# LittleDang/2DLIW-SLAM

Hardware: AMD Instinct MI355X
Metric: sliding-window solves/sec (30 KF, 2k scan pts) (higher is better)
Workload: dtype f64; 1 GPU; C2 synthetic: 49152 windows/GPU x (n=30 frames, L=2000 laser_factor blocks, 29 IMU + 29 wheel, 1800 ground); step = init-topology LM solve (cap 50 iters) + marginalization per window; windows_per_gpu=49152, frames=30, laser_blocks=2000, parallelism=windows replicated over 1 GPU(s), no data-path collective, distinct_windows_per_gpu=64

## Files before the change

### 2dliw-slam_amd/__init__.py

```python
import ctypes as C
import os

import numpy as np

_HERE = os.path.dirname(os.path.abspath(__file__))
LIB_PATH = os.path.join(_HERE, "libliw_window.so")

LIW_MODE_INIT, LIW_MODE_TRACK, LIW_MODE_MARG = 0, 1, 2
LIW_ENODEV = -19
LASER_PARTIAL = 128
LASER_PARTIAL_COMPACT = 48

dp = C.POINTER(C.c_double)
ip = C.POINTER(C.c_int)
up = C.POINTER(C.c_ubyte)


class LiwError(RuntimeError):
    def __init__(self, code, msg):
        super().__init__("liw error %d: %s" % (code, msg))
        self.code = code


class ParamsC(C.Structure):
    _fields_ = [("T_imu_to_wheel", C.c_double * 16), ("T_imu_to_laser", C.c_double * 16), ("g", C.c_double),
                ("line_to_line_sigma", C.c_double), ("manifold_p_sigma", C.c_double), ("manifold_q_sigma", C.c_double),
                ("imu_noise_acc_sigma", C.c_double * 3), ("imu_bias_acc_sigma", C.c_double * 3),
                ("imu_noise_gyro_sigma", C.c_double * 3), ("imu_bias_gyro_sigma", C.c_double * 3),
                ("wheel_sigma", C.c_double * 3), ("fast_mode", C.c_int), ("normalize_extrinsics", C.c_int),
                ("device", C.c_int)]


class WindowC(C.Structure):
    _fields_ = [("n", C.c_int), ("L", C.c_int), ("states", dp), ("laser_frame", ip), ("laser_pts", dp),
                ("match_pose", dp), ("has_match", up), ("imu_X", dp), ("imu_J", dp), ("imu_sqrtP", dp), ("imu_Dt", dp),
                ("wheel_T", dp), ("wheel_sqrtP", dp), ("wheel_Dt", dp)]


class SummaryC(C.Structure):
    _fields_ = [("iterations", C.c_int), ("successful_steps", C.c_int), ("termination", C.c_int),
                ("initial_cost", C.c_double), ("final_cost", C.c_double)]


class BatchC(C.Structure):
    _fields_ = [("B", C.c_int), ("n", C.c_int), ("Ltot", C.c_int), ("x", C.c_void_p), ("laser_off", C.c_void_p),
                ("laser_frame", C.c_void_p), ("laser_pts", C.c_void_p), ("match_pose", C.c_void_p),
                ("has_match", C.c_void_p), ("imu_X", C.c_void_p), ("imu_J", C.c_void_p), ("imu_sqrtP", C.c_void_p),
                ("imu_Dt", C.c_void_p), ("wheel_T", C.c_void_p), ("wheel_sqrtP", C.c_void_p), ("prior_X", C.c_void_p),
                ("prior_J", C.c_void_p), ("prior_R", C.c_void_p), ("has_prior", C.c_void_p), ("eval_small", C.c_int),
                ("history_records", C.c_int)]


class WsLayoutC(C.Structure):
    _fields_ = [("bytes", C.c_size_t), ("laser_partial_off", C.c_size_t * 2), ("laser_partial_bytes", C.c_size_t),
                ("info_off", C.c_size_t), ("history_off", C.c_size_t), ("laser_partial_stride", C.c_int)]


EXPORTS = [
    "liw_create", "liw_destroy", "liw_last_error", "liw_get_extrinsics", "liw_set_window", "liw_clear_window", "liw_solve", "liw_get_history",
    "liw_linearize", "liw_eval_factors", "liw_marginalize", "liw_get_prior", "liw_set_prior", "liw_batch_ws_layout",
    "liw_batch_set_max_iters", "liw_batch_launch_paths", "liw_batch_packed_rows", "liw_batch_linearize", "liw_batch_time_kernels", "liw_batch_lm_begin", "liw_batch_lm_linearize", "liw_batch_laser_records", "liw_batch_lm_step",
    "liw_batch_lm_finish", "liw_batch_lm_linearize_async", "liw_batch_lm_join", "liw_batch_exchange_doubles", "liw_batch_exchange_pack",
    "liw_batch_exchange_unpack", "liw_batch_solve_sharded", "liw_batch_exchange_timing", "liw_batch_p2p_area_doubles", "liw_batch_p2p_setup", "liw_batch_p2p_status", "liw_batch_solve", "liw_batch_marg_linearize", "liw_batch_marg_schur", "liw_batch_export_dense",
    "liw_set_timing", "liw_get_timing", "liw_batch_imu_preint", "liw_batch_wheel_preint", "liw_imu_preint_create", "liw_imu_preint_destroy", "liw_imu_preint_reset",
    "liw_imu_preint_add", "liw_imu_preint_update_only_t", "liw_imu_preint_Dt", "liw_imu_preint_result",
    "liw_wheel_preint_create", "liw_wheel_preint_destroy", "liw_wheel_preint_reset", "liw_wheel_preint_add",
    "liw_wheel_preint_update_only_t", "liw_wheel_preint_result",
]

_LIB = None


def lib():
    global _LIB
    if _LIB is None:
        if not os.path.exists(LIB_PATH):
            raise LiwError(-2, "libliw_window.so is not built (run python 2dliw-slam_amd/build.py); there is no CPU fallback")
        try:
            import torch
        except ImportError:
            pass
        L = C.CDLL(LIB_PATH)
        L.liw_create.restype = C.c_void_p
        L.liw_create.argtypes = [C.POINTER(ParamsC)]
        L.liw_last_error.restype = C.c_char_p
        L.liw_last_error.argtypes = [C.c_void_p]
        L.liw_destroy.argtypes = [C.c_void_p]
        L.liw_imu_preint_create.restype = C.c_void_p
        L.liw_imu_preint_create.argtypes = [C.POINTER(ParamsC)]
        L.liw_wheel_preint_create.restype = C.c_void_p
        L.liw_wheel_preint_create.argtypes = [C.POINTER(ParamsC)]
        L.liw_imu_preint_Dt.restype = C.c_double
        for name in ("liw_imu_preint_destroy", "liw_wheel_preint_destroy"):
            getattr(L, name).argtypes = [C.c_void_p]
        _LIB = L
    return _LIB


def params_struct(prm, device=0):
    s = ParamsC()
    s.T_imu_to_wheel[:] = [float(v) for v in np.asarray(prm["T_imu_to_wheel"], dtype=np.float64).reshape(16)]
    s.T_imu_to_laser[:] = [float(v) for v in np.asarray(prm["T_imu_to_laser"], dtype=np.float64).reshape(16)]
    for k in ("g", "line_to_line_sigma", "manifold_p_sigma", "manifold_q_sigma"):
        setattr(s, k, float(prm[k]))
    for k in ("imu_noise_acc_sigma", "imu_bias_acc_sigma", "imu_noise_gyro_sigma", "imu_bias_gyro_sigma", "wheel_sigma"):
        getattr(s, k)[:] = [float(v) for v in prm[k]]
    s.fast_mode = int(bool(prm.get("fast_mode", False)))
    s.normalize_extrinsics = int(bool(prm.get("normalize_extrinsics", True)))
    s.device = int(device)
    return s


def _p(a):
    return a.ctypes.data_as(dp)


WINDOW_FIELDS = ("states", "laser_frame", "laser_pts", "match_pose", "has_match", "imu_X", "imu_J", "imu_sqrtP", "imu_Dt",
                 "wheel_T", "wheel_sqrtP", "wheel_Dt")


class Window:

    def __init__(self, d):
        self.n = int(d["n"])
        self.a = {}
        for k in WINDOW_FIELDS:
            dt = np.int32 if k == "laser_frame" else (np.uint8 if k == "has_match" else np.float64)
            arr = np.ascontiguousarray(np.array(d[k], dtype=dt, copy=True))
            if arr.size == 0:
                arr = np.zeros(12 if k == "laser_pts" else 1, dtype=dt)
            self.a[k] = arr
        self.L = int(np.asarray(d["laser_frame"]).shape[0])
        c = WindowC()
        c.n, c.L = self.n, self.L
        c.states = _p(self.a["states"]); c.laser_frame = self.a["laser_frame"].ctypes.data_as(ip)
        c.laser_pts = _p(self.a["laser_pts"]); c.match_pose = _p(self.a["match_pose"])
        c.has_match = self.a["has_match"].ctypes.data_as(up)
        for k in ("imu_X", "imu_J", "imu_sqrtP", "imu_Dt", "wheel_T", "wheel_sqrtP", "wheel_Dt"):
            setattr(c, k, _p(self.a[k]))
        self.c = c

    def __getitem__(self, k):
        return self.a[k]


class Solver:

    def __init__(self, prm, device=0):
        self.L = lib()
        self._ps = params_struct(prm, device)
        self.h = C.c_void_p(self.L.liw_create(C.byref(self._ps)))
        if not self.h:
            raise LiwError(-22, "liw_create failed")
        self.win = None

    def close(self):
        if self.h:
            self.L.liw_destroy(self.h)
            self.h = None

    def __del__(self):
        try:
            self.close()
        except Exception:
            pass

    def _chk(self, r):
        if r < 0:
            raise LiwError(r, self.L.liw_last_error(self.h).decode())
        return r

    def extrinsics(self):
        a, b = np.zeros(16), np.zeros(16)
        self._chk(self.L.liw_get_extrinsics(self.h, _p(a), _p(b)))
        return a.reshape(4, 4), b.reshape(4, 4)

    def set_window(self, win):
        self.win = win
        self._chk(self.L.liw_set_window(self.h, C.byref(win.c)))

    def _solve(self, mode, max_iters):
        s = SummaryC()
        self._chk(self.L.liw_solve(self.h, C.c_int(mode), C.c_int(max_iters), C.byref(s)))
        return dict(iterations=s.iterations, successful=s.successful_steps, termination=s.termination,
                    initial_cost=s.initial_cost, final_cost=s.final_cost)

    def init_solve(self, max_iters=0):
        return self._solve(LIW_MODE_INIT, max_iters)

    def solve(self, max_iters=0):
        return self._solve(LIW_MODE_TRACK, max_iters)

    def history(self, max_records=128):
        x = np.zeros((max_records, self.win.n, 15))
        r = self._chk(self.L.liw_get_history(self.h, _p(x), C.c_int(max_records)))
        return x[:r]

    def linearize(self, mode):
        N = 15 * self.win.n
        H, g, c = np.zeros((N, N)), np.zeros(N), C.c_double(0)
        self._chk(self.L.liw_linearize(self.h, C.c_int(mode), _p(H), _p(g), C.byref(c)))
        return H, g, c.value

    def eval_factors(self, mode):
        n, L = self.win.n, self.win.L
        out = dict(laser_res=np.zeros((max(L, 1), 2)), laser_jac=np.zeros((max(L, 1), 2, 12)), imu_res=np.zeros((max(n - 1, 1), 15)),
                   imu_jac=np.zeros((max(n - 1, 1), 15, 30)), wheel_res=np.zeros((max(n - 1, 1), 3)), wheel_jac=np.zeros((max(n - 1, 1), 3, 12)),
                   ground_res=np.zeros((n, 2)), ground_jac=np.zeros((n, 2, 6)))
        self._chk(self.L.liw_eval_factors(self.h, C.c_int(mode), *[_p(out[k]) for k in
                                          ("laser_res", "laser_jac", "imu_res", "imu_jac", "wheel_res", "wheel_jac", "ground_res", "ground_jac")]))
        out["laser_res"], out["laser_jac"] = out["laser_res"][:L], out["laser_jac"][:L]
        out["imu_res"], out["imu_jac"] = out["imu_res"][:n - 1], out["imu_jac"][:n - 1]
        out["wheel_res"], out["wheel_jac"] = out["wheel_res"][:n - 1], out["wheel_jac"][:n - 1]
        return out

    def marginalization(self):
        out = np.zeros(36 + 225 + 15)
        base = out.ctypes.data
        self._chk(self.L.liw_marginalize(self.h, C.cast(base, dp), C.cast(base + 36 * 8, dp), C.cast(base + 261 * 8, dp)))
        return dict(sqrt_H=out[:36].reshape(6, 6), Delta_H=out[36:261].reshape(15, 15), Delta_g=out[261:])

    def get_prior(self):
        X, J, R = np.zeros(15), np.zeros(225), np.zeros(15)
        has = self._chk(self.L.liw_get_prior(self.h, _p(X), _p(J), _p(R)))
        return (X, J.reshape(15, 15), R) if has else None

    def set_prior(self, prior):
        if prior is None:
            self._chk(self.L.liw_set_prior(self.h, C.c_int(0), None, None, None))
            return
        X, J, R = [np.ascontiguousarray(v, dtype=np.float64) for v in prior]
        self._chk(self.L.liw_set_prior(self.h, C.c_int(1), _p(X), _p(J.reshape(225)), _p(R)))


class ImuPreintegration:

    def __init__(self, prm):
        self.L = lib()
        self._ps = params_struct(prm)
        self.h = C.c_void_p(self.L.liw_imu_preint_create(C.byref(self._ps)))

    def __del__(self):
        try:
            self.L.liw_imu_preint_destroy(self.h)
        except Exception:
            pass

    def reset_imu_measure(self, time, acc_bias, gyr_bias):
        a, g = np.ascontiguousarray(acc_bias, dtype=np.float64), np.ascontiguousarray(gyr_bias, dtype=np.float64)
        self.L.liw_imu_preint_reset(self.h, C.c_double(time), _p(a), _p(g))

    def add_imu_measure(self, t, acc, gyro):
        a, g = np.ascontiguousarray(acc, dtype=np.float64), np.ascontiguousarray(gyro, dtype=np.float64)
        return bool(self.L.liw_imu_preint_add(self.h, C.c_double(t), _p(a), _p(g)))

    def update_only_t(self, t):
        self.L.liw_imu_preint_update_only_t(self.h, C.c_double(t))

    @property
    def Dt(self):
        return self.L.liw_imu_preint_Dt(self.h)

    def get_preintegraption_result(self):
        X, J, P, Dt = np.zeros(15), np.zeros(225), np.zeros(225), C.c_double(0)
        self.L.liw_imu_preint_result(self.h, _p(X), _p(J), _p(P), C.byref(Dt))
        return X, J.reshape(15, 15), P.reshape(15, 15), Dt.value


class WheelPreintegration:

    def __init__(self, prm):
        self.L = lib()
        self._ps = params_struct(prm)
        self.h = C.c_void_p(self.L.liw_wheel_preint_create(C.byref(self._ps)))

    def __del__(self):
        try:
            self.L.liw_wheel_preint_destroy(self.h)
        except Exception:
            pass

    def reset_wheel_odom_measure(self, time):
        self.L.liw_wheel_preint_reset(self.h, C.c_double(time))

    def add_wheel_odom_measure(self, t, R9, t3):
        r, tt = np.ascontiguousarray(R9, dtype=np.float64).reshape(9), np.ascontiguousarray(t3, dtype=np.float64)
        return bool(self.L.liw_wheel_preint_add(self.h, C.c_double(t), _p(r), _p(tt)))

    def update_only_t(self, t):
        self.L.liw_wheel_preint_update_only_t(self.h, C.c_double(t))

    def get_preintegraption_result(self):
        T, P, Dt = np.zeros(12), np.zeros(9), C.c_double(0)
        self.L.liw_wheel_preint_result(self.h, _p(T), _p(P), C.byref(Dt))
        return T, P.reshape(3, 3), Dt.value


class HostPreint:

    def __init__(self, prm):
        self.prm = prm

    def imu_preint(self, samples, t_start, t_end, bias6):
        p = ImuPreintegration(self.prm)
        for i, s in enumerate(np.asarray(samples)):
            p.add_imu_measure(s[0], s[1:4], s[4:7])
            if i == 0:
                p.reset_imu_measure(t_start, bias6[0:3], bias6[3:6])
        p.update_only_t(t_end)
        return p.get_preintegraption_result()

    def wheel_preint(self, samples, t_start, t_end):
        p = WheelPreintegration(self.prm)
        did = False
        for s in np.asarray(samples):
            if not did and s[0] > t_start:
                p.update_only_t(t_start)
                p.reset_wheel_odom_measure(t_start)
                did = True
            p.add_wheel_odom_measure(s[0], s[1:10], s[10:13])
        if not did:
            p.update_only_t(t_start)
            p.reset_wheel_odom_measure(t_start)
        p.update_only_t(t_end)
        return p.get_preintegraption_result()


from .batch import BatchPreint, BatchSolver, shard_laser
from . import fleet, gridmap, laser, laser_batch, loop, loop_batch, outputs, posegraph, posegraph_batch
from .fleet import FleetTracker, FleetTrajectory
from .loop_batch import FleetLoopDetector
from .posegraph_batch import FleetBackEnd
```

### 2dliw-slam_amd/batch.py

```python
import ctypes as C

import numpy as np


XFN = C.CFUNCTYPE(C.c_int, C.c_void_p, C.c_void_p, C.c_void_p, C.c_size_t, C.c_void_p)


def shard_laser(win, rank, world):
    L = int(np.asarray(win["laser_frame"]).shape[0])
    lo, hi = (L * rank) // world, (L * (rank + 1)) // world
    out = dict(win)
    out["laser_frame"] = np.asarray(win["laser_frame"])[lo:hi].copy()
    out["laser_pts"] = np.asarray(win["laser_pts"])[lo:hi].copy()
    return out


def allreduce_sum_(t, group=None):
    import torch.distributed as dist
    if dist.is_available() and dist.is_initialized() and dist.get_world_size(group) > 1:
        dist.all_reduce(t, op=dist.ReduceOp.SUM, group=group)
    return t


def allgather_(out, t, group=None):
    import torch.distributed as dist
    if dist.is_available() and dist.is_initialized() and dist.get_world_size(group) > 1:
        if t.is_cuda and dist.get_backend(group) == "gloo":
            import torch
            host = torch.empty(out.shape, dtype=out.dtype)
            dist.all_gather_into_tensor(host.view(-1), t.cpu(), group=group)
            out.copy_(host)
        else:
            dist.all_gather_into_tensor(out.view(-1), t, group=group)
    else:
        out.view(-1)[:t.numel()].copy_(t)
    return out


EXCHANGES = ("allreduce", "oneshot", "auto", "p2p")


class TorchComm:

    def __init__(self, group=None):
        self.group = group

    def all_reduce_sum_(self, t):
        return allreduce_sum_(t, self.group)

    def all_gather_(self, out, t):
        return allgather_(out, t, self.group)

    def all_reduce_max_(self, t):
        import torch.distributed as dist
        if dist.is_available() and dist.is_initialized() and dist.get_world_size(self.group) > 1:
            if t.is_cuda and dist.get_backend(self.group) == "gloo":
                h = t.cpu()
                dist.all_reduce(h, op=dist.ReduceOp.MAX, group=self.group)
                t.copy_(h)
            else:
                dist.all_reduce(t, op=dist.ReduceOp.MAX, group=self.group)
        return t


class LockstepComm:

    def __init__(self, shared, rank):
        self.sh, self.rank = shared, rank

    @staticmethod
    def make(world):
        import threading
        shared = {"slots": [None] * world, "bar": threading.Barrier(world), "world": world}
        return [LockstepComm(shared, r) for r in range(world)]

    def _deposit(self, t):
        self.sh["slots"][self.rank] = t
        self.sh["bar"].wait()

    def all_reduce_sum_(self, t):
        self._deposit(t)
        tot = self.sh["slots"][0].clone()
        for r in range(1, self.sh["world"]):
            tot += self.sh["slots"][r]
        self.sh["bar"].wait()
        t.copy_(tot)
        self.sh["bar"].wait()
        return t

    def all_gather_(self, out, t):
        self._deposit(t)
        for r in range(self.sh["world"]):
            out[r].copy_(self.sh["slots"][r])
        self.sh["bar"].wait()
        return out

    def all_reduce_max_(self, t):
        self._deposit(t)
        tot = self.sh["slots"][0].clone()
        for r in range(1, self.sh["world"]):
            tot = self.torch_max(tot, self.sh["slots"][r])
        self.sh["bar"].wait()
        t.copy_(tot)
        self.sh["bar"].wait()
        return t

    @staticmethod
    def torch_max(a, b):
        import torch
        return torch.maximum(a, b)


def host_arrays(windows):
    B = len(windows)
    Ls = [int(np.asarray(w["laser_frame"]).shape[0]) for w in windows]
    Ltot = int(sum(Ls))
    off = np.zeros(B + 1, dtype=np.int32)
    off[1:] = np.cumsum(Ls)
    cat = lambda k, dt: np.ascontiguousarray(np.concatenate([np.asarray(w[k], dtype=dt).reshape(-1) for w in windows]))
    pts = np.concatenate([np.asarray(w["laser_pts"], dtype=np.float64).reshape(-1, 12) for w in windows], axis=0) if Ltot else np.zeros((1, 12))
    return dict(
        x=cat("states", np.float64), laser_off=off, laser_frame=cat("laser_frame", np.int32) if Ltot else np.zeros(1, np.int32),
        laser_pts=np.ascontiguousarray(pts.T).reshape(-1),
        match_pose=cat("match_pose", np.float64), has_match=cat("has_match", np.uint8),
        imu_X=cat("imu_X", np.float64), imu_J=cat("imu_J", np.float64), imu_sqrtP=cat("imu_sqrtP", np.float64), imu_Dt=cat("imu_Dt", np.float64),
        wheel_T=cat("wheel_T", np.float64), wheel_sqrtP=cat("wheel_sqrtP", np.float64),
        prior_X=np.zeros(B * 15), prior_J=np.zeros(B * 225), prior_R=np.zeros(B * 15), has_prior=np.zeros(B, dtype=np.int32), _Ltot=Ltot)


def tiled_tensors(base, tile, device):
    import torch
    B, nb, n = int(tile["B"]), len(base), int(base[0]["n"])
    dev = torch.device(device)
    assert B >= 1 and nb >= 1
    reps, rem = divmod(B, nb)
    host = host_arrays(base)
    Lb = int(host.pop("_Ltot"))
    Lrem = int(host["laser_off"][rem])
    Ltot = reps * Lb + Lrem
    assert Ltot < 2 ** 31, "laser_off is int32"
    d = {k: torch.from_numpy(a if a.size else np.zeros(1, dtype=a.dtype)).to(dev) for k, a in host.items()}

    t_ = {}

    def cyc(t, per):
        if per == 0 or t.numel() < nb * per:
            return t.clone()
        return torch.cat([t.repeat(reps), t[:rem * per]]) if rem else t.repeat(reps)
    for k, per in (("has_match", n), ("imu_X", (n - 1) * 15), ("imu_J", (n - 1) * 225), ("imu_sqrtP", (n - 1) * 225), ("imu_Dt", n - 1),
                   ("wheel_T", (n - 1) * 12), ("wheel_sqrtP", (n - 1) * 9)):
        t_[k] = cyc(d[k], per)
    if Lb:
        pb = d["laser_pts"].view(12, Lb)
        t_["laser_pts"] = (torch.cat([pb.repeat(1, reps), pb[:, :Lrem]], dim=1) if Lrem else pb.repeat(1, reps)).contiguous().view(-1)
        fb = d["laser_frame"]
        t_["laser_frame"] = torch.cat([fb.repeat(reps), fb[:Lrem]]) if Lrem else fb.repeat(reps)
    else:
        t_["laser_pts"], t_["laser_frame"] = d["laser_pts"], d["laser_frame"]
    ob = d["laser_off"][:nb].to(torch.int64)
    off = (torch.arange(reps, device=dev, dtype=torch.int64)[:, None] * Lb + ob[None, :]).reshape(-1)
    tail = reps * Lb + d["laser_off"][:rem + 1].to(torch.int64)
    t_["laser_off"] = torch.cat([off, tail]).to(torch.int32)
    assert t_["laser_off"].numel() == B + 1
    st = np.ascontiguousarray(np.asarray(tile["states"], dtype=np.float64).reshape(-1))
    mp = np.ascontiguousarray(np.asarray(tile["match_pose"], dtype=np.float64).reshape(-1))
    assert st.size == B * n * 15 and mp.size == B * n * 12
    t_["x"] = torch.from_numpy(st).to(dev)
    t_["match_pose"] = torch.from_numpy(mp).to(dev)
    z = lambda m, dt=torch.float64: torch.zeros(m, dtype=dt, device=dev)
    t_.update(prior_X=z(B * 15), prior_J=z(B * 225), prior_R=z(B * 15), has_prior=z(B, torch.int32))
    return t_, B, Ltot


class BatchSolver:

    def __init__(self, prm, windows, device="cuda:0", history_records=0, rank=0, world=1, group=None, exchange="allreduce", force_exchange=False, comm=None, tile=None):
        import torch
        from . import BatchC, WsLayoutC, lib, params_struct, LiwError
        self.torch = torch
        self.LiwError = LiwError
        self.L = lib()
        self.dev = torch.device(device)
        dev_index = self.dev.index if self.dev.index is not None else 0
        self._ps = params_struct(prm, dev_index)
        self.h = C.c_void_p(self.L.liw_create(C.byref(self._ps)))
        self.rank, self.world, self.group = rank, world, group
        assert exchange in EXCHANGES, exchange
        self.exchange, self.sharded = exchange, (world > 1 or force_exchange)
        self.comm = comm if comm is not None else TorchComm(group)
        self.exchange_ms, self.exchange_calls, self._xev, self._xbuf = 0.0, 0, [], {}
        self.time_exchange = False
        if world > 1:
            windows = [shard_laser(w, rank, world) for w in windows]
        self.n = int(windows[0]["n"])
        n = self.n
        for w in windows:
            assert int(w["n"]) == n, "uniform n per batch"
        if tile is None:
            self.B = len(windows)
            host = host_arrays(windows)
            self.Ltot = int(host.pop("_Ltot"))
            self.t = {}
            for k, a in host.items():
                if a.size == 0:
                    a = np.zeros(1, dtype=a.dtype)
                self.t[k] = torch.from_numpy(a).to(self.dev)
        else:
            self.t, self.B, self.Ltot = tiled_tensors(windows, tile, self.dev)
        B = self.B
        self.history_records = int(history_records)
        lay = WsLayoutC()
        r = self.L.liw_batch_ws_layout(C.c_int(B), C.c_int(n), C.c_int(self.history_records), C.byref(lay))
        if r < 0:
            raise LiwError(r, "liw_batch_ws_layout")
        self.lay = lay
        self.ws = torch.zeros(int(lay.bytes), dtype=torch.uint8, device=self.dev)
        b = BatchC()
        b.B, b.n, b.Ltot = B, n, self.Ltot
        for k in ("x", "laser_off", "laser_frame", "laser_pts", "match_pose", "has_match", "imu_X", "imu_J", "imu_sqrtP", "imu_Dt",
                  "wheel_T", "wheel_sqrtP", "prior_X", "prior_J", "prior_R", "has_prior"):
            setattr(b, k, self.t[k].data_ptr())
        b.eval_small = 1
        b.history_records = self.history_records
        self.b = b
        nd = int(lay.laser_partial_bytes) // 8
        self.PL_raw = [self.ws[int(lay.laser_partial_off[k]):int(lay.laser_partial_off[k]) + nd * 8].view(torch.float64) for k in range(2)]
        self._pl_mode = 0

    @property
    def PL(self):
        from . import LASER_PARTIAL
        if int(self.lay.laser_partial_stride) == LASER_PARTIAL:
            return self.PL_raw
        out = []
        for k in range(2):
            o = self.torch.empty(self.B * self.n * LASER_PARTIAL, dtype=self.torch.float64, device=self.dev)
            self._chk(self.L.liw_batch_laser_records(self.h, C.byref(self.b), C.c_int(self._pl_mode), C.c_int(k), self._wsp(),
                                                     C.c_void_p(o.data_ptr()), self._stream()))
            out.append(o)
        return out

    INPUT_KEYS = ("x", "laser_off", "laser_frame", "laser_pts", "match_pose", "has_match", "imu_X", "imu_J", "imu_sqrtP", "imu_Dt", "wheel_T", "wheel_sqrtP")

    def rebind(self, t, Ltot):
        for k in self.INPUT_KEYS:
            self.t[k] = t[k]
            setattr(self.b, k, t[k].data_ptr())
        self.Ltot = int(Ltot)
        self.b.Ltot = int(Ltot)

    def close(self):
        if self.h:
            self.L.liw_destroy(self.h)
            self.h = None

    def __del__(self):
        try:
            self.close()
        except Exception:
            pass

    def _chk(self, r):
        if r < 0:
            raise self.LiwError(r, self.L.liw_last_error(self.h).decode())
        return r

    def _stream(self):
        return C.c_void_p(self.torch.cuda.current_stream(self.dev).cuda_stream)

    def _wsp(self):
        return C.c_void_p(self.ws.data_ptr())

    def launch_paths(self):
        flags, rows, blocks = C.c_int(0), C.c_longlong(0), C.c_longlong(0)
        self._chk(self.L.liw_batch_launch_paths(self.h, C.byref(self.b), self._wsp(), C.byref(flags)))
        self._chk(self.L.liw_batch_packed_rows(self.h, C.byref(self.b), self._wsp(), C.byref(rows), C.byref(blocks)))
        return dict(flags=flags.value, large_batch_format=bool(flags.value & 1), lane_per_group_laser=bool(flags.value & 2), packed_rows=rows.value,
                    blocks=blocks.value, padding_ratio=(64.0 * rows.value / blocks.value) if (rows.value and blocks.value) else None)

    def solve(self, mode, max_iters=0, use_graph=False):
        self._pl_mode = int(mode)
        if not self.sharded:
            if use_graph:
                torch = self.torch
                if getattr(self, "_side", None) is None:
                    self._side = torch.cuda.Stream(device=self.dev)
                cur = torch.cuda.current_stream(self.dev)
                self._side.wait_stream(cur)
                with torch.cuda.stream(self._side):
                    self._chk(self.L.liw_batch_solve(self.h, C.byref(self.b), C.c_int(mode), C.c_int(max_iters), self._wsp(), self._stream(), C.c_int(1)))
                cur.wait_stream(self._side)
                return
            self._chk(self.L.liw_batch_solve(self.h, C.byref(self.b), C.c_int(mode), C.c_int(max_iters), self._wsp(), self._stream(), C.c_int(0)))
            return
        buf, allb, nd = self._xbuffers(mode)
        if self.exchange == "p2p":
            assert getattr(self, "_p2p", None) is not None and self._p2p["mode"] == mode, "attach the receive areas first (p2p_attach_local / p2p_attach_ipc)"
            self._chk(self.L.liw_batch_exchange_timing(self.h, C.c_int(1 if self.time_exchange else 0), None, None))
            self._chk(self.L.liw_batch_solve_sharded(self.h, C.byref(self.b), C.c_int(mode), C.c_int(max_iters), self._wsp(), self._stream(),
                                                     C.c_void_p(buf.data_ptr()), None, C.c_int(max(self.world, 1)), XFN(0), None))
            self._last_x = buf
            return
        oneshot = self.exchange == "oneshot"
        err = []

        def _cb(user, pbuf, pall, doubles, stream):
            try:
                if oneshot:
                    self.comm.all_gather_(allb, buf)
                    return max(self.world, 1)
                self.comm.all_reduce_sum_(buf)
                return 1
            except BaseException as e:
                err.append(e)
                return -1
        cb = XFN(_cb)
        self._chk(self.L.liw_batch_exchange_timing(self.h, C.c_int(1 if self.time_exchange else 0), None, None))
        r = self.L.liw_batch_solve_sharded(self.h, C.byref(self.b), C.c_int(mode), C.c_int(max_iters), self._wsp(), self._stream(),
                                           C.c_void_p(buf.data_ptr()), C.c_void_p(allb.data_ptr()) if allb is not None else None,
                                           C.c_int(max(self.world, 1)), cb, None)
        if err:
            raise err[0]
        self._chk(r)
        self._last_x = allb[0] if oneshot else buf

    def pick_exchange(self, mode, reps=3):
        t = self.torch
        reps = max(1, int(reps))
        nd = int(self.L.liw_batch_exchange_doubles(C.c_int(self.B), C.c_int(self.n), C.c_int(mode)))
        buf = t.zeros(nd, dtype=t.float64, device=self.dev)
        allb = t.zeros((max(self.world, 1), nd), dtype=t.float64, device=self.dev)
        ms = {}
        for name in ("allreduce", "oneshot"):
            for rep in range(reps + 1):
                if rep == 1:
                    e0, e1 = t.cuda.Event(enable_timing=True), t.cuda.Event(enable_timing=True)
                    e0.record()
                if name == "allreduce":
                    self.comm.all_reduce_sum_(buf)
                else:
                    self.comm.all_gather_(allb, buf)
                    buf.copy_(allb.sum(dim=0))
            e1.record()
            t.cuda.synchronize(self.dev)
            ms[name] = e0.elapsed_time(e1) / reps
            buf.zero_()
        both = t.tensor([ms["allreduce"], ms["oneshot"]], dtype=t.float64, device=self.dev)
        self.comm.all_reduce_max_(both)
        ms = {"allreduce": float(both[0].item()), "oneshot": float(both[1].item())}
        ms["picked"] = "oneshot" if ms["oneshot"] < ms["allreduce"] else "allreduce"
        self.exchange = ms["picked"]
        self._xbuf = {}
        self.exchange_pick = ms
        return ms

    def _xbuffers(self, mode):
        if self.exchange == "auto":
            self.pick_exchange(mode)
        nd = int(self.L.liw_batch_exchange_doubles(C.c_int(self.B), C.c_int(self.n), C.c_int(mode)))
        if (mode, "buf") not in self._xbuf:
            t = self.torch
            self._xbuf[(mode, "buf")] = t.zeros(nd, dtype=t.float64, device=self.dev)
            self._xbuf[(mode, "all")] = t.zeros((max(self.world, 1), nd), dtype=t.float64, device=self.dev) if self.exchange == "oneshot" else None
        return self._xbuf[(mode, "buf")], self._xbuf[(mode, "all")], nd

    def exchange_bytes(self, mode):
        return 8 * int(self.L.liw_batch_exchange_doubles(C.c_int(self.B), C.c_int(self.n), C.c_int(mode)))

    def _exchange(self, mode, candidate):
        buf, allb, nd = self._xbuffers(mode)
        s = self._stream()
        ev = None
        if self.time_exchange:
            ev = (self.torch.cuda.Event(enable_timing=True), self.torch.cuda.Event(enable_timing=True))
            ev[0].record()
        self._chk(self.L.liw_batch_exchange_pack(self.h, C.byref(self.b), C.c_int(mode), C.c_int(candidate), self._wsp(), C.c_void_p(buf.data_ptr()), s))
        if self.exchange == "oneshot":
            self.comm.all_gather_(allb, buf)
            self._chk(self.L.liw_batch_exchange_unpack(self.h, C.byref(self.b), C.c_int(mode), C.c_int(candidate), self._wsp(),
                                                       C.c_void_p(allb.data_ptr()), C.c_int(max(self.world, 1)), s))
            self._last_x = allb[0]
        else:
            self.comm.all_reduce_sum_(buf)
            self._chk(self.L.liw_batch_exchange_unpack(self.h, C.byref(self.b), C.c_int(mode), C.c_int(candidate), self._wsp(),
                                                       C.c_void_p(buf.data_ptr()), C.c_int(1), s))
            self._last_x = buf
        if ev:
            ev[1].record()
            self._xev.append(ev)

    def _lin_exchange(self, mode, candidate):
        self._chk(self.L.liw_batch_lm_linearize_async(self.h, C.byref(self.b), C.c_int(mode), C.c_int(candidate), self._wsp(), self._stream()))
        self._exchange(mode, candidate)
        self._chk(self.L.liw_batch_lm_join(self.h, self._stream()))

    def active_windows(self, mode):
        buf, allb, nd = self._xbuffers(mode)
        if self.exchange == "oneshot":
            return int(round(float(allb[:, nd - 1].sum().item()))) // max(self.world, 1)
        return int(round(float(buf[nd - 1].item()))) // max(self.world, 1)

    def _p2p_alloc(self, mode):
        t = self.torch
        L = self.L
        L.liw_batch_p2p_area_doubles.restype = C.c_size_t
        nd = int(L.liw_batch_p2p_area_doubles(C.c_int(self.B), C.c_int(self.n), C.c_int(mode), C.c_int(max(self.world, 1))))
        area = t.zeros(nd, dtype=t.float64, device=self.dev)
        flags = t.zeros(max(self.world, 1), dtype=t.int64, device=self.dev)
        return area, flags

    def _p2p_set(self, mode, area_ptrs, flag_ptrs, keep):
        w = max(self.world, 1)
        A = (C.c_void_p * w)(*area_ptrs)
        F = (C.c_void_p * w)(*flag_ptrs)
        self._chk(self.L.liw_batch_p2p_setup(self.h, C.c_int(self.rank), C.c_int(w), A, F))
        self._p2p = {"mode": mode, "keep": keep}

    @staticmethod
    def p2p_attach_local(ranks, mode):
        bufs = [rk._p2p_alloc(mode) for rk in ranks]
        for rk in ranks:
            rk.torch.cuda.synchronize(rk.dev)
            rk._p2p_set(mode, [a.data_ptr() for a, _ in bufs], [f.data_ptr() for _, f in bufs], bufs)

    def p2p_attach_ipc(self, mode):
        import torch.distributed as dist
        hip = C.CDLL("libamdhip64.so")

        class Handle(C.Structure):
            _fields_ = [("reserved", C.c_byte * 64)]
        L = self.L
        L.liw_batch_p2p_area_doubles.restype = C.c_size_t
        w = max(self.world, 1)
        nd = int(L.liw_batch_p2p_area_doubles(C.c_int(self.B), C.c_int(self.n), C.c_int(mode), C.c_int(w)))
        own = []
        for nbytes in (8 * nd, 8 * w):
            p = C.c_void_p()
            assert hip.hipMalloc(C.byref(p), C.c_size_t(nbytes)) == 0
            assert hip.hipMemset(p, 0, C.c_size_t(nbytes)) == 0
            own.append(p)
        hs = []
        for p in own:
            h = Handle()
            assert hip.hipIpcGetMemHandle(C.byref(h), p) == 0
            hs.append(bytes(h.reserved))
        allh = [None] * w
        dist.all_gather_object(allh, hs, group=self.group)
        areas, flags = [], []
        for r in range(w):
            if r == self.rank:
                areas.append(own[0].value); flags.append(own[1].value)
                continue
            ptrs = []
            for raw in allh[r]:
                h = Handle()
                C.memmove(h.reserved, raw, 64)
                q = C.c_void_p()
                assert hip.hipIpcOpenMemHandle(C.byref(q), h, C.c_uint(1)) == 0
                ptrs.append(q.value)
            areas.append(ptrs[0]); flags.append(ptrs[1])
        dist.barrier(group=self.group)
        self._p2p_ptrs = (areas, flags)
        self._p2p_set(mode, areas, flags, own)

    def exchange_timing(self):
        self.torch.cuda.synchronize(self.dev)
        ms = [a.elapsed_time(b) for a, b in self._xev]
        self._xev = []
        avg, cnt = C.c_double(0.0), C.c_int(0)
        self._chk(self.L.liw_batch_exchange_timing(self.h, C.c_int(1 if self.time_exchange else 0), C.byref(avg), C.byref(cnt)))
        tot, num = sum(ms) + avg.value * cnt.value, len(ms) + cnt.value
        return (tot / num if num else 0.0), num

    def lm_begin(self, mode, max_iters=0):
        K = self._chk(self.L.liw_batch_set_max_iters(self.h, C.c_int(mode), C.c_int(max_iters)))
        self._chk(self.L.liw_batch_lm_begin(self.h, C.byref(self.b), C.c_int(mode), C.c_int(K), self._wsp(), self._stream()))
        return K

    def lm_linearize(self, mode, candidate):
        self._pl_mode = int(mode)
        self._chk(self.L.liw_batch_lm_linearize(self.h, C.byref(self.b), C.c_int(mode), C.c_int(candidate), self._wsp(), self._stream()))

    def lm_step(self, mode):
        self._chk(self.L.liw_batch_lm_step(self.h, C.byref(self.b), C.c_int(mode), self._wsp(), self._stream()))

    def lm_finish(self, mode):
        self._chk(self.L.liw_batch_lm_finish(self.h, C.byref(self.b), C.c_int(mode), self._wsp(), self._stream()))

    def time_kernels(self, mode, reps=3):
        out = (C.c_double * 6)()
        self._chk(self.L.liw_batch_time_kernels(self.h, C.byref(self.b), C.c_int(mode), self._wsp(), self._stream(), C.c_int(reps), out))
        self.torch.cuda.synchronize(self.dev)
        return dict(zip(("k_lin_laser", "k_lin_imu", "k_lin_small", "k_lm_step", "k_marg_schur", "k_lin_laser_marg"), [float(v) for v in out]))

    def linearize(self, mode):
        self._pl_mode = int(mode)
        self._chk(self.L.liw_batch_linearize(self.h, C.byref(self.b), C.c_int(mode), self._wsp(), self._stream()))
        if self.sharded:
            self._exchange_plain(mode)

    def _exchange_plain(self, mode):
        self.comm.all_reduce_sum_(self.PL_raw[0])

    def export_dense(self, mode):
        N = 15 * self.n
        torch = self.torch
        H = torch.zeros((self.B, N, N), dtype=torch.float64, device=self.dev)
        g = torch.zeros((self.B, N), dtype=torch.float64, device=self.dev)
        c = torch.zeros(self.B, dtype=torch.float64, device=self.dev)
        self._chk(self.L.liw_batch_export_dense(self.h, C.byref(self.b), C.c_int(mode), C.c_int(0), self._wsp(), C.c_void_p(H.data_ptr()),
                                                C.c_void_p(g.data_ptr()), C.c_void_p(c.data_ptr()), self._stream()))
        return H, g, c

    def marginalize(self):
        torch = self.torch
        sH = torch.zeros((self.B, 36), dtype=torch.float64, device=self.dev)
        dH = torch.zeros((self.B, 225), dtype=torch.float64, device=self.dev)
        dg = torch.zeros((self.B, 15), dtype=torch.float64, device=self.dev)
        s = self._stream()
        from . import LIW_MODE_MARG as _MARG
        self._pl_mode = _MARG
        self._chk(self.L.liw_batch_marg_linearize(self.h, C.byref(self.b), self._wsp(), s))
        if self.sharded:
            from . import LIW_MODE_MARG
            self._exchange(LIW_MODE_MARG, 0)
        self._chk(self.L.liw_batch_marg_schur(self.h, C.byref(self.b), self._wsp(), C.c_void_p(sH.data_ptr()), C.c_void_p(dH.data_ptr()),
                                              C.c_void_p(dg.data_ptr()), s))
        return sH, dH, dg

    def states(self):
        return self.t["x"].cpu().numpy().reshape(self.B, self.n, 15)

    def set_states(self, x):
        self.t["x"].copy_(self.torch.from_numpy(np.ascontiguousarray(x, dtype=np.float64).reshape(-1)).to(self.dev))

    def summaries(self):
        from . import SummaryC
        raw = self.ws[int(self.lay.info_off):int(self.lay.info_off) + C.sizeof(SummaryC) * self.B].cpu().numpy().tobytes()
        arr = (SummaryC * self.B).from_buffer_copy(raw)
        return [dict(iterations=a.iterations, successful=a.successful_steps, termination=a.termination,
                     initial_cost=a.initial_cost, final_cost=a.final_cost) for a in arr]

    def history(self):
        if not self.history_records:
            return None
        nd = self.history_records * self.B * self.n * 15
        o = int(self.lay.history_off)
        return self.ws[o:o + nd * 8].view(self.torch.float64).cpu().numpy().reshape(self.history_records, self.B, self.n, 15)

    def set_timing(self, on):
        self._chk(self.L.liw_set_timing(self.h, C.c_int(int(on))))

    def get_timing(self):
        a, b, c, d = C.c_double(0), C.c_int(0), C.c_double(0), C.c_int(0)
        self._chk(self.L.liw_get_timing(self.h, C.byref(a), C.byref(b), C.byref(c), C.byref(d)))
        return dict(linearize_ms=a.value, linearize_launches=b.value, step_ms=c.value, step_launches=d.value)


class BatchPreint:

    def __init__(self, prm, device="cuda:0"):
        import torch
        from . import lib, params_struct, LiwError
        self.torch, self.LiwError, self.L = torch, LiwError, lib()
        self.dev = torch.device(device)
        self._ps = params_struct(prm, self.dev.index if self.dev.index is not None else 0)
        self.h = C.c_void_p(self.L.liw_create(C.byref(self._ps)))

    def close(self):
        if self.h:
            self.L.liw_destroy(self.h)
            self.h = None

    def __del__(self):
        try:
            self.close()
        except Exception:
            pass

    def _chk(self, r):
        if r < 0:
            raise self.LiwError(r, self.L.liw_last_error(self.h).decode())

    def _pack(self, intervals, width):
        torch = self.torch
        M = len(intervals)
        cnt = [int(np.asarray(iv[0]).shape[0]) for iv in intervals]
        off = np.zeros(M + 1, dtype=np.int32)
        off[1:] = np.cumsum(cnt)
        smp = np.concatenate([np.asarray(iv[0], dtype=np.float64).reshape(-1, width) for iv in intervals], axis=0) if M else np.zeros((1, width))
        ts = np.array([iv[1] for iv in intervals], dtype=np.float64)
        te = np.array([iv[2] for iv in intervals], dtype=np.float64)
        d = lambda a: torch.from_numpy(np.ascontiguousarray(a)).to(self.dev)
        return M, d(off), d(smp.reshape(-1)), d(ts), d(te)

    def imu(self, intervals):
        torch = self.torch
        M, off, smp, ts, te = self._pack(intervals, 7)
        bias = torch.from_numpy(np.ascontiguousarray(np.array([iv[3] for iv in intervals], dtype=np.float64).reshape(-1))).to(self.dev)
        z = lambda *sh: torch.zeros(sh, dtype=torch.float64, device=self.dev)
        X, J, P, S, Dt = z(M, 15), z(M, 15, 15), z(M, 15, 15), z(M, 15, 15), z(M)
        p = lambda t: C.c_void_p(t.data_ptr())
        self._chk(self.L.liw_batch_imu_preint(self.h, C.c_int(M), p(off), p(smp), p(ts), p(te), p(bias), p(X), p(J), p(P), p(S), p(Dt),
                                              C.c_void_p(torch.cuda.current_stream(self.dev).cuda_stream)))
        self.last_P = P
        return X, J, S, Dt

    def wheel(self, intervals):
        torch = self.torch
        M, off, smp, ts, te = self._pack(intervals, 13)
        z = lambda *sh: torch.zeros(sh, dtype=torch.float64, device=self.dev)
        T, S, Dt = z(M, 12), z(M, 3, 3), z(M)
        p = lambda t: C.c_void_p(t.data_ptr())
        self._chk(self.L.liw_batch_wheel_preint(self.h, C.c_int(M), p(off), p(smp), p(ts), p(te), p(T), p(S), p(Dt),
                                                C.c_void_p(torch.cuda.current_stream(self.dev).cuda_stream)))
        return T, S, Dt
```

### 2dliw-slam_amd/csrc/k_laser_slab.hip

```cpp
#include "liw_kernels.hpp"
#include <algorithm>
#include <cstdlib>

namespace liw {

#ifdef LIW_CLK
__device__ long long g_clk_slab[16];
#define SSTAMP(id) do { asm volatile("s_waitcnt vmcnt(0) lgkmcnt(0)" ::: "memory"); if (item == slab_items_probe && (threadIdx.x & 63) == 0) g_clk_slab[(id)] = clock64(); } while (0)
__device__ int slab_items_probe = 11000;
#else
#define SSTAMP(id) do { } while (0)
#endif

namespace {

constexpr int TF2 = 24;
__device__ __forceinline__ void frame_tf2(const DevParams& P, const double* pose6, double* o) {
    typedef LJN<3> J3;
    const V3<J3> p = cast_v3<J3>(pose6);
    const V3<J3> th(seed<3>(pose6[3], 0, true), seed<3>(pose6[4], 1, true), seed<3>(pose6[5], 2, true));
    const Iso<J3> Twl = mul(make_tf(p, th), cast_iso<J3>(P.Ril, P.til));
    const J3 tt[2] = {Twl.t.x, Twl.t.y};
#pragma unroll
    for (int r = 0; r < 2; ++r) {
#pragma unroll
        for (int c = 0; c < 2; ++c) {
            o[r * 2 + c] = Twl.R(r, c).v;
#pragma unroll
            for (int k = 0; k < 3; ++k) o[6 + 4 * k + 2 * r + c] = Twl.R(r, c).d[k];
        }
        o[4 + r] = tt[r].v;
#pragma unroll
        for (int k = 0; k < 3; ++k) o[18 + 2 * k + r] = tt[r].d[k];
    }
}

constexpr int slab_pairidx(int c1, int c2) { return laser_pairidx<true>(c1, c2); }
constexpr int slab_pairidx1(int c1, int c2) { return laser_pairidx<false>(c1, c2); }
constexpr int slab_slot_code(int s) { return laser_slot_code<true>(s); }
constexpr int slab_slot_code1(int s) { return laser_slot_code<false>(s); }
template <bool BOTH, int S_> __device__ __forceinline__ double slab_slot(const double* acc) {
    constexpr int code = BOTH ? slab_slot_code(S_) : slab_slot_code1(S_);
    if constexpr (code < 0) return 0.0;
    else if constexpr ((code & 64) != 0) return -acc[code & 63];
    else return acc[code & 63];
}

constexpr int STG = 34;
template <bool BOTH, int C_, int I_ = 0> __device__ __forceinline__ void slab_stage(double* st, const double* acc) {
    if constexpr (I_ < 16) {
        typedef double __attribute__((ext_vector_type(2))) dbl2;
        dbl2 v;
        v.x = slab_slot<BOTH, 32 * C_ + 2 * I_>(acc); v.y = slab_slot<BOTH, 32 * C_ + 2 * I_ + 1>(acc);
        *reinterpret_cast<dbl2*>(st + 2 * I_) = v;
        slab_stage<BOTH, C_, I_ + 1>(st, acc);
    }
}
template <bool BOTH, int C_> __device__ __forceinline__ void slab_flush(double* lds, const unsigned long long* pw, const double* acc, int lane) {
    if constexpr (C_ < 4) {
        typedef double __attribute__((ext_vector_type(2))) dbl2;
        lds_sync();
        slab_stage<BOTH, C_>(lds + lane * STG, acc);
        lds_sync();
        const int wq = lane >> 4, pc = lane & 15;
#pragma unroll
        for (int t = 0; t < 16; ++t) {
            const int w = 4 * t + wq;
            const unsigned long long p = pw[w];
            const dbl2 v = *reinterpret_cast<const dbl2*>(lds + w * STG + 2 * pc);
            if (p) __builtin_nontemporal_store(v, reinterpret_cast<dbl2*>(reinterpret_cast<double*>(p) + 32 * C_ + 2 * pc));
        }
        slab_flush<BOTH, C_ + 1>(lds, pw, acc, lane);
    }
}

template <int N_, int S_> __device__ __forceinline__ double slab_total(const double* acc) {
    if constexpr (S_ < N_) return acc[S_]; else return 0.0;
}
template <int N_, int S0_, int CNT_, int I_ = 0> __device__ __forceinline__ void slab_stage_totals(double* st, const double* acc) {
    if constexpr (I_ < CNT_) {
        typedef double __attribute__((ext_vector_type(2))) dbl2;
        dbl2 v;
        v.x = slab_total<N_, S0_ + 2 * I_>(acc); v.y = slab_total<N_, S0_ + 2 * I_ + 1>(acc);
        *reinterpret_cast<dbl2*>(st + 2 * I_) = v;
        slab_stage_totals<N_, S0_, CNT_, I_ + 1>(st, acc);
    }
}
template <int N_> __device__ __forceinline__ void slab_flush_compact(double* lds, const unsigned long long* pw, const double* acc, int lane) {
    typedef double __attribute__((ext_vector_type(2))) dbl2;
    static_assert(LPC == 48 && N_ <= LPC, "one and a half chunks");
    lds_sync();
    slab_stage_totals<N_, 0, 16>(lds + lane * STG, acc);
    lds_sync();
    {
        const int wq = lane >> 4, pc = lane & 15;
#pragma unroll
        for (int t = 0; t < 16; ++t) {
            const int w = 4 * t + wq;
            const unsigned long long p = pw[w];
            const dbl2 v = *reinterpret_cast<const dbl2*>(lds + w * STG + 2 * pc);
            if (p) __builtin_nontemporal_store(v, reinterpret_cast<dbl2*>(reinterpret_cast<double*>(p) + 2 * pc));
        }
    }
    lds_sync();
    slab_stage_totals<N_, 32, 8>(lds + lane * STG, acc);
    lds_sync();
    {
        const int wq = lane >> 3, pc = lane & 7;
#pragma unroll
        for (int t = 0; t < 8; ++t) {
            const int w = 8 * t + wq;
            const unsigned long long p = pw[w];
            const dbl2 v = *reinterpret_cast<const dbl2*>(lds + w * STG + 2 * pc);
            if (p) __builtin_nontemporal_store(v, reinterpret_cast<dbl2*>(reinterpret_cast<double*>(p) + 32 + 2 * pc));
        }
    }
}

__device__ __forceinline__ double slab_weight(double d1x, double d1y, double d2x, double d2y) {
    const double l2 = fmin(d1x * d1x + d1y * d1y, d2x * d2x + d2y * d2y);
    const double lmin25 = l2 > 0.0 ? 25.0 * (l2 * fast_rsqrt(l2)) : 0.0;
    return lmin25 > 0.0 ? lmin25 * fast_rsqrt(lmin25) : 0.0;
}

constexpr int SLAB = 64;
constexpr int ROWD = LASER_SLAB_ROWD;
constexpr int NPL = ROWD / SLAB;

}

template <bool BOTH>
__device__ __forceinline__ void slab_item(const LinArgs& A, const DevParams& P, const int item) {
    const int lane = threadIdx.x & 63, n = A.n;
    const int s = item / n, f = item % n;
    SSTAMP(0);
    const int b = A.laser_perm[(size_t)f * ((size_t)laser_slab_count(A.B) * SLAB) + (size_t)s * SLAB + lane];
    bool in = b >= 0;
    const int bb = in ? b : 0;
    const int g0 = A.group_off[bb * (n + 1) + f], g1 = A.group_off[bb * (n + 1) + f + 1];
    const int hm = A.has_match[bb * n + f];
    const int curv = A.lm ? A.lm[bb].cur : 0;
    double pa6[6], pb6[6];
#pragma unroll
    for (int k = 0; k < 6; ++k) {
        pa6[k] = BOTH ? A.x[(size_t)bb * n * 15 + k] : A.match_pose[((size_t)bb * n + f) * 12 + k];
        pb6[k] = A.x[((size_t)bb * n + f) * 15 + k];
    }
    if (in) in = window_live(A, bb);
    if (!__any(in)) return;
    const bool fon = in && hm != 0 && (BOTH || A.mode != LIW_MODE_TRACK || f == n - 1 || A.marg_older);
    const int cnt = fon ? g1 - g0 : 0;
    int maxc = cnt;
#pragma unroll
    for (int o = 32; o > 0; o >>= 1) maxc = max(maxc, __shfl_xor(maxc, o, 64));
    maxc = __builtin_amdgcn_readfirstlane(maxc);
    const int psel = (in && A.lm) ? (A.candidate ? 1 - curv : curv) : 0;
    constexpr int TFR = 4;
    __shared__ double lds[2 * (TF2 - TFR) * SLAB];
    double* const lta = lds;
    double* const ltb = lds + (TF2 - TFR) * SLAB;
    double ra[TFR], rb[TFR];
    SSTAMP(1);
    {
        double ta2[TF2], tb2[TF2];
        if (in && maxc > 0) { frame_tf2(P, pa6, ta2); frame_tf2(P, pb6, tb2); }
        else {
#pragma unroll
            for (int k = 0; k < TF2; ++k) { ta2[k] = 0.0; tb2[k] = 0.0; }
        }
#pragma unroll
        for (int k = 0; k < TF2; ++k) {
            if (k < TFR) { ra[k] = ta2[k]; rb[k] = tb2[k]; }
            else { lta[(k - TFR) * SLAB + lane] = ta2[k]; ltb[(k - TFR) * SLAB + lane] = tb2[k]; }
        }
    }
    lds_sync();
    SSTAMP(2);
    constexpr int NACC = BOTH ? 45 : 21;
    double acc[NACC];
#pragma unroll
    for (int e = 0; e < NACC; ++e) acc[e] = 0.0;
    const double* row0 = A.laser_pk + (size_t)A.laser_slab_off[(size_t)s * n + f] * ROWD + lane;
    auto load_row = [&](double* q, int j) {
        const double* r = row0 + (size_t)j * ROWD;
#pragma unroll
        for (int c = 0; c < NPL; ++c) q[c] = __builtin_nontemporal_load(r + c * SLAB);
    };
    const double w0 = P.laser_sqrt_info;
#define TA(k) ((k) < TFR ? ra[(k) < TFR ? (k) : 0] : lta[((k) < TFR ? 0 : (k) - TFR) * SLAB + lane])
#define TB(k) ((k) < TFR ? rb[(k) < TFR ? (k) : 0] : ltb[((k) < TFR ? 0 : (k) - TFR) * SLAB + lane])
    auto block = [&](const double* p) {
        const double d1x = p[0] - p[2], d1y = p[1] - p[3];
        const double d2x = p[4] - p[6], d2y = p[5] - p[7];
        const double l2 = fmin(d1x * d1x + d1y * d1y, d2x * d2x + d2y * d2y);
        const double lmin25 = l2 > 0.0 ? 25.0 * (l2 * fast_rsqrt(l2)) : 0.0;
        const double sum = lmin25 > 0.0 ? lmin25 * fast_rsqrt(lmin25) : 0.0;
        double Ap[2], Bp[2], C[2][2];
#pragma unroll
        for (int r = 0; r < 2; ++r) {
            Ap[r] = TA(4 + r) + TA(r * 2) * p[0] + TA(r * 2 + 1) * p[1];
            Bp[r] = TA(4 + r) + TA(r * 2) * p[2] + TA(r * 2 + 1) * p[3];
            C[0][r] = TB(4 + r) + TB(r * 2) * p[4] + TB(r * 2 + 1) * p[5];
            C[1][r] = TB(4 + r) + TB(r * 2) * p[6] + TB(r * 2 + 1) * p[7];
        }
        __builtin_amdgcn_sched_barrier(0);
        const double ux = Bp[0] - Ap[0], uy = Bp[1] - Ap[1];
        const double zz = ux * ux + uy * uy;
        const bool regular = zz > 0.0;
        const double rlen = regular ? fast_rsqrt(zz) : 1.0;
        const double lx = ux * rlen, ly = uy * rlen;
        double dBx[3], dBy[3], dlx[3], dly[3];
#pragma unroll
        for (int k = 0; k < 3; ++k) {
            const double m0 = TA(6 + 4 * k), m1 = TA(6 + 4 * k + 1), m3 = TA(6 + 4 * k + 2), m4 = TA(6 + 4 * k + 3);
            const double t0 = TA(18 + 2 * k), t1 = TA(18 + 2 * k + 1);
            const double dAx = t0 + m0 * p[0] + m1 * p[1];
            const double dAy = t1 + m3 * p[0] + m4 * p[1];
            dBx[k] = t0 + m0 * p[2] + m1 * p[3];
            dBy[k] = t1 + m3 * p[2] + m4 * p[3];
            const double dux = dBx[k] - dAx, duy = dBy[k] - dAy;
            const double pr = lx * dux + ly * duy;
            dlx[k] = (dux - lx * pr) * rlen;
            dly[k] = (duy - ly * pr) * rlen;
        }
        const double w = sum * w0;
        __builtin_amdgcn_sched_barrier(0);
#pragma unroll
        for (int k = 0; k < 2; ++k) {
            __builtin_amdgcn_sched_barrier(0);
            const double pt0 = p[4 + 2 * k], pt1 = p[5 + 2 * k];
            const double ex = C[k][0] - Bp[0], ey = C[k][1] - Bp[1];
            double dCx[3], dCy[3];
#pragma unroll
            for (int m = 0; m < 3; ++m) {
                dCx[m] = TB(18 + 2 * m) + TB(6 + 4 * m) * pt0 + TB(6 + 4 * m + 1) * pt1;
                dCy[m] = TB(18 + 2 * m + 1) + TB(6 + 4 * m + 2) * pt0 + TB(6 + 4 * m + 3) * pt1;
            }
            double dist, jc[8], ws = w;
            if (regular) {
                const double sg = lx * ey - ly * ex;
                ws = sg < 0.0 ? -w : w;
                dist = fabs(sg);
                {
                    const double prj = lx * ex + ly * ey;
                    const double vx = ex - prj * lx, vy = ey - prj * ly;
                    if (vx * vx + vy * vy == 0.0) ws = __builtin_nan("");
                }
                jc[0] = ly; jc[1] = -lx;
#pragma unroll
                for (int m = 0; m < 3; ++m) {
                    jc[2 + m] = dlx[m] * ey - dly[m] * ex - lx * dBy[m] + ly * dBx[m];
                    jc[5 + m] = lx * dCy[m] - ly * dCx[m];
                }
            } else {
                dist = sqrt(ex * ex + ey * ey);
                const double nx = ex / dist, ny = ey / dist;
                jc[0] = -nx; jc[1] = -ny;
#pragma unroll
                for (int m = 0; m < 3; ++m) {
                    jc[2 + m] = -(nx * dBx[m] + ny * dBy[m]);
                    jc[5 + m] = nx * dCx[m] + ny * dCy[m];
                }
            }
            __builtin_amdgcn_sched_barrier(0);
            double rw[9];
#pragma unroll
            for (int c = 0; c < 8; ++c) rw[c] = ws * jc[c];
            rw[8] = sum * (w0 * dist);
            if constexpr (BOTH) {
#pragma unroll
                for (int c1 = 0; c1 < 9; ++c1)
#pragma unroll
                    for (int c2 = c1; c2 < 9; ++c2) acc[c1 * 9 - c1 * (c1 - 1) / 2 + (c2 - c1)] += rw[c1] * rw[c2];
            } else {
                const double r1[6] = {-rw[0], -rw[1], rw[5], rw[6], rw[7], rw[8]};
#pragma unroll
                for (int c1 = 0; c1 < 6; ++c1)
#pragma unroll
                    for (int c2 = c1; c2 < 6; ++c2) acc[c1 * 6 - c1 * (c1 - 1) / 2 + (c2 - c1)] += r1[c1] * r1[c2];
            }
        }
    };
    bool irregular = false;
    auto block_fast = [&](const double* p) {
        const double d1x = p[0] - p[2], d1y = p[1] - p[3];
        const double d2x = p[4] - p[6], d2y = p[5] - p[7];
        const double w = slab_weight(d1x, d1y, d2x, d2y) * w0;
        const double ux = -(ra[0] * d1x + ra[1] * d1y), uy = -(ra[2] * d1x + ra[3] * d1y);
        const double zz = ux * ux + uy * uy;
        if (__builtin_expect(!(zz > 0.0), 0)) { irregular = true; return; }
        const double Bx = TA(4) + ra[0] * p[2] + ra[1] * p[3], By = TA(5) + ra[2] * p[2] + ra[3] * p[3];
        const double tbx = TB(4), tby = TB(5);
        double ex[2], ey[2];
#pragma unroll
        for (int k = 0; k < 2; ++k) {
            ex[k] = (tbx + rb[0] * p[4 + 2 * k] + rb[1] * p[5 + 2 * k]) - Bx;
            ey[k] = (tby + rb[2] * p[4 + 2 * k] + rb[3] * p[5 + 2 * k]) - By;
        }
        __builtin_amdgcn_sched_barrier(0);
        const double rlen = fast_rsqrt(zz);
        const double lx = ux * rlen, ly = uy * rlen;
        const double rlw = rlen * w;
        const double lxw = ux * rlw, lyw = uy * rlw;
        double dlxw[3], dlyw[3], kap[3];
        if constexpr (BOTH) {
#pragma unroll
            for (int k = 0; k < 3; ++k) {
                const double m0 = TA(6 + 4 * k), m1 = TA(6 + 4 * k + 1), m3 = TA(6 + 4 * k + 2), m4 = TA(6 + 4 * k + 3);
                const double dux = -(m0 * d1x + m1 * d1y), duy = -(m3 * d1x + m4 * d1y);
                const double pr = lx * dux + ly * duy;
                dlxw[k] = (dux - lx * pr) * rlw;
                dlyw[k] = (duy - ly * pr) * rlw;
                const double dBx = TA(18 + 2 * k) + m0 * p[2] + m1 * p[3];
                const double dBy = TA(18 + 2 * k + 1) + m3 * p[2] + m4 * p[3];
                kap[k] = lyw * dBx - lxw * dBy;
            }
        }
        __builtin_amdgcn_sched_barrier(0);
        double al[3], be[3], ga[3];
#pragma unroll
        for (int m = 0; m < 3; ++m) {
            al[m] = lxw * TB(18 + 2 * m + 1) - lyw * TB(18 + 2 * m);
            be[m] = lxw * TB(6 + 4 * m + 2) - lyw * TB(6 + 4 * m);
            ga[m] = lxw * TB(6 + 4 * m + 3) - lyw * TB(6 + 4 * m + 1);
        }
        const double tiny = 1e-13 * w;
#pragma unroll
        for (int k = 0; k < 2; ++k) {
            __builtin_amdgcn_sched_barrier(0);
            const double pt0 = p[4 + 2 * k], pt1 = p[5 + 2 * k];
            if constexpr (BOTH) {
                double rw[9];
                rw[0] = lyw; rw[1] = -lxw;
                rw[8] = lxw * ey[k] - lyw * ex[k];
#pragma unroll
                for (int m = 0; m < 3; ++m) {
                    rw[2 + m] = dlxw[m] * ey[k] - dlyw[m] * ex[k] + kap[m];
                    rw[5 + m] = al[m] + be[m] * pt0 + ga[m] * pt1;
                }
                if (__builtin_expect(fabs(rw[8]) <= tiny * (fabs(ex[k]) + fabs(ey[k])), 0)) {
                    const double prj = lx * ex[k] + ly * ey[k];
                    const double vx = ex[k] - prj * lx, vy = ey[k] - prj * ly;
                    if (vx * vx + vy * vy == 0.0) {
#pragma unroll
                        for (int c = 0; c < 8; ++c) rw[c] = __builtin_nan("");
                    }
                }
                __builtin_amdgcn_sched_barrier(0);
#pragma unroll
                for (int c1 = 0; c1 < 9; ++c1)
#pragma unroll
                    for (int c2 = c1; c2 < 9; ++c2) acc[c1 * 9 - c1 * (c1 - 1) / 2 + (c2 - c1)] += rw[c1] * rw[c2];
            } else {
                double rw[6];
                rw[0] = -lyw; rw[1] = lxw;
                rw[5] = lxw * ey[k] - lyw * ex[k];
#pragma unroll
                for (int m = 0; m < 3; ++m) rw[2 + m] = al[m] + be[m] * pt0 + ga[m] * pt1;
                if (__builtin_expect(fabs(rw[5]) <= tiny * (fabs(ex[k]) + fabs(ey[k])), 0)) {
                    const double prj = lx * ex[k] + ly * ey[k];
                    const double vx = ex[k] - prj * lx, vy = ey[k] - prj * ly;
                    if (vx * vx + vy * vy == 0.0) {
#pragma unroll
                        for (int c = 0; c < 5; ++c) rw[c] = __builtin_nan("");
                    }
                }
                __builtin_amdgcn_sched_barrier(0);
#pragma unroll
                for (int c1 = 0; c1 < 6; ++c1)
#pragma unroll
                    for (int c2 = c1; c2 < 6; ++c2) acc[c1 * 6 - c1 * (c1 - 1) / 2 + (c2 - c1)] += rw[c1] * rw[c2];
            }
        }
    };
    const int last = maxc - 1;
    double q0[NPL], q1[NPL];
    if (maxc > 0) {
        load_row(q0, 0);
        for (int j = 0; j < maxc; j += 2) {
            asm volatile("" ::: "memory");
            load_row(q1, min(j + 1, last));
            if (j < cnt) block_fast(q0);
            __builtin_amdgcn_sched_barrier(0);
            load_row(q0, min(j + 2, last));
            if (j + 1 < cnt) block_fast(q1);
            __builtin_amdgcn_sched_barrier(0);
        }
    }
    if (__builtin_expect(__any(irregular), 0)) {
        for (int j = 0; j < maxc; ++j) {
            double q[NPL];
            load_row(q, j);
            const double d1x = q[0] - q[2], d1y = q[1] - q[3];
            const double ux = -(ra[0] * d1x + ra[1] * d1y), uy = -(ra[2] * d1x + ra[3] * d1y);
            if (irregular && j < cnt && !(ux * ux + uy * uy > 0.0)) block(q);
        }
    }
    SSTAMP(3);
#undef TA
#undef TB
    {
        static_assert(SLAB * STG + SLAB <= 2 * (TF2 - TFR) * SLAB && LP == 128, "staging area of the record epilogue");
        unsigned long long* pw = reinterpret_cast<unsigned long long*>(lds + SLAB * STG);
        lds_sync();
        pw[lane] = in ? (unsigned long long)((psel ? A.PL[1] : A.PL[0]) + ((size_t)bb * n + f) * laser_stride(A.pl_compact)) : 0ull;
        if (A.pl_compact) slab_flush_compact<NACC>(lds, pw, acc, lane);
        else slab_flush<BOTH, 0>(lds, pw, acc, lane);
    }
    if (in && A.CS[0]) (psel ? A.CS[1] : A.CS[0])[cs_index(n, bb, CS_LASER, f)] = acc[BOTH ? slab_pairidx(8, 8) : slab_pairidx1(5, 5)];
    SSTAMP(4);
}
__global__ __launch_bounds__(64, 2) void k_lin_laser_slab(LinArgs A, DevParams P) { slab_item<true>(A, P, (int)blockIdx.x); }
__global__ __launch_bounds__(64, 2) void k_lin_laser_slab1(LinArgs A, DevParams P) { slab_item<false>(A, P, (int)blockIdx.x); }

constexpr int SORT_BINS = 4096;
__global__ __launch_bounds__(1024) void k_laser_slab_order(int B, int n, const int* group_off, int* perm) {
    __shared__ int bin[SORT_BINS];
    __shared__ int part[1024];
    const int f = (int)blockIdx.x, t = (int)threadIdx.x;
    const size_t Bp = (size_t)((B + SLAB - 1) / SLAB) * SLAB;
    for (int e = t; e < SORT_BINS; e += 1024) bin[e] = 0;
    __syncthreads();
    auto key = [&](int b) { return SORT_BINS - 1 - min(group_off[b * (n + 1) + f + 1] - group_off[b * (n + 1) + f], SORT_BINS - 1); };
    for (int b = t; b < B; b += 1024) atomicAdd(&bin[key(b)], 1);
    __syncthreads();
    int sum = 0;
#pragma unroll
    for (int k = 0; k < SORT_BINS / 1024; ++k) sum += bin[t * (SORT_BINS / 1024) + k];
    part[t] = sum;
    __syncthreads();
    for (int d = 1; d < 1024; d <<= 1) {
        const int v = t >= d ? part[t - d] : 0;
        __syncthreads();
        part[t] += v;
        __syncthreads();
    }
    int base = part[t] - sum;
#pragma unroll
    for (int k = 0; k < SORT_BINS / 1024; ++k) { const int h = bin[t * (SORT_BINS / 1024) + k]; bin[t * (SORT_BINS / 1024) + k] = base; base += h; }
    __syncthreads();
    for (int b = t; b < B; b += 1024) perm[(size_t)f * Bp + atomicAdd(&bin[key(b)], 1)] = b;
    for (size_t e = (size_t)B + t; e < Bp; e += 1024) perm[(size_t)f * Bp + e] = -1;
}
__global__ void k_laser_slab_max(int B, int n, const int* group_off, const int* perm, int* mx) {
    const int t = blockIdx.x * blockDim.x + threadIdx.x;
    const int S = (B + SLAB - 1) / SLAB;
    if (t >= S * n) return;
    const int s = t / n, f = t % n;
    int m = 0;
    for (int l = 0; l < SLAB; ++l) {
        const int b = perm[(size_t)f * ((size_t)S * SLAB) + (size_t)s * SLAB + l];
        if (b >= 0) m = max(m, group_off[b * (n + 1) + f + 1] - group_off[b * (n + 1) + f]);
    }
    mx[t] = m;
}
__global__ __launch_bounds__(1024) void k_laser_slab_scan(int N, const int* mx, long long* off, const int* hz) {
    __shared__ long long part[1024];
    const int t = threadIdx.x, per = (N + 1023) / 1024;
    long long sum = 0;
    for (int k = 0; k < per; ++k) { const int e = t * per + k; if (e < N) sum += mx[e]; }
    part[t] = sum;
    __syncthreads();
    for (int d = 1; d < 1024; d <<= 1) {
        const long long v = t >= d ? part[t - d] : 0;
        __syncthreads();
        part[t] += v;
        __syncthreads();
    }
    long long base = part[t] - sum;
    for (int k = 0; k < per; ++k) { const int e = t * per + k; if (e < N) { off[e] = base; base += mx[e]; } }
    if (t == 1023) { off[N] = part[1023]; off[N + 1] = hz ? (long long)*hz : 0; }
}
__global__ __launch_bounds__(256) void k_laser_slab_pack(int B, int n, long Ltot, const int* group_off, const int* perm, const double* pts, const long long* off, const int* mx, double* pk) {
    __shared__ double tile[64 * 65];
    __shared__ int g0s[SLAB], cnts[SLAB];
    const int s = (int)blockIdx.x / n, f = (int)blockIdx.x % n, t = threadIdx.x;
    if (t < SLAB) {
        const int b = perm[(size_t)f * ((size_t)((B + SLAB - 1) / SLAB) * SLAB) + (size_t)s * SLAB + t];
        g0s[t] = b >= 0 ? group_off[b * (n + 1) + f] : 0;
        cnts[t] = b >= 0 ? group_off[b * (n + 1) + f + 1] - g0s[t] : 0;
    }
    __syncthreads();
    const int maxc = mx[(size_t)s * n + f];
    double* base = pk + (size_t)off[(size_t)s * n + f] * ROWD;
    for (int jb = 0; jb < maxc; jb += 64) {
        for (int c = 0; c < 8; ++c) {
            const double* plane = pts + (size_t)(c + c / 2) * (size_t)Ltot;
            for (int pass = 0; pass < 4; ++pass) {
                const int l = pass * 16 + (t >> 4), jj = t & 15;
#pragma unroll
                for (int i = 0; i < 4; ++i) {
                    const int j = jb + jj + 16 * i;
                    tile[(jj + 16 * i) * 65 + l] = j < cnts[l] ? plane[(size_t)g0s[l] + j] : 0.0;
                }
            }
            __syncthreads();
            const int rows = min(64, maxc - jb);
            for (int r = t >> 6; r < rows; r += 4) base[(size_t)(jb + r) * ROWD + c * SLAB + (t & 63)] = tile[r * 65 + (t & 63)];
            __syncthreads();
        }
    }
}

#ifdef LIW_CLK
extern "C" void liw_debug_clk_slab(long long* out, int nn) { hipMemcpyFromSymbol(out, HIP_SYMBOL(g_clk_slab), sizeof(long long) * nn); }
#endif
__global__ void k_laser_slab_identity(int B, int n, int* perm) {
    const size_t Bp = (size_t)((B + SLAB - 1) / SLAB) * SLAB;
    const size_t t = (size_t)blockIdx.x * blockDim.x + threadIdx.x;
    if (t < Bp * n) perm[t] = (int)(t % Bp) < B ? (int)(t % Bp) : -1;
}
void launch_laser_slab_prepare(int B, int n, const int* group_off, int* perm, int* mx, long long* off, const int* hz, hipStream_t s) {
    const int N = laser_slab_count(B) * n;
    if (std::getenv("LIW_SLAB_BATCH_ORDER")) hipLaunchKernelGGL(k_laser_slab_identity, dim3((unsigned)(((size_t)N * SLAB + 255) / 256)), dim3(256), 0, s, B, n, perm);
    else hipLaunchKernelGGL(k_laser_slab_order, dim3((unsigned)n), dim3(1024), 0, s, B, n, group_off, perm);
    hipLaunchKernelGGL(k_laser_slab_max, dim3((N + 255) / 256), dim3(256), 0, s, B, n, group_off, (const int*)perm, mx);
    hipLaunchKernelGGL(k_laser_slab_scan, dim3(1), dim3(1024), 0, s, N, (const int*)mx, off, hz);
}
void launch_laser_slab_pack(int B, int n, long Ltot, const int* group_off, const int* perm, const double* pts, const long long* off, const int* mx, double* pk, hipStream_t s) {
    hipLaunchKernelGGL(k_laser_slab_pack, dim3((unsigned)(laser_slab_count(B) * n)), dim3(256), 0, s, B, n, Ltot, group_off, perm, pts, off, mx, pk);
}
void launch_lin_laser_slab(const LinArgs& A, const DevParams& P, hipStream_t s) {
    if (A.mode == LIW_MODE_INIT) hipLaunchKernelGGL(k_lin_laser_slab, dim3((unsigned)(laser_slab_count(A.B) * A.n)), dim3(64), 0, s, A, P);
    else hipLaunchKernelGGL(k_lin_laser_slab1, dim3((unsigned)(laser_slab_count(A.B) * A.n)), dim3(64), 0, s, A, P);
}

}
```

### 2dliw-slam_amd/csrc/liw_capi.hip

```cpp
#include <hip/hip_runtime.h>

#include <algorithm>
#include <cmath>
#include <cstdio>
#include <cstdlib>
#include <atomic>
#include <chrono>
#include <cstring>
#include <string>
#include <vector>

#include "liw_kernels.hpp"

using namespace liw;

struct DevBuf {
    void* p = nullptr;
    size_t cap = 0;
    int ensure(size_t bytes) {
        if (bytes <= cap && p) return 0;
        if (p) (void)hipFree(p);
        p = nullptr; cap = 0;
        if (hipMalloc(&p, bytes ? bytes : 8) != hipSuccess) return -1;
        cap = bytes ? bytes : 8;
        return 0;
    }
    void release() { if (p) (void)hipFree(p); p = nullptr; cap = 0; }
    template <class T> T* as() const { return (T*)p; }
};

struct liw_ctx {
    liw_params prm;
    DevParams dp;
    std::string err;
    bool have_device = false;
    hipStream_t stream = nullptr;
    liw_window hw{};
    bool have_window = false;
    int n = 0, L = 0;
    DevBuf arena;
    void* pinned = nullptr;
    size_t pinned_cap = 0, img_cap = 0, readback_cap = 0;
    int img_cur = 0;
    bool img_valid = false;
    size_t part_off[13] = {0}, part_bytes[13] = {0};
    hipEvent_t ev_upload = nullptr;
    DevBuf prior_X, prior_J, prior_R, has_prior, ws, scratch;
    DevBuf priorn_X, priorn_J, priorn_R, has_priorn, result, marg_status;
    bool spec_marg = true, spec_valid = false;
    bool reattach = true;
    double spec_out[36 + 225 + 15];
    liw_batch sb{};
    liw_ws_layout lay{};
    int hist_records = 0;
    int last_iters = 0;
    int solved_records = 0;
    bool timing = false;
    std::vector<hipEvent_t> ev_lin, ev_step, ev_x;
    size_t ev_lin_used = 0, ev_step_used = 0, xev_used = 0;
    bool time_exchange = false;
    int pack_seq = 0;
    const double* last_x = nullptr;
    int last_x_copies = 1;
    P2pPeers p2p{};
    int p2p_rank = 0, p2p_world = 0;
    unsigned long long p2p_epoch = 0;
    DevBuf p2p_err;
    LinFork fork{};
    bool have_fork = false;
    DevBuf lpk, lpk_off, lpk_mx, lpk_perm;
    struct { const void* ws; const void* pts; const void* frame; int B, n; long Ltot; } lpk_key{};
    bool lpk_on = false;
    long long lpk_rows = 0;
    int* rb_pin = nullptr;
    hipGraphExec_t gexec = nullptr;
    std::vector<unsigned char> gkey;
};

static int fail(liw_ctx* c, int code, const char* what, hipError_t e = hipSuccess) {
    if (c) {
        char buf[256];
        if (e != hipSuccess) snprintf(buf, sizeof buf, "%s: %s", what, hipGetErrorString(e));
        else snprintf(buf, sizeof buf, "%s", what);
        c->err = buf;
    }
    return code;
}
#define HIPCHK(c, call)                                                   \
    do {                                                                  \
        hipError_t e_ = (call);                                           \
        if (e_ != hipSuccess) return fail((c), LIW_EHIP, #call, e_);      \
    } while (0)
#define NEEDDEV(c)                                                                                         \
    do {                                                                                                   \
        if (!(c)) return LIW_EINVAL;                                                                       \
        if (!(c)->have_device) return fail((c), LIW_ENODEV, "no usable gfx950 device (no CPU fallback)"); \
    } while (0)

static void normalize_tf_host(double* R) {
    double c[4];
    double t = R[0] + R[4] + R[8];
    auto M = [&](int r, int cc) { return R[r * 3 + cc]; };
    if (t > 0.0) {
        t = std::sqrt(t + 1.0);
        c[3] = 0.5 * t; t = 0.5 / t;
        c[0] = (M(2, 1) - M(1, 2)) * t; c[1] = (M(0, 2) - M(2, 0)) * t; c[2] = (M(1, 0) - M(0, 1)) * t;
    } else {
        int i = 0;
        if (M(1, 1) > M(0, 0)) i = 1;
        if (M(2, 2) > M(i, i)) i = 2;
        int j = (i + 1) % 3, k = (j + 1) % 3;
        t = std::sqrt(M(i, i) - M(j, j) - M(k, k) + 1.0);
        c[i] = 0.5 * t; t = 0.5 / t;
        c[3] = (M(k, j) - M(j, k)) * t; c[j] = (M(j, i) + M(i, j)) * t; c[k] = (M(k, i) + M(i, k)) * t;
    }
    const double qw = c[3], qx = c[0], qy = c[1], qz = c[2];
    const double tx = 2 * qx, ty = 2 * qy, tz = 2 * qz;
    const double twx = tx * qw, twy = ty * qw, twz = tz * qw, txx = tx * qx, txy = ty * qx, txz = tz * qx, tyy = ty * qy, tyz = tz * qy, tzz = tz * qz;
    R[0] = 1 - (tyy + tzz); R[1] = txy - twz;       R[2] = txz + twy;
    R[3] = txy + twz;       R[4] = 1 - (txx + tzz); R[5] = tyz - twx;
    R[6] = txz - twy;       R[7] = tyz + twx;       R[8] = 1 - (txx + tyy);
}
void liw_normalize_rotation_host(double* R9) { normalize_tf_host(R9); }
hipStream_t liw_ctx_stream(liw_ctx* c) { return c->stream; }
const DevParams* liw_ctx_devparams(liw_ctx* c) { return &c->dp; }
int liw_ctx_device(liw_ctx* c) { return c->prm.device; }
bool liw_ctx_has_device(liw_ctx* c) { return c && c->have_device; }
int liw_ctx_fail(liw_ctx* c, int code, const char* what) { return fail(c, code, what); }

void liw_fill_devparams(const liw_params* prm, DevParams* dp) {
    for (int i = 0; i < 3; ++i) {
        for (int j = 0; j < 3; ++j) { dp->Riw[i * 3 + j] = prm->T_imu_to_wheel[i * 4 + j]; dp->Ril[i * 3 + j] = prm->T_imu_to_laser[i * 4 + j]; }
        dp->tiw[i] = prm->T_imu_to_wheel[i * 4 + 3];
        dp->til[i] = prm->T_imu_to_laser[i * 4 + 3];
    }
    if (prm->normalize_extrinsics) { normalize_tf_host(dp->Riw); normalize_tf_host(dp->Ril); }
    dp->g = prm->g;
    dp->laser_sqrt_info = 1.0 / prm->line_to_line_sigma;
    dp->ground_p_info = 1.0 / prm->manifold_p_sigma;
    dp->ground_q_info = 1.0 / prm->manifold_q_sigma;
    dp->fast_mode = prm->fast_mode;
}

extern "C" {

liw_ctx* liw_create(const liw_params* prm) {
    if (!prm) return nullptr;
    liw_ctx* c = new liw_ctx();
    c->prm = *prm;
    liw_fill_devparams(prm, &c->dp);
    int ndev = 0;
    if (hipGetDeviceCount(&ndev) == hipSuccess && ndev > prm->device && prm->device >= 0) {
        hipDeviceProp_t props;
        if (hipSetDevice(prm->device) == hipSuccess && hipGetDeviceProperties(&props, prm->device) == hipSuccess) {
            if (std::strstr(props.gcnArchName, "gfx950") != nullptr) {
                if (hipStreamCreate(&c->stream) == hipSuccess) c->have_device = true;
                if (c->have_device && hipStreamCreateWithFlags(&c->fork.side[0], hipStreamNonBlocking) == hipSuccess &&
                    hipStreamCreateWithFlags(&c->fork.side[1], hipStreamNonBlocking) == hipSuccess &&
                    hipEventCreateWithFlags(&c->fork.ev_fork, hipEventDisableTiming) == hipSuccess &&
                    hipEventCreateWithFlags(&c->fork.ev_join[0], hipEventDisableTiming) == hipSuccess &&
                    hipEventCreateWithFlags(&c->fork.ev_join[1], hipEventDisableTiming) == hipSuccess &&
                    hipEventCreateWithFlags(&c->fork.ev_compact, hipEventDisableTiming) == hipSuccess)
                    c->have_fork = true;
                if (std::getenv("LIW_SERIAL_ROLES")) c->have_fork = false;
                if (std::getenv("LIW_NO_SPEC_MARG")) c->spec_marg = false;
                if (std::getenv("LIW_NO_REATTACH")) c->reattach = false;
                (void)hipEventCreateWithFlags(&c->ev_upload, hipEventDisableTiming);
            } else {
                c->err = std::string("device is ") + props.gcnArchName + ", this library is built for gfx950 only";
            }
        }
    }
    if (!c->have_device && c->err.empty()) c->err = "no HIP device";
    return c;
}

void liw_destroy(liw_ctx* c) {
    if (!c) return;
    if (c->have_device) {
        (void)hipSetDevice(c->prm.device);
        DevBuf* bufs[] = {&c->lpk, &c->lpk_off, &c->lpk_mx, &c->lpk_perm, &c->p2p_err, &c->arena, &c->prior_X, &c->prior_J, &c->prior_R, &c->has_prior, &c->ws, &c->scratch,
                          &c->priorn_X, &c->priorn_J, &c->priorn_R, &c->has_priorn, &c->result, &c->marg_status};
        if (c->pinned) (void)hipHostFree(c->pinned);
        if (c->rb_pin) (void)hipHostFree(c->rb_pin);
        if (c->ev_upload) (void)hipEventDestroy(c->ev_upload);
        for (DevBuf* b : bufs) b->release();
        for (auto e : c->ev_lin) (void)hipEventDestroy(e);
        for (auto e : c->ev_step) (void)hipEventDestroy(e);
        for (auto e : c->ev_x) (void)hipEventDestroy(e);
        if (c->gexec) (void)hipGraphExecDestroy(c->gexec);
        if (c->have_fork) {
            (void)hipStreamDestroy(c->fork.side[0]); (void)hipStreamDestroy(c->fork.side[1]);
            (void)hipEventDestroy(c->fork.ev_fork); (void)hipEventDestroy(c->fork.ev_join[0]); (void)hipEventDestroy(c->fork.ev_join[1]); (void)hipEventDestroy(c->fork.ev_compact);
        }
        if (c->stream) (void)hipStreamDestroy(c->stream);
    }
    delete c;
}

const char* liw_last_error(const liw_ctx* c) { return c ? c->err.c_str() : "null ctx"; }

int liw_get_extrinsics(const liw_ctx* c, double* A, double* Bm) {
    if (!c) return LIW_EINVAL;
    auto put = [](const double* R, const double* t, double* m) {
        for (int i = 0; i < 3; ++i) { for (int j = 0; j < 3; ++j) m[i * 4 + j] = R[i * 3 + j]; m[i * 4 + 3] = t[i]; }
        m[12] = m[13] = m[14] = 0.0; m[15] = 1.0;
    };
    if (A) put(c->dp.Riw, c->dp.tiw, A);
    if (Bm) put(c->dp.Ril, c->dp.til, Bm);
    return LIW_OK;
}

static size_t al256(size_t v) { return (v + 255) & ~(size_t)255; }
struct FullLayout {
    size_t PL[2], PI[2], PW[2], PG[2], CS[2], x_cand, group_off, lm, solve_ws, info, history, active, imu_pk, imu_pk_bad, bytes;
};
static FullLayout full_layout(int B, int n, int hist) {
    FullLayout f{};
    size_t o = 0;
    const int nm = n > 1 ? n - 1 : 1;
    const int lps = laser_stride(pi_frame_format(B) ? 1 : 0);
    for (int k = 0; k < 2; ++k) { f.PI[k] = o; o = al256(o + sizeof(double) * (size_t)B * pi_doubles_per_window(n)); }
    for (int k = 0; k < 2; ++k) { f.PW[k] = o; o = al256(o + sizeof(double) * (size_t)B * nm * PWS); }
    for (int k = 0; k < 2; ++k) { f.PL[k] = o; o = al256(o + sizeof(double) * (size_t)B * n * lps); }
    for (int k = 0; k < 2; ++k) { f.PG[k] = o; o = al256(o + sizeof(double) * (size_t)B * n * PGS); }
    f.x_cand = o; o = al256(o + sizeof(double) * (size_t)B * n * 15);
    f.group_off = o; o = al256(o + sizeof(int) * (size_t)B * (n + 1));
    f.active = o; o = al256(o + compact_list_bytes_host(B));
    f.lm = o; o = al256(o + sizeof(LmState) * (size_t)B);
    f.solve_ws = o; o = al256(o + sizeof(double) * (size_t)B * n * SOLVE_WS);
    f.info = o; o = al256(o + sizeof(liw_summary) * (size_t)B);
    f.history = hist > 0 ? o : 0;
    if (hist > 0) o = al256(o + sizeof(double) * (size_t)hist * B * n * 15);
    f.imu_pk_bad = o; o = al256(o + 2 * sizeof(int));
    f.imu_pk = o; o = al256(o + sizeof(double) * (size_t)B * nm * IMU_PK);
    for (int k = 0; k < 2; ++k) { f.CS[k] = o; o = al256(o + sizeof(double) * (size_t)B * 4 * n); }
    f.bytes = o;
    return f;
}
static WsView make_view(void* ws, int B, int n, int hist) {
    FullLayout f = full_layout(B, n, hist);
    char* base = (char*)ws;
    WsView v{};
    for (int k = 0; k < 2; ++k) {
        v.PL[k] = (double*)(base + f.PL[k]); v.PI[k] = (double*)(base + f.PI[k]);
        v.PW[k] = (double*)(base + f.PW[k]); v.PG[k] = (double*)(base + f.PG[k]);
    }
    v.x_cand = (double*)(base + f.x_cand);
    v.group_off = (int*)(base + f.group_off);
    v.lm = (LmState*)(base + f.lm);
    v.solve_ws = (double*)(base + f.solve_ws);
    v.info = (liw_summary*)(base + f.info);
    v.history = hist > 0 ? (double*)(base + f.history) : nullptr;
    v.history_records = hist;
    v.active = (int*)(base + f.active);
    v.pi_frame = pi_frame_format(B) ? 1 : 0;
    v.pl_compact = v.pi_frame;
    for (int k = 0; k < 2; ++k) v.CS[k] = (double*)(base + f.CS[k]);
    v.imu_pk = (double*)(base + f.imu_pk);
    v.imu_pk_bad = (int*)(base + f.imu_pk_bad);
    return v;
}

int liw_batch_ws_layout(int B, int n, int history_records, liw_ws_layout* out) {
    if (!out || B <= 0 || n <= 0 || n > 64) return LIW_EINVAL;
    FullLayout f = full_layout(B, n, history_records);
    out->bytes = f.bytes;
    out->laser_partial_off[0] = f.PL[0];
    out->laser_partial_off[1] = f.PL[1];
    out->laser_partial_stride = laser_stride(pi_frame_format(B) ? 1 : 0);
    out->laser_partial_bytes = sizeof(double) * (size_t)B * n * out->laser_partial_stride;
    out->info_off = f.info;
    out->history_off = f.history;
    return LIW_OK;
}

static int check_batch(liw_ctx* c, const liw_batch* b, int min_n = 1) {
    if (!b || b->B <= 0 || b->n <= 0 || b->n > 64) return fail(c, LIW_EINVAL, "bad batch (need 1 <= n <= 64, B >= 1)");
    if (b->n < min_n) return fail(c, LIW_EINVAL, "TRACK / MARG topology needs n >= 2 (the prior block is tied to frame n-2)");
    return LIW_OK;
}
static int min_frames(int mode) { return mode == LIW_MODE_INIT ? 1 : 2; }
static bool lpk_matches(const liw_ctx* c, const liw_batch* b, const void* ws) {
    return c && c->lpk_on && c->lpk_key.ws == ws && c->lpk_key.pts == b->laser_pts && c->lpk_key.frame == b->laser_frame && c->lpk_key.B == b->B &&
           c->lpk_key.n == b->n && c->lpk_key.Ltot == (long)b->Ltot;
}
static int laser_slab_begin(liw_ctx* c, const liw_batch* b, int mode, const WsView& v, void* ws, hipStream_t s, bool may_sync) {
    c->lpk_on = false;
    if (!may_sync || std::getenv("LIW_NO_LASER_SLAB")) return LIW_OK;
    const int S = laser_slab_count(b->B), N = S * b->n;
    if ((mode == LIW_MODE_INIT ? N < 2048 : S < 256) || b->Ltot <= 0) return LIW_OK;
    if (c->lpk_mx.ensure(sizeof(int) * (size_t)N) || c->lpk_off.ensure(sizeof(long long) * ((size_t)N + 2)) || c->lpk_perm.ensure(sizeof(int) * (size_t)N * 64))
        return fail(c, LIW_ENOMEM, "hipMalloc");
    launch_laser_slab_prepare(b->B, b->n, v.group_off, c->lpk_perm.as<int>(), c->lpk_mx.as<int>(), c->lpk_off.as<long long>(), v.imu_pk_bad + 1, s);
    if (!c->rb_pin) HIPCHK(c, hipHostMalloc((void**)&c->rb_pin, 64, hipHostMallocDefault));
    long long* const tail = reinterpret_cast<long long*>(c->rb_pin) + 2;
    tail[0] = 0; tail[1] = 1;
    HIPCHK(c, hipMemcpyAsync(tail, c->lpk_off.as<long long>() + N, 2 * sizeof(long long), hipMemcpyDeviceToHost, s));
    HIPCHK(c, hipStreamSynchronize(s));
    const long long rows = tail[0];
    if (tail[1] != 0 || rows <= 0) return LIW_OK;
    if (rows * 64 > 4 * (long long)b->Ltot + 64ll * N) return LIW_OK;
    if (c->lpk.ensure(sizeof(double) * LASER_SLAB_ROWD * (size_t)rows)) { c->lpk.release(); return LIW_OK; }
    launch_laser_slab_pack(b->B, b->n, (long)b->Ltot, v.group_off, c->lpk_perm.as<int>(), b->laser_pts, c->lpk_off.as<long long>(), c->lpk_mx.as<int>(), c->lpk.as<double>(), s);
    c->lpk_key = {ws, b->laser_pts, b->laser_frame, b->B, b->n, (long)b->Ltot};
    c->lpk_on = true;
    c->lpk_rows = rows;
    return LIW_OK;
}
static LinArgs lin_args(const liw_batch* b, int mode, const double* x, const WsView& v, int candidate, bool use_lm, bool packed = false, const liw_ctx* c = nullptr, const void* ws = nullptr) {
    LinArgs A{};
    A.B = b->B; A.n = b->n; A.mode = mode; A.eval_small = b->eval_small;
    A.x = x; A.group_off = v.group_off; A.laser_off = b->laser_off; A.laser_pts = b->laser_pts; A.Ltot = b->Ltot;
    A.match_pose = b->match_pose; A.has_match = b->has_match;
    A.imu_X = b->imu_X; A.imu_J = b->imu_J; A.imu_sqrtP = b->imu_sqrtP; A.imu_Dt = b->imu_Dt;
    A.wheel_T = b->wheel_T; A.wheel_sqrtP = b->wheel_sqrtP;
    for (int k = 0; k < 2; ++k) { A.PL[k] = v.PL[k]; A.PI[k] = v.PI[k]; A.PW[k] = v.PW[k]; A.PG[k] = v.PG[k]; }
    A.lm = use_lm ? v.lm : nullptr;
    A.active = use_lm ? v.active : nullptr;
    A.candidate = candidate;
    A.pi_frame = v.pi_frame;
    A.pl_compact = v.pl_compact;
    for (int k = 0; k < 2; ++k) A.CS[k] = v.pi_frame ? v.CS[k] : nullptr;
    if (packed && b->n > 1 && b->eval_small) { A.imu_pk = v.imu_pk; A.imu_pk_bad = v.imu_pk_bad; }
    if (packed) A.laser_hz = v.imu_pk_bad + 1;
    if (packed && lpk_matches(c, b, ws)) { A.laser_pk = c->lpk.as<double>(); A.laser_slab_off = c->lpk_off.as<long long>(); A.laser_perm = c->lpk_perm.as<int>(); }
    return A;
}
static StepArgs step_args(liw_ctx* c, const liw_batch* b, int mode, int max_iters, const WsView& v) {
    StepArgs a{};
    a.B = b->B; a.n = b->n; a.mode = mode; a.max_iters = max_iters; a.fast_mode = c->prm.fast_mode;
    a.x = b->x; a.match_pose = b->match_pose; a.has_match = b->has_match;
    a.prior_X = b->prior_X; a.prior_J = b->prior_J; a.has_prior = b->has_prior;
    a.w = v;
    a.use_active = lin_builds_active_list(b->B, b->eval_small) ? 1 : 0;
    return a;
}
static int resolve_iters(liw_ctx* c, int mode, int max_iters) {
    if (max_iters > 0) return max_iters;
    return (mode == LIW_MODE_TRACK && c->prm.fast_mode) ? 10 : 50;
}


int liw_batch_lm_begin(liw_ctx* c, const liw_batch* b, int mode, int max_iters, void* ws, void* stream) {
    NEEDDEV(c);
    if (int r = check_batch(c, b, min_frames(mode))) return r;
    c->last_iters = resolve_iters(c, mode, max_iters);
    WsView v = make_view(ws, b->B, b->n, b->history_records);
    hipStream_t s = (hipStream_t)stream;
    launch_group_offsets(b->B, b->n, b->laser_off, b->laser_frame, v.group_off, s);
    launch_lm_begin(b->B, b->n, v.lm, c->last_iters, s);
    (void)hipMemsetAsync(v.active + b->B + 1, 0, compact_list_bytes_host(b->B) - sizeof(int) * ((size_t)b->B + 1), s);
    if (b->n > 1 && b->eval_small) {
        if ((long)b->B * (b->n - 1) >= 4096 && !std::getenv("LIW_NO_IMU_PACK"))
            launch_imu_pack(b->B, b->n, b->imu_X, b->imu_J, b->imu_sqrtP, b->imu_Dt, v.imu_pk, v.imu_pk_bad, s);
        else (void)hipMemsetAsync(v.imu_pk_bad, 0xff, sizeof(int), s);
    }
    if ((long)b->B * (b->n - 1) >= 4096) {
        launch_laser_z_scan(b->Ltot, b->laser_pts, v.imu_pk_bad + 1, s);
        hipStreamCaptureStatus cap = hipStreamCaptureStatusNone;
        (void)hipStreamIsCapturing(s, &cap);
        if (int r = laser_slab_begin(c, b, mode, v, ws, s, cap == hipStreamCaptureStatusNone)) return r;
    } else {
        (void)hipMemsetAsync(v.imu_pk_bad + 1, 0xff, sizeof(int), s);
        c->lpk_on = false;
    }
    HIPCHK(c, hipGetLastError());
    return LIW_OK;
}
int liw_batch_launch_paths(liw_ctx* c, const liw_batch* b, const void* ws, int* flags) {
    if (!c) return LIW_EINVAL;
    if (int r = check_batch(c, b)) return r;
    if (!flags) return fail(c, LIW_EINVAL, "liw_batch_launch_paths: null flags");
    *flags = (pi_frame_format(b->B) ? 1 : 0) | (lpk_matches(c, b, ws) ? 2 : 0);
    return LIW_OK;
}
int liw_batch_packed_rows(liw_ctx* c, const liw_batch* b, const void* ws, long long* rows, long long* blocks) {
    if (!c) return LIW_EINVAL;
    if (int r = check_batch(c, b)) return r;
    if (rows) *rows = lpk_matches(c, b, ws) ? c->lpk_rows : 0;
    if (blocks) *blocks = (long long)b->Ltot;
    return LIW_OK;
}
int liw_batch_lm_linearize(liw_ctx* c, const liw_batch* b, int mode, int candidate, void* ws, void* stream) {
    NEEDDEV(c);
    if (int r = check_batch(c, b, min_frames(mode))) return r;
    WsView v = make_view(ws, b->B, b->n, b->history_records);
    LinArgs A = lin_args(b, mode, candidate ? v.x_cand : b->x, v, candidate != 0, true, true, c, ws);
    launch_linearize(A, c->dp, (hipStream_t)stream, c->have_fork ? &c->fork : nullptr);
    HIPCHK(c, hipGetLastError());
    return LIW_OK;
}
int liw_batch_lm_linearize_async(liw_ctx* c, const liw_batch* b, int mode, int candidate, void* ws, void* stream) {
    NEEDDEV(c);
    if (int r = check_batch(c, b, min_frames(mode))) return r;
    WsView v = make_view(ws, b->B, b->n, b->history_records);
    LinArgs A = lin_args(b, mode, candidate ? v.x_cand : b->x, v, candidate != 0, true, true, c, ws);
    launch_linearize(A, c->dp, (hipStream_t)stream, c->have_fork ? &c->fork : nullptr, true);
    HIPCHK(c, hipGetLastError());
    return LIW_OK;
}
int liw_batch_lm_join(liw_ctx* c, void* stream) {
    NEEDDEV(c);
    launch_linearize_join((hipStream_t)stream, c->have_fork ? &c->fork : nullptr);
    HIPCHK(c, hipGetLastError());
    return LIW_OK;
}
int liw_batch_exchange_doubles(int B, int n, int mode) {
    if (B <= 0 || n <= 0 || n > 64) return LIW_EINVAL;
    return B * n * (mode == LIW_MODE_INIT ? 45 : 21) + 1;
}
int liw_batch_exchange_pack(liw_ctx* c, const liw_batch* b, int mode, int candidate, void* ws, double* buf, void* stream) {
    NEEDDEV(c);
    if (int r = check_batch(c, b, min_frames(mode))) return r;
    if (!buf) return fail(c, LIW_EINVAL, "liw_batch_exchange_pack: null buffer");
    WsView v = make_view(ws, b->B, b->n, b->history_records);
    launch_exchange_pack(b->B, b->n, mode == LIW_MODE_INIT, v.pl_compact, v.PL[0], v.PL[1], candidate, mode == LIW_MODE_MARG ? nullptr : v.lm, buf, (hipStream_t)stream);
    HIPCHK(c, hipGetLastError());
    return LIW_OK;
}
int liw_batch_exchange_unpack(liw_ctx* c, const liw_batch* b, int mode, int candidate, void* ws, const double* buf, int copies, void* stream) {
    NEEDDEV(c);
    if (int r = check_batch(c, b, min_frames(mode))) return r;
    if (!buf || copies < 1) return fail(c, LIW_EINVAL, "liw_batch_exchange_unpack: null buffer / copies < 1");
    WsView v = make_view(ws, b->B, b->n, b->history_records);
    const size_t stride = (size_t)liw_batch_exchange_doubles(b->B, b->n, mode);
    launch_exchange_unpack(b->B, b->n, mode == LIW_MODE_INIT, v.pl_compact, copies, stride, buf, v.PL[0], v.PL[1], v.pi_frame ? v.CS[0] : nullptr, v.pi_frame ? v.CS[1] : nullptr, candidate, mode == LIW_MODE_MARG ? nullptr : v.lm, (hipStream_t)stream);
    HIPCHK(c, hipGetLastError());
    return LIW_OK;
}
int liw_batch_laser_records(liw_ctx* c, const liw_batch* b, int mode, int buffer, void* ws, double* out, void* stream) {
    NEEDDEV(c);
    if (int r = check_batch(c, b, min_frames(mode))) return r;
    if (!out || buffer < 0 || buffer > 1) return fail(c, LIW_EINVAL, "liw_batch_laser_records: null output / buffer not 0 or 1");
    WsView v = make_view(ws, b->B, b->n, b->history_records);
    launch_laser_expand(b->B, b->n, mode == LIW_MODE_INIT, v.pl_compact, v.PL[buffer], out, (hipStream_t)stream);
    HIPCHK(c, hipGetLastError());
    return LIW_OK;
}
static hipEvent_t next_event(std::vector<hipEvent_t>& pool, size_t& used);
int liw_batch_solve_sharded(liw_ctx* c, const liw_batch* b, int mode, int max_iters, void* ws, void* stream,
                            double* xbuf, double* xall, int world, liw_exchange_fn exchange, void* user) {
    NEEDDEV(c);
    if (int r = check_batch(c, b, min_frames(mode))) return r;
    if (mode != LIW_MODE_INIT && mode != LIW_MODE_TRACK) return fail(c, LIW_EINVAL, "liw_batch_solve_sharded: mode must be INIT or TRACK");
    const bool p2p = exchange == nullptr && c->p2p_world > 0;
    if (!xbuf || (!exchange && !p2p) || world < 1) return fail(c, LIW_EINVAL, "liw_batch_solve_sharded: exchange buffer / callback (or liw_batch_p2p_setup) / world");
    if (p2p && world != c->p2p_world) return fail(c, LIW_EINVAL, "liw_batch_solve_sharded: world differs from liw_batch_p2p_setup");
    const int K = resolve_iters(c, mode, max_iters);
    const size_t nd = (size_t)liw_batch_exchange_doubles(b->B, b->n, mode);
    hipStream_t s = (hipStream_t)stream;
    c->xev_used = 0;
    auto lin_exchange = [&](int cand) -> int {
        if (int r = liw_batch_lm_linearize_async(c, b, mode, cand, ws, stream)) return r;
        if (c->time_exchange) (void)hipEventRecord(next_event(c->ev_x, c->xev_used), s);
        if (int r = liw_batch_exchange_pack(c, b, mode, cand, ws, xbuf, stream)) return r;
        if (p2p) {
            const unsigned long long e = ++c->p2p_epoch;
            launch_p2p_exchange(nd, xbuf, c->p2p, c->p2p_rank, world, e, c->p2p_err.as<int>(), s);
            c->last_x = c->p2p.area[c->p2p_rank] + (size_t)(e & 1ull) * world * nd;
            c->last_x_copies = world;
            WsView v = make_view(ws, b->B, b->n, b->history_records);
            launch_exchange_unpack(b->B, b->n, mode == LIW_MODE_INIT, v.pl_compact, world, nd, c->last_x, v.PL[0], v.PL[1], v.pi_frame ? v.CS[0] : nullptr, v.pi_frame ? v.CS[1] : nullptr, cand, v.lm, s, true);
            HIPCHK(c, hipGetLastError());
            if (c->time_exchange) (void)hipEventRecord(next_event(c->ev_x, c->xev_used), s);
            return liw_batch_lm_join(c, stream);
        }
        const int copies = exchange(user, xbuf, xall, nd, stream);
        if (copies != 1 && !(copies == world && xall)) return fail(c, LIW_EINVAL, "liw_batch_solve_sharded: the exchange callback must return 1 (sum in buf) or world (images in all)");
        c->last_x = copies == 1 ? xbuf : xall;
        c->last_x_copies = copies;
        if (int r = liw_batch_exchange_unpack(c, b, mode, cand, ws, c->last_x, copies, stream)) return r;
        if (c->time_exchange) (void)hipEventRecord(next_event(c->ev_x, c->xev_used), s);
        return liw_batch_lm_join(c, stream);
    };
    auto p2p_failed = [&]() -> int {
        int e = 0;
        HIPCHK(c, hipMemcpyAsync(&e, c->p2p_err.p, sizeof(int), hipMemcpyDeviceToHost, s));
        HIPCHK(c, hipStreamSynchronize(s));
        if (e) return fail(c, LIW_EHIP, "peer-write exchange: a peer's flag never arrived (rank in p2p status)");
        return LIW_OK;
    };
    auto active = [&](long* out) -> int {
        double tot = 0.0;
        for (int k = 0; k < c->last_x_copies; ++k) {
            double v = 0.0;
            HIPCHK(c, hipMemcpyAsync(&v, c->last_x + (size_t)k * nd + (nd - 1), sizeof(double), hipMemcpyDeviceToHost, s));
            HIPCHK(c, hipStreamSynchronize(s));
            tot += v;
        }
        *out = (long)(tot + 0.5) / world;
        if (p2p) return p2p_failed();
        return LIW_OK;
    };
    if (int r = liw_batch_lm_begin(c, b, mode, K, ws, stream)) return r;
    if (int r = lin_exchange(0)) return r;
    int k = 0, chunk = 4;
    while (k < K) {
        const int m = std::min(chunk, K - k);
        for (int i = 0; i < m; ++i) {
            if (int r = liw_batch_lm_step(c, b, mode, ws, stream)) return r;
            if (int r = lin_exchange(1)) return r;
        }
        k += m;
        if (k < K) {
            long act = 0;
            if (int r = active(&act)) return r;
            if (act == 0) break;
        }
        chunk *= 2;
    }
    if (int r = liw_batch_lm_step(c, b, mode, ws, stream)) return r;
    if (int r = liw_batch_lm_finish(c, b, mode, ws, stream)) return r;
    if (p2p) return p2p_failed();
    return LIW_OK;
}
size_t liw_batch_p2p_area_doubles(int B, int n, int mode, int world) {
    if (world < 1 || world > P2P_MAX) return 0;
    const int nd = liw_batch_exchange_doubles(B, n, mode);
    return nd > 0 ? (size_t)2 * world * nd : 0;
}
int liw_batch_p2p_setup(liw_ctx* c, int rank, int world, double* const* areas, unsigned long long* const* flags) {
    NEEDDEV(c);
    if (world == 0) { c->p2p_world = 0; return LIW_OK; }
    if (world < 1 || world > P2P_MAX || rank < 0 || rank >= world || !areas || !flags) return fail(c, LIW_EINVAL, "liw_batch_p2p_setup: rank / world / pointers");
    for (int r = 0; r < world; ++r) {
        if (!areas[r] || !flags[r]) return fail(c, LIW_EINVAL, "liw_batch_p2p_setup: null peer pointer");
        c->p2p.area[r] = areas[r]; c->p2p.flags[r] = flags[r];
    }
    if (c->p2p_err.ensure(sizeof(int))) return fail(c, LIW_ENOMEM, "hipMalloc");
    HIPCHK(c, hipMemset(c->p2p_err.p, 0, sizeof(int)));
    unsigned long long seen[P2P_MAX] = {0}, e0 = 0;
    HIPCHK(c, hipMemcpy(seen, flags[rank], sizeof(unsigned long long) * (size_t)world, hipMemcpyDeviceToHost));
    for (int r = 0; r < world; ++r) e0 = std::max(e0, seen[r]);
    c->p2p_rank = rank; c->p2p_world = world; c->p2p_epoch = e0;
    return LIW_OK;
}
int liw_batch_p2p_status(liw_ctx* c, int* timed_out_rank_plus_1) {
    NEEDDEV(c);
    int e = 0;
    if (c->p2p_err.p) HIPCHK(c, hipMemcpy(&e, c->p2p_err.p, sizeof(int), hipMemcpyDeviceToHost));
    if (timed_out_rank_plus_1) *timed_out_rank_plus_1 = e;
    return LIW_OK;
}
int liw_batch_exchange_timing(liw_ctx* c, int enable, double* avg_ms, int* count) {
    NEEDDEV(c);
    if (avg_ms || count) {
        double tot = 0.0;
        int cnt = 0;
        for (size_t i = 0; i + 1 < c->xev_used; i += 2) {
            float ms = 0.f;
            (void)hipEventSynchronize(c->ev_x[i + 1]);
            if (hipEventElapsedTime(&ms, c->ev_x[i], c->ev_x[i + 1]) == hipSuccess) { tot += ms; ++cnt; }
        }
        if (avg_ms) *avg_ms = cnt ? tot / cnt : 0.0;
        if (count) *count = cnt;
        c->xev_used = 0;
    }
    c->time_exchange = enable != 0;
    return LIW_OK;
}
int liw_batch_lm_step(liw_ctx* c, const liw_batch* b, int mode, void* ws, void* stream) {
    NEEDDEV(c);
    if (int r = check_batch(c, b, min_frames(mode))) return r;
    WsView v = make_view(ws, b->B, b->n, b->history_records);
    StepArgs a = step_args(c, b, mode, c->last_iters, v);
    launch_lm_step(a, (hipStream_t)stream);
    HIPCHK(c, hipGetLastError());
    return LIW_OK;
}
int liw_batch_lm_finish(liw_ctx* c, const liw_batch* b, int mode, void* ws, void* stream) {
    NEEDDEV(c);
    if (int r = check_batch(c, b, min_frames(mode))) return r;
    WsView v = make_view(ws, b->B, b->n, b->history_records);
    StepArgs a = step_args(c, b, mode, c->last_iters, v);
    launch_lm_finish(a, (hipStream_t)stream);
    HIPCHK(c, hipGetLastError());
    return LIW_OK;
}
int liw_batch_set_max_iters(liw_ctx* c, int mode, int max_iters) {
    if (!c) return LIW_EINVAL;
    c->last_iters = resolve_iters(c, mode, max_iters);
    return c->last_iters;
}

static hipEvent_t next_event(std::vector<hipEvent_t>& pool, size_t& used) {
    if (used == pool.size()) { hipEvent_t e; (void)hipEventCreate(&e); pool.push_back(e); }
    return pool[used++];
}

static int enqueue_solve(liw_ctx* c, const liw_batch* b, int mode, int K, void* ws, hipStream_t s, bool timed) {
    WsView v = make_view(ws, b->B, b->n, b->history_records);
    launch_group_offsets(b->B, b->n, b->laser_off, b->laser_frame, v.group_off, s);
    launch_lm_begin(b->B, b->n, v.lm, K, s);
    (void)hipMemsetAsync(v.active + b->B + 1, 0, compact_list_bytes_host(b->B) - sizeof(int) * ((size_t)b->B + 1), s);
    const bool pack = b->n > 1 && b->eval_small && !std::getenv("LIW_NO_IMU_PACK") && (long)b->B * (b->n - 1) >= 4096;
    if (pack) launch_imu_pack(b->B, b->n, b->imu_X, b->imu_J, b->imu_sqrtP, b->imu_Dt, v.imu_pk, v.imu_pk_bad, s);
    if (pack) launch_laser_z_scan(b->Ltot, b->laser_pts, v.imu_pk_bad + 1, s);
    c->lpk_on = false;
    if (pack) {
        hipStreamCaptureStatus cap = hipStreamCaptureStatusNone;
        (void)hipStreamIsCapturing(s, &cap);
        if (int r = laser_slab_begin(c, b, mode, v, ws, s, cap == hipStreamCaptureStatusNone)) return r;
    }
    StepArgs st = step_args(c, b, mode, K, v);
    auto lin = [&](int cand) {
        LinArgs A = lin_args(b, mode, cand ? v.x_cand : b->x, v, cand, true, pack, c, ws);
        if (timed) (void)hipEventRecord(next_event(c->ev_lin, c->ev_lin_used), s);
        launch_linearize(A, c->dp, s, c->have_fork ? &c->fork : nullptr);
        if (timed) (void)hipEventRecord(next_event(c->ev_lin, c->ev_lin_used), s);
    };
    auto step = [&]() {
        if (timed) (void)hipEventRecord(next_event(c->ev_step, c->ev_step_used), s);
        launch_lm_step(st, s);
        if (timed) (void)hipEventRecord(next_event(c->ev_step, c->ev_step_used), s);
    };
    lin(0);
    hipStreamCaptureStatus capst = hipStreamCaptureStatusNone;
    (void)hipStreamIsCapturing(s, &capst);
    const bool no_exit = std::getenv("LIW_NO_EARLY_EXIT") != nullptr;
    const bool can_exit = capst == hipStreamCaptureStatusNone && !no_exit && lin_builds_active_list(b->B, b->eval_small);
    int next_check = can_exit ? 3 : K + 1;
    for (int k = 0; k < K; ++k) {
        step();
        lin(1);
        if (k + 1 == next_check && k + 1 < K) {
            if (!c->rb_pin) HIPCHK(c, hipHostMalloc((void**)&c->rb_pin, 64, hipHostMallocDefault));
            int* const act = c->rb_pin;
            act[0] = -1; act[1] = 0;
            HIPCHK(c, hipMemcpyAsync(act, v.active, sizeof(int), hipMemcpyDeviceToHost, s));
            HIPCHK(c, hipMemcpyAsync(act + 1, v.active + b->B + 2, sizeof(int), hipMemcpyDeviceToHost, s));
            HIPCHK(c, hipStreamSynchronize(s));
            if (act[1] != 1 || act[0] < 0 || act[0] > b->B) { next_check = K + 1; continue; }
            if (act[0] == 0) break;
            next_check += act[0] > b->B / 4 ? (mode == LIW_MODE_TRACK ? 3 : 8) : (act[0] > b->B / 64 ? 3 : 2);
        }
    }
    step();
    launch_lm_finish(st, s);
    return LIW_OK;
}

int liw_batch_solve(liw_ctx* c, const liw_batch* b, int mode, int max_iters, void* ws, void* stream, int use_graph) {
    NEEDDEV(c);
    if (int r = check_batch(c, b, min_frames(mode))) return r;
    if (mode != LIW_MODE_INIT && mode != LIW_MODE_TRACK) return fail(c, LIW_EINVAL, "liw_batch_solve: mode must be INIT or TRACK");
    const int K = resolve_iters(c, mode, max_iters);
    c->last_iters = K;
    hipStream_t s = (hipStream_t)stream;
    if (use_graph && !c->timing) {
        std::vector<unsigned char> key(sizeof(liw_batch) + sizeof(int) * 2 + sizeof(void*));
        std::memcpy(key.data(), b, sizeof(liw_batch));
        std::memcpy(key.data() + sizeof(liw_batch), &mode, sizeof(int));
        std::memcpy(key.data() + sizeof(liw_batch) + sizeof(int), &K, sizeof(int));
        std::memcpy(key.data() + sizeof(liw_batch) + 2 * sizeof(int), &ws, sizeof(void*));
        if (!c->gexec || key != c->gkey) {
            if (c->gexec) { (void)hipGraphExecDestroy(c->gexec); c->gexec = nullptr; }
            hipGraph_t g = nullptr;
            HIPCHK(c, hipStreamBeginCapture(s, hipStreamCaptureModeThreadLocal));
            enqueue_solve(c, b, mode, K, ws, s, false);
            HIPCHK(c, hipStreamEndCapture(s, &g));
            HIPCHK(c, hipGraphInstantiate(&c->gexec, g, nullptr, nullptr, 0));
            (void)hipGraphDestroy(g);
            c->gkey = key;
        }
        c->lpk_on = false;
        HIPCHK(c, hipGraphLaunch(c->gexec, s));
        return LIW_OK;
    }
    if (int r = enqueue_solve(c, b, mode, K, ws, s, c->timing)) return r;
    HIPCHK(c, hipGetLastError());
    return LIW_OK;
}

int liw_batch_marg_linearize(liw_ctx* c, const liw_batch* b, void* ws, void* stream) {
    NEEDDEV(c);
    if (int r = check_batch(c, b, 2)) return r;
    WsView v = make_view(ws, b->B, b->n, b->history_records);
    hipStream_t s = (hipStream_t)stream;
    launch_group_offsets(b->B, b->n, b->laser_off, b->laser_frame, v.group_off, s);
    LinArgs A = lin_args(b, LIW_MODE_MARG, b->x, v, 0, false);
    if (lpk_matches(c, b, ws)) { A.laser_pk = c->lpk.as<double>(); A.laser_slab_off = c->lpk_off.as<long long>(); A.laser_perm = c->lpk_perm.as<int>(); }
    if (c->timing) (void)hipEventRecord(next_event(c->ev_lin, c->ev_lin_used), s);
    launch_linearize(A, c->dp, s, c->have_fork ? &c->fork : nullptr);
    if (c->timing) (void)hipEventRecord(next_event(c->ev_lin, c->ev_lin_used), s);
    HIPCHK(c, hipGetLastError());
    return LIW_OK;
}
int liw_batch_marg_schur(liw_ctx* c, const liw_batch* b, void* ws, double* sqrt_H, double* Delta_H, double* Delta_g, void* stream) {
    NEEDDEV(c);
    if (int r = check_batch(c, b, 2)) return r;
    if (c->prm.fast_mode) return LIW_OK;
    WsView v = make_view(ws, b->B, b->n, b->history_records);
    MargArgs a{};
    a.B = b->B; a.n = b->n; a.x = b->x;
    a.prior_X = b->prior_X; a.prior_J = b->prior_J; a.prior_R = b->prior_R; a.has_prior = b->has_prior;
    a.w = v; a.sqrt_H = sqrt_H; a.Delta_H = Delta_H; a.Delta_g = Delta_g; a.status = nullptr;
    launch_marg_schur(a, (hipStream_t)stream);
    HIPCHK(c, hipGetLastError());
    return LIW_OK;
}
int liw_batch_export_dense(liw_ctx* c, const liw_batch* b, int mode, int buf, void* ws, double* H, double* g, double* cost, void* stream) {
    NEEDDEV(c);
    if (int r = check_batch(c, b, min_frames(mode))) return r;
    WsView v = make_view(ws, b->B, b->n, b->history_records);
    ExportArgs a{};
    a.B = b->B; a.n = b->n; a.mode = mode; a.fast_mode = c->prm.fast_mode; a.buf = buf;
    a.x = b->x; a.prior_X = b->prior_X; a.prior_J = b->prior_J; a.has_prior = b->has_prior;
    a.w = v; a.H = H; a.g = g; a.cost = cost;
    launch_export_dense(a, (hipStream_t)stream);
    HIPCHK(c, hipGetLastError());
    return LIW_OK;
}
int liw_batch_linearize(liw_ctx* c, const liw_batch* b, int mode, void* ws, void* stream) {
    NEEDDEV(c);
    if (int r = check_batch(c, b, min_frames(mode))) return r;
    WsView v = make_view(ws, b->B, b->n, b->history_records);
    hipStream_t s = (hipStream_t)stream;
    launch_group_offsets(b->B, b->n, b->laser_off, b->laser_frame, v.group_off, s);
    LinArgs A = lin_args(b, mode, b->x, v, 0, false);
    if (c->timing) (void)hipEventRecord(next_event(c->ev_lin, c->ev_lin_used), s);
    launch_linearize(A, c->dp, s, c->have_fork ? &c->fork : nullptr);
    if (c->timing) (void)hipEventRecord(next_event(c->ev_lin, c->ev_lin_used), s);
    HIPCHK(c, hipGetLastError());
    return LIW_OK;
}

int liw_batch_time_kernels(liw_ctx* c, const liw_batch* b, int mode, void* ws, void* stream, int reps, double* out_ms) {
    NEEDDEV(c);
    if (int r = check_batch(c, b, 2)) return r;
    if (mode != LIW_MODE_INIT && mode != LIW_MODE_TRACK) return fail(c, LIW_EINVAL, "liw_batch_time_kernels: mode must be INIT or TRACK");
    if (!out_ms || reps < 1) return fail(c, LIW_EINVAL, "liw_batch_time_kernels: out / reps");
    hipStream_t s = (hipStream_t)stream;
    WsView v = make_view(ws, b->B, b->n, b->history_records);
    const int K = resolve_iters(c, mode, 0);
    if (int r = liw_batch_lm_begin(c, b, mode, K, ws, stream)) return r;
    const bool packed = true;
    auto lin = [&](int cand, int mask) {
        LinArgs A = lin_args(b, mode, cand ? v.x_cand : b->x, v, cand, true, packed, c, ws);
        A.role_mask = mask;
        launch_linearize(A, c->dp, s, nullptr);
    };
    StepArgs st = step_args(c, b, mode, K, v);
    lin(0, 0);
    launch_lm_step(st, s);
    lin(1, 0);
    struct EventPool {
        std::vector<hipEvent_t> v;
        ~EventPool() { for (auto e : v) if (e) (void)hipEventDestroy(e); }
        hipEvent_t& operator[](size_t i) { return v[i]; }
    } ev;
    ev.v.assign((size_t)reps * 5 + 4, nullptr);
    for (auto& e : ev.v) HIPCHK(c, hipEventCreate(&e));
    for (int r = 0; r < reps; ++r) {
        hipEvent_t* e = &ev[(size_t)r * 5];
        lin(1, 8);
        (void)hipEventRecord(e[0], s); lin(1, 1);
        if (getenv("LIW_KT_IMU_TWICE")) lin(1, 2);
        (void)hipEventRecord(e[1], s); lin(1, 2);
        (void)hipEventRecord(e[2], s); lin(1, 4);
        (void)hipEventRecord(e[3], s); launch_lm_step(st, s);
        (void)hipEventRecord(e[4], s);
    }
    hipEvent_t* m = &ev[(size_t)reps * 5];
    {
        launch_group_offsets(b->B, b->n, b->laser_off, b->laser_frame, v.group_off, s);
        LinArgs A = lin_args(b, LIW_MODE_MARG, b->x, v, 0, false);
        if (lpk_matches(c, b, ws)) { A.laser_pk = c->lpk.as<double>(); A.laser_slab_off = c->lpk_off.as<long long>(); A.laser_perm = c->lpk_perm.as<int>(); }
        A.role_mask = 6;
        launch_linearize(A, c->dp, s, nullptr);
        (void)hipEventRecord(m[0], s);
        A.role_mask = 1;
        launch_linearize(A, c->dp, s, nullptr);
        (void)hipEventRecord(m[1], s);
    }
    if (!c->prm.fast_mode) {
        DevBuf tmp;
        if (tmp.ensure(sizeof(double) * (size_t)b->B * (36 + 225 + 15))) return fail(c, LIW_ENOMEM, "hipMalloc");
        DevBuf pX, pJ, pR, pH;
        if (pX.ensure(sizeof(double) * 15 * b->B) || pJ.ensure(sizeof(double) * 225 * b->B) || pR.ensure(sizeof(double) * 15 * b->B) || pH.ensure(sizeof(int) * b->B))
            return fail(c, LIW_ENOMEM, "hipMalloc");
        MargArgs a{};
        a.B = b->B; a.n = b->n; a.x = b->x;
        a.prior_X = b->prior_X; a.prior_J = b->prior_J; a.prior_R = b->prior_R; a.has_prior = b->has_prior;
        a.out_X = pX.as<double>(); a.out_J = pJ.as<double>(); a.out_R = pR.as<double>(); a.out_has = pH.as<int>();
        a.w = v; a.sqrt_H = tmp.as<double>(); a.Delta_H = a.sqrt_H + (size_t)36 * b->B; a.Delta_g = a.Delta_H + (size_t)225 * b->B; a.status = nullptr;
        (void)hipEventRecord(m[2], s);
        launch_marg_schur(a, s);
        (void)hipEventRecord(m[3], s);
        HIPCHK(c, hipStreamSynchronize(s));
        tmp.release(); pX.release(); pJ.release(); pR.release(); pH.release();
    } else {
        (void)hipEventRecord(m[2], s); (void)hipEventRecord(m[3], s);
    }
    HIPCHK(c, hipStreamSynchronize(s));
    for (int k = 0; k < 6; ++k) out_ms[k] = 0.0;
    for (int r = 0; r < reps; ++r)
        for (int k = 0; k < 4; ++k) {
            float f = 0.f;
            (void)hipEventElapsedTime(&f, ev[(size_t)r * 5 + k], ev[(size_t)r * 5 + k + 1]);
            out_ms[k] += f / reps;
        }
    float f = 0.f;
    (void)hipEventElapsedTime(&f, m[2], m[3]); out_ms[4] = f;
    (void)hipEventElapsedTime(&f, m[0], m[1]); out_ms[5] = f;
    HIPCHK(c, hipGetLastError());
    return LIW_OK;
}

static PreintNoise preint_noise(const liw_params& prm) {
    PreintNoise N{};
    for (int k = 0; k < 3; ++k) {
        N.q_na[k] = prm.imu_noise_acc_sigma[k] * prm.imu_noise_acc_sigma[k];
        N.q_nw[k] = prm.imu_noise_gyro_sigma[k] * prm.imu_noise_gyro_sigma[k];
        N.q_nba[k] = prm.imu_bias_acc_sigma[k] * prm.imu_bias_acc_sigma[k];
        N.q_nbw[k] = prm.imu_bias_gyro_sigma[k] * prm.imu_bias_gyro_sigma[k];
        N.wheel_cov[k] = prm.wheel_sigma[k] * prm.wheel_sigma[k];
    }
    return N;
}
int liw_batch_imu_preint(liw_ctx* c, int M, const int* sample_off, const double* samples, const double* t_start, const double* t_end,
                         const double* bias6, double* X, double* J, double* P_scratch, double* sqrt_inverse_P, double* Dt, void* stream) {
    NEEDDEV(c);
    if (M < 0 || (M > 0 && (!sample_off || !samples || !t_start || !t_end || !bias6 || !X || !J || !P_scratch || !sqrt_inverse_P || !Dt)))
        return fail(c, LIW_EINVAL, "liw_batch_imu_preint: null argument");
    if (M == 0) return LIW_OK;
    launch_preint_imu(M, sample_off, samples, t_start, t_end, bias6, preint_noise(c->prm), X, J, P_scratch, sqrt_inverse_P, Dt, (hipStream_t)stream);
    HIPCHK(c, hipGetLastError());
    return LIW_OK;
}
int liw_batch_wheel_preint(liw_ctx* c, int M, const int* sample_off, const double* samples, const double* t_start, const double* t_end,
                           double* delta_Tij, double* sqrt_inverse_P, double* Dt, void* stream) {
    NEEDDEV(c);
    if (M < 0 || (M > 0 && (!sample_off || !samples || !t_start || !t_end || !delta_Tij || !sqrt_inverse_P || !Dt)))
        return fail(c, LIW_EINVAL, "liw_batch_wheel_preint: null argument");
    if (M == 0) return LIW_OK;
    launch_preint_wheel(M, sample_off, samples, t_start, t_end, preint_noise(c->prm), delta_Tij, sqrt_inverse_P, Dt, (hipStream_t)stream);
    HIPCHK(c, hipGetLastError());
    return LIW_OK;
}

int liw_set_timing(liw_ctx* c, int enable) {
    if (!c) return LIW_EINVAL;
    c->timing = enable != 0;
    c->ev_lin_used = c->ev_step_used = 0;
    return LIW_OK;
}
int liw_get_timing(liw_ctx* c, double* lin_ms, int* lin_n, double* step_ms, int* step_n) {
    NEEDDEV(c);
    auto total = [&](std::vector<hipEvent_t>& pool, size_t used, double* ms, int* cnt) {
        double t = 0.0; int k = 0;
        for (size_t i = 0; i + 1 < used; i += 2) {
            float f = 0.f;
            if (hipEventSynchronize(pool[i + 1]) != hipSuccess) continue;
            if (hipEventElapsedTime(&f, pool[i], pool[i + 1]) == hipSuccess) { t += f; ++k; }
        }
        if (ms) *ms = k ? t / k : 0.0;
        if (cnt) *cnt = k;
    };
    total(c->ev_lin, c->ev_lin_used, lin_ms, lin_n);
    total(c->ev_step, c->ev_step_used, step_ms, step_n);
    c->ev_lin_used = c->ev_step_used = 0;
    return LIW_OK;
}

int liw_set_window(liw_ctx* c, const liw_window* w) {
    NEEDDEV(c);
    if (!w || w->n < 1 || w->n > 64 || w->L < 0) return fail(c, LIW_EINVAL, "liw_set_window: need 1 <= n <= 64, L >= 0");
    if (!w->states || !w->match_pose || !w->has_match) return fail(c, LIW_EINVAL, "liw_set_window: states / match_pose / has_match are NULL");
    if (w->L > 0 && (!w->laser_frame || !w->laser_pts)) return fail(c, LIW_EINVAL, "liw_set_window: L > 0 but laser_frame / laser_pts are NULL");
    if (w->n > 1 && (!w->imu_X || !w->imu_J || !w->imu_sqrtP || !w->imu_Dt || !w->wheel_T || !w->wheel_sqrtP))
        return fail(c, LIW_EINVAL, "liw_set_window: n > 1 but an IMU / wheel array is NULL");
    HIPCHK(c, hipSetDevice(c->prm.device));
    const int n = w->n, L = w->L;
    for (int j = 1; j < L; ++j) if (w->laser_frame[j] < w->laser_frame[j - 1]) return fail(c, LIW_EINVAL, "laser_frame must be ascending");
    for (int j = 0; j < L; ++j) if (w->laser_frame[j] < 0 || w->laser_frame[j] >= n) return fail(c, LIW_EINVAL, "laser_frame out of range");
    struct Part { const void* src; size_t bytes; };
    int off2[2] = {0, L};
    int goff[65];
    for (int i = 0, j = 0; i <= n; ++i) { while (j < L && w->laser_frame[j] < i) ++j; goff[i] = j; }
    const Part parts[13] = {
        {w->states, sizeof(double) * n * 15}, {off2, sizeof(off2)}, {w->laser_frame, sizeof(int) * (size_t)L},
        {nullptr, sizeof(double) * 12 * (size_t)L},
        {w->match_pose, sizeof(double) * n * 12}, {w->has_match, (size_t)n},
        {w->imu_X, sizeof(double) * (n - 1) * 15}, {w->imu_J, sizeof(double) * (n - 1) * 225},
        {w->imu_sqrtP, sizeof(double) * (n - 1) * 225}, {w->imu_Dt, sizeof(double) * (n - 1)},
        {w->wheel_T, sizeof(double) * (n - 1) * 12}, {w->wheel_sqrtP, sizeof(double) * (n - 1) * 9},
        {goff, sizeof(int) * (size_t)(n + 1)},
    };
    size_t off[13], tot = 0;
    for (int k = 0; k < 13; ++k) { off[k] = tot; tot = al256(tot + (parts[k].bytes ? parts[k].bytes : 8)); }
    const size_t readback = al256(sizeof(double) * (LIW_RESULT_HDR + (size_t)n * 27 + 276));
    if (c->img_cap < tot || c->readback_cap < readback) {
        (void)hipStreamSynchronize(c->stream);
        if (c->pinned) (void)hipHostFree(c->pinned);
        c->pinned = nullptr; c->img_cap = c->readback_cap = c->pinned_cap = 0; c->img_valid = false;
        const size_t ic = std::max(tot * 2, (size_t)65536), rc = std::max(readback * 2, (size_t)8192);
        if (hipHostMalloc(&c->pinned, 2 * ic + rc, hipHostMallocDefault) != hipSuccess) return fail(c, LIW_ENOMEM, "hipHostMalloc");
        c->img_cap = ic; c->readback_cap = rc; c->pinned_cap = 2 * ic + rc;
        std::memset((char*)c->pinned + 2 * ic, 0, rc);
    }
    const int stage_id = c->img_valid ? 1 - c->img_cur : 0;
    char* stage = (char*)c->pinned + (size_t)stage_id * c->img_cap;
    if (c->ev_upload) (void)hipEventSynchronize(c->ev_upload);
    for (int k = 0; k < 13; ++k) {
        if (k == 3) {
            double* soa = (double*)(stage + off[k]);
            for (int j = 0; j < L; ++j) for (int q = 0; q < 12; ++q) soa[(size_t)q * L + j] = w->laser_pts[(size_t)j * 12 + q];
        } else if (parts[k].bytes) {
            std::memcpy(stage + off[k], parts[k].src, parts[k].bytes);
        }
    }
    bool same = c->reattach && c->img_valid && c->n == n && c->L == L;
    if (same) {
        const char* cur = (const char*)c->pinned + (size_t)c->img_cur * c->img_cap;
        for (int k = 0; k < 13 && same; ++k)
            if (parts[k].bytes && std::memcmp(stage + off[k], cur + off[k], parts[k].bytes) != 0) same = false;
    }
    if (same) { c->hw = *w; c->have_window = true; return LIW_OK; }
    c->solved_records = 0;
    c->spec_valid = false;
    c->have_window = false;
    if (c->arena.ensure(tot)) return fail(c, LIW_ENOMEM, "hipMalloc");
    HIPCHK(c, hipMemcpyAsync(c->arena.p, stage, tot, hipMemcpyHostToDevice, c->stream));
    if (c->ev_upload) HIPCHK(c, hipEventRecord(c->ev_upload, c->stream));
    c->img_valid = false;
    for (int k = 0; k < 13; ++k) { c->part_off[k] = off[k]; c->part_bytes[k] = parts[k].bytes; }
    char* dev = (char*)c->arena.p;
    bool fresh_prior = c->prior_X.p == nullptr;
    if (c->prior_X.ensure(sizeof(double) * 15) || c->prior_J.ensure(sizeof(double) * 225) || c->prior_R.ensure(sizeof(double) * 15) ||
        c->has_prior.ensure(sizeof(int)) || c->priorn_X.ensure(sizeof(double) * 15) || c->priorn_J.ensure(sizeof(double) * 225) ||
        c->priorn_R.ensure(sizeof(double) * 15) || c->has_priorn.ensure(sizeof(int)) || c->marg_status.ensure(sizeof(int)) ||
        c->result.ensure(sizeof(double) * (LIW_RESULT_HDR + (size_t)n * 27 + 276)))
        return fail(c, LIW_ENOMEM, "hipMalloc");
    if (fresh_prior) {
        HIPCHK(c, hipMemsetAsync(c->prior_X.p, 0, sizeof(double) * 15, c->stream));
        HIPCHK(c, hipMemsetAsync(c->prior_J.p, 0, sizeof(double) * 225, c->stream));
        HIPCHK(c, hipMemsetAsync(c->prior_R.p, 0, sizeof(double) * 15, c->stream));
        HIPCHK(c, hipMemsetAsync(c->has_prior.p, 0, sizeof(int), c->stream));
    }
    c->hist_records = 64;
    FullLayout f = full_layout(1, n, c->hist_records);
    if (c->ws.ensure(f.bytes)) return fail(c, LIW_ENOMEM, "hipMalloc workspace");
    c->hw = *w; c->have_window = true; c->n = n; c->L = L;
    c->img_cur = stage_id; c->img_valid = true;
    liw_batch& b = c->sb;
    b.B = 1; b.n = n; b.Ltot = L;
    b.x = (double*)(dev + off[0]); b.laser_off = (int*)(dev + off[1]); b.laser_frame = (int*)(dev + off[2]);
    b.laser_pts = (double*)(dev + off[3]); b.match_pose = (double*)(dev + off[4]); b.has_match = (unsigned char*)(dev + off[5]);
    b.imu_X = (double*)(dev + off[6]); b.imu_J = (double*)(dev + off[7]); b.imu_sqrtP = (double*)(dev + off[8]);
    b.imu_Dt = (double*)(dev + off[9]); b.wheel_T = (double*)(dev + off[10]); b.wheel_sqrtP = (double*)(dev + off[11]);
    b.prior_X = c->prior_X.as<double>(); b.prior_J = c->prior_J.as<double>(); b.prior_R = c->prior_R.as<double>(); b.has_prior = c->has_prior.as<int>();
    b.eval_small = 1; b.history_records = c->hist_records;
    return LIW_OK;
}
int liw_clear_window(liw_ctx* c) {
    if (!c) return LIW_EINVAL;
    c->have_window = false;
    c->hw = liw_window{};
    c->solved_records = 0;
    return LIW_OK;
}
#define NEEDWIN(c)                                                                          \
    do {                                                                                    \
        NEEDDEV(c);                                                                         \
        if (!(c)->have_window) return fail((c), LIW_ESTATE, "liw_set_window was not called"); \
        HIPCHK(c, hipSetDevice((c)->prm.device));                                           \
    } while (0)

int liw_solve(liw_ctx* c, int mode, int max_iters, liw_summary* summary) {
    NEEDWIN(c);
    if (mode != LIW_MODE_INIT && mode != LIW_MODE_TRACK) return fail(c, LIW_EINVAL, "liw_solve: mode must be LIW_MODE_INIT or LIW_MODE_TRACK");
    if (c->n < min_frames(mode)) return fail(c, LIW_EINVAL, "liw_solve: TRACK topology needs n >= 2");
    if (mode == LIW_MODE_INIT && c->L > 0 && c->hw.laser_frame[0] == 0 && c->hw.has_match[0])
        return fail(c, LIW_EINVAL, "init topology: frame 0 must not own laser blocks (duplicate parameter blocks)");
    int K = resolve_iters(c, mode, max_iters);
    c->solved_records = 0;
    c->spec_valid = false;
    if (K + 1 > c->hist_records) {
        c->hist_records = K + 1;
        c->sb.history_records = c->hist_records;
        FullLayout f = full_layout(1, c->n, c->hist_records);
        if (c->ws.ensure(f.bytes)) return fail(c, LIW_ENOMEM, "hipMalloc workspace");
    }
    bool spec = c->spec_marg && mode == LIW_MODE_TRACK && !c->prm.fast_mode && c->n >= 2;
    if (spec && c->L > 0) {
        const int* lf = c->hw.laser_frame;
        const long older = std::lower_bound(lf, lf + c->L, c->n - 1) - lf, newest = (long)c->L - older;
        static const char* lim_env = std::getenv("LIW_SPEC_OLDER_MAX");
        const long lim = lim_env ? std::atol(lim_env) : 256;
        if (older > std::max(lim, 4 * newest)) spec = false;
    }
    const size_t rdoubles = LIW_RESULT_HDR + (size_t)c->n * 27 + 276;
    char* rb = (char*)c->pinned + 2 * c->img_cap;
    {
        c->last_iters = K;
        const liw_batch* b = &c->sb;
        hipStream_t s = c->stream;
        WsView v = make_view(c->ws.p, 1, c->n, b->history_records);
        v.group_off = (int*)((char*)c->arena.p + c->part_off[12]);
        StepArgs st = step_args(c, b, mode, K, v);
        bool first = true;
        auto lin = [&](int cand) {
            LinArgs A = lin_args(b, mode, cand ? v.x_cand : b->x, v, cand, !first);
            if (first) { A.reset_lm = v.lm; A.reset_iters = K; first = false; }
            A.active = nullptr;
            A.marg_older = spec ? 1 : 0;
            launch_linearize(A, c->dp, s, c->have_fork ? &c->fork : nullptr);
        };
        static const bool zero_copy = std::getenv("LIW_NO_ZEROCOPY") == nullptr;
        double* res = zero_copy ? (double*)rb : c->result.as<double>();
        double* marg_out = res + LIW_RESULT_HDR + (size_t)c->n * 27;
        PackArgs pk{};
        pk.n = c->n; pk.mode = mode; pk.lm = v.lm; pk.info = v.info; pk.x = b->x; pk.match_pose = b->match_pose; pk.has_match = b->has_match;
        pk.marg = nullptr; pk.marg_status = spec ? c->marg_status.as<int>() : nullptr; pk.out = res;
        MargArgs ma{};
        if (spec) {
            ma.B = 1; ma.n = c->n; ma.x = b->x;
            ma.prior_X = b->prior_X; ma.prior_J = b->prior_J; ma.prior_R = b->prior_R; ma.has_prior = b->has_prior;
            ma.out_X = c->priorn_X.as<double>(); ma.out_J = c->priorn_J.as<double>(); ma.out_R = c->priorn_R.as<double>(); ma.out_has = c->has_priorn.as<int>();
            ma.w = v; ma.sqrt_H = marg_out; ma.Delta_H = marg_out + 36; ma.Delta_g = marg_out + 36 + 225; ma.status = c->marg_status.as<int>();
            ma.gate = v.lm; ma.use_cur = 1;
        }
        int k = 0, chunk = 4;
        bool done = false;
        while (!done) {
            const int m = std::min(chunk, K + 1 - k);
            for (int i = 0; i < m; ++i) { lin(k + i > 0 ? 1 : 0); launch_lm_step(st, s); }
            k += m;
            if (spec) launch_marg_schur(ma, s);
            pk.seq = ++c->pack_seq;
            launch_pack_result(pk, s);
            HIPCHK(c, hipGetLastError());
            if (!zero_copy) HIPCHK(c, hipMemcpyAsync(rb, res, sizeof(double) * rdoubles, hipMemcpyDeviceToHost, s));
            static const bool poll = zero_copy && std::getenv("LIW_NO_POLL") == nullptr;
            bool seen = false;
            if (poll) {
                const volatile int* h = (const volatile int*)rb;
                const auto t0 = std::chrono::steady_clock::now();
                for (int spin = 0; !seen; ++spin) {
                    if (h[3] == pk.seq) { seen = true; break; }
                    if ((spin & 255) == 255 && std::chrono::steady_clock::now() - t0 > std::chrono::microseconds(2000)) break;
                }
                std::atomic_thread_fence(std::memory_order_acquire);
            }
            if (!seen) HIPCHK(c, hipStreamSynchronize(s));
            done = ((const int*)rb)[0] != 0;
            if (!done && k >= K + 1) return fail(c, LIW_EHIP, "liw_solve: the window did not terminate within its iteration cap");
            chunk *= 2;
        }
    }
    const int* hdr = (const int*)rb;
    const liw_summary* sp = (const liw_summary*)(rb + 16);
    const double* xs = (const double*)rb + LIW_RESULT_HDR;
    const double* mp = xs + (size_t)c->n * 15;
    std::memcpy(c->hw.states, xs, sizeof(double) * c->n * 15);
    std::memcpy(c->hw.match_pose, mp, sizeof(double) * c->n * 12);
    {
        char* img = (char*)c->pinned + (size_t)c->img_cur * c->img_cap;
        std::memcpy(img + c->part_off[0], xs, sizeof(double) * c->n * 15);
        std::memcpy(img + c->part_off[4], mp, sizeof(double) * c->n * 12);
    }
    if (spec && hdr[1] == 0) {
        std::memcpy(c->spec_out, mp + (size_t)c->n * 12, sizeof(c->spec_out));
        c->spec_valid = true;
    }
    if (summary) *summary = *sp;
    c->solved_records = std::max(0, std::min(sp->iterations + 1, c->hist_records));
    return LIW_OK;
}
int liw_get_history(liw_ctx* c, double* x, int max_records) {
    NEEDWIN(c);
    if (c->solved_records <= 0) return fail(c, LIW_ESTATE, "liw_get_history: no completed liw_solve on the current window");
    if (!x || max_records <= 0) return fail(c, LIW_EINVAL, "liw_get_history: null buffer");
    FullLayout f = full_layout(1, c->n, c->hist_records);
    int rec = c->solved_records;
    if (rec > max_records) rec = max_records;
    HIPCHK(c, hipMemcpy(x, (char*)c->ws.p + f.history, sizeof(double) * (size_t)rec * c->n * 15, hipMemcpyDeviceToHost));
    return rec;
}
int liw_linearize(liw_ctx* c, int mode, double* H, double* g, double* cost) {
    NEEDWIN(c);
    const size_t N = (size_t)15 * c->n;
    if (c->scratch.ensure(sizeof(double) * (N * N + N + 1))) return fail(c, LIW_ENOMEM, "hipMalloc");
    double* dH = c->scratch.as<double>();
    double* dg = dH + N * N;
    double* dc = dg + N;
    if (int r = liw_batch_linearize(c, &c->sb, mode, c->ws.p, c->stream)) return r;
    if (int r = liw_batch_export_dense(c, &c->sb, mode, 0, c->ws.p, dH, dg, dc, c->stream)) return r;
    if (H) HIPCHK(c, hipMemcpyAsync(H, dH, sizeof(double) * N * N, hipMemcpyDeviceToHost, c->stream));
    if (g) HIPCHK(c, hipMemcpyAsync(g, dg, sizeof(double) * N, hipMemcpyDeviceToHost, c->stream));
    if (cost) HIPCHK(c, hipMemcpyAsync(cost, dc, sizeof(double), hipMemcpyDeviceToHost, c->stream));
    HIPCHK(c, hipStreamSynchronize(c->stream));
    return LIW_OK;
}
int liw_eval_factors(liw_ctx* c, int mode, double* laser_res, double* laser_jac, double* imu_res, double* imu_jac, double* wheel_res,
                     double* wheel_jac, double* ground_res, double* ground_jac) {
    NEEDWIN(c);
    const size_t n = c->n, L = c->L, nm = n - 1;
    const size_t sz[8] = {L * 2, L * 24, nm * 15, nm * 450, nm * 3, nm * 36, n * 2, n * 12};
    size_t tot = 0;
    for (size_t v : sz) tot += v;
    if (c->scratch.ensure(sizeof(double) * (tot + 8))) return fail(c, LIW_ENOMEM, "hipMalloc");
    HIPCHK(c, hipMemsetAsync(c->scratch.p, 0, sizeof(double) * (tot + 8), c->stream));
    double* base = c->scratch.as<double>();
    double* dptr[8];
    size_t o = 0;
    for (int k = 0; k < 8; ++k) { dptr[k] = base + o; o += sz[k]; }
    WsView v = make_view(c->ws.p, 1, c->n, c->sb.history_records);
    launch_group_offsets(1, c->n, c->sb.laser_off, c->sb.laser_frame, v.group_off, c->stream);
    LinArgs A = lin_args(&c->sb, mode, c->sb.x, v, 0, false);
    A.dbg_laser_res = dptr[0]; A.dbg_laser_jac = dptr[1]; A.dbg_imu_res = dptr[2]; A.dbg_imu_jac = dptr[3];
    A.dbg_wheel_res = dptr[4]; A.dbg_wheel_jac = dptr[5]; A.dbg_ground_res = dptr[6]; A.dbg_ground_jac = dptr[7];
    launch_linearize(A, c->dp, c->stream, c->have_fork ? &c->fork : nullptr);
    HIPCHK(c, hipGetLastError());
    double* hptr[8] = {laser_res, laser_jac, imu_res, imu_jac, wheel_res, wheel_jac, ground_res, ground_jac};
    for (int k = 0; k < 8; ++k)
        if (hptr[k] && sz[k]) HIPCHK(c, hipMemcpyAsync(hptr[k], dptr[k], sizeof(double) * sz[k], hipMemcpyDeviceToHost, c->stream));
    HIPCHK(c, hipStreamSynchronize(c->stream));
    return LIW_OK;
}
int liw_marginalize(liw_ctx* c, double* sqrt_H36, double* Delta_H225, double* Delta_g15) {
    NEEDWIN(c);
    if (c->prm.fast_mode) return LIW_OK;
    if (c->n < 2) return fail(c, LIW_EINVAL, "liw_marginalize: needs n >= 2");
    if (c->spec_valid) {
        c->spec_valid = false;
        if (sqrt_H36) std::memcpy(sqrt_H36, c->spec_out, sizeof(double) * 36);
        if (Delta_H225) std::memcpy(Delta_H225, c->spec_out + 36, sizeof(double) * 225);
        if (Delta_g15) std::memcpy(Delta_g15, c->spec_out + 36 + 225, sizeof(double) * 15);
        std::swap(c->prior_X, c->priorn_X); std::swap(c->prior_J, c->priorn_J); std::swap(c->prior_R, c->priorn_R); std::swap(c->has_prior, c->has_priorn);
        c->sb.prior_X = c->prior_X.as<double>(); c->sb.prior_J = c->prior_J.as<double>();
        c->sb.prior_R = c->prior_R.as<double>(); c->sb.has_prior = c->has_prior.as<int>();
        return LIW_OK;
    }
    if (c->scratch.ensure(sizeof(double) * (36 + 225 + 15))) return fail(c, LIW_ENOMEM, "hipMalloc");
    double* d = c->scratch.as<double>();
    if (int r = liw_batch_marg_linearize(c, &c->sb, c->ws.p, c->stream)) return r;
    if (int r = liw_batch_marg_schur(c, &c->sb, c->ws.p, d, d + 36, d + 36 + 225, c->stream)) return r;
    double h[36 + 225 + 15];
    HIPCHK(c, hipMemcpyAsync(h, d, sizeof(h), hipMemcpyDeviceToHost, c->stream));
    HIPCHK(c, hipStreamSynchronize(c->stream));
    if (sqrt_H36) std::memcpy(sqrt_H36, h, sizeof(double) * 36);
    if (Delta_H225) std::memcpy(Delta_H225, h + 36, sizeof(double) * 225);
    if (Delta_g15) std::memcpy(Delta_g15, h + 36 + 225, sizeof(double) * 15);
    return LIW_OK;
}
int liw_get_prior(liw_ctx* c, double* X15, double* J225, double* R15) {
    NEEDDEV(c);
    if (!c->prior_X.p) return 0;
    int has = 0;
    HIPCHK(c, hipMemcpy(&has, c->has_prior.p, sizeof(int), hipMemcpyDeviceToHost));
    if (!has) return 0;
    if (X15) HIPCHK(c, hipMemcpy(X15, c->prior_X.p, sizeof(double) * 15, hipMemcpyDeviceToHost));
    if (J225) HIPCHK(c, hipMemcpy(J225, c->prior_J.p, sizeof(double) * 225, hipMemcpyDeviceToHost));
    if (R15) HIPCHK(c, hipMemcpy(R15, c->prior_R.p, sizeof(double) * 15, hipMemcpyDeviceToHost));
    return 1;
}
int liw_set_prior(liw_ctx* c, int has_prior, const double* X15, const double* J225, const double* R15) {
    if (c) c->spec_valid = false;
    NEEDDEV(c);
    HIPCHK(c, hipSetDevice(c->prm.device));
    if (c->prior_X.ensure(sizeof(double) * 15) || c->prior_J.ensure(sizeof(double) * 225) || c->prior_R.ensure(sizeof(double) * 15) ||
        c->has_prior.ensure(sizeof(int)))
        return fail(c, LIW_ENOMEM, "hipMalloc");
    int has = has_prior ? 1 : 0;
    HIPCHK(c, hipMemcpy(c->has_prior.p, &has, sizeof(int), hipMemcpyHostToDevice));
    if (has) {
        if (!X15 || !J225) return fail(c, LIW_EINVAL, "liw_set_prior: X and J required");
        double z[15] = {0};
        HIPCHK(c, hipMemcpy(c->prior_X.p, X15, sizeof(double) * 15, hipMemcpyHostToDevice));
        HIPCHK(c, hipMemcpy(c->prior_J.p, J225, sizeof(double) * 225, hipMemcpyHostToDevice));
        HIPCHK(c, hipMemcpy(c->prior_R.p, R15 ? R15 : z, sizeof(double) * 15, hipMemcpyHostToDevice));
    }
    if (c->have_window) {
        c->sb.prior_X = c->prior_X.as<double>(); c->sb.prior_J = c->prior_J.as<double>();
        c->sb.prior_R = c->prior_R.as<double>(); c->sb.has_prior = c->has_prior.as<int>();
    }
    return LIW_OK;
}

}
```

### 2dliw-slam_amd/csrc/liw_kernels.hpp

```cpp
#pragma once
#include <cstdlib>
#include <hip/hip_runtime.h>
#include <stdint.h>

#include "../../include/liw_window.h"
#include "liw_dual.hpp"
#include "liw_lm_rules.hpp"

namespace liw {

struct DevParams {
    double Riw[9], tiw[3];
    double Ril[9], til[3];
    double g;
    double laser_sqrt_info;
    double ground_p_info;
    double ground_q_info;
    int fast_mode;
};

constexpr int LP = LIW_LASER_PARTIAL;
constexpr int PIS = 496;
constexpr int PI_II = 0, PI_IJ = 120, PI_JJ = 345, PI_G = 465, PI_C = 495;
__host__ __device__ inline int pi_tri(int r, int c) {
    const int lo = r < c ? r : c, hi = r < c ? c : r;
    return lo * 15 - (lo * (lo - 1)) / 2 + (hi - lo);
}
constexpr int PIF_D = 0, PIF_IJ = 120, PIF_GJ = 345, PIF_GI = 360, PIF_C = 375, PIFS = 376;
constexpr int QUAD_MIN_BATCH = 1024;
enum StepVariant { STEP_AUTO = -1, STEP_LATENCY = 0, STEP_THROUGHPUT = 1, STEP_TWO_WAVE = 2, STEP_QUAD = 3, STEP_DENSE2 = 4 };
inline StepVariant forced_step_variant() {
    const char* env = getenv("LIW_STEP_VARIANT");
    if (!env) return STEP_AUTO;
    return env[0] >= '1' && env[0] <= '4' ? (StepVariant)(env[0] - '0') : STEP_LATENCY;
}
inline bool step_variant_is(StepVariant forced, StepVariant v, bool by_size) { return forced == STEP_AUTO ? by_size : forced == v; }
inline bool pi_frame_format(int B, StepVariant forced = forced_step_variant()) { return step_variant_is(forced, STEP_QUAD, B >= QUAD_MIN_BATCH); }
__host__ __device__ inline size_t pi_doubles_per_window(int n) {
    const size_t a = (size_t)(n > 1 ? n - 1 : 1) * PIS, b = (size_t)n * PIFS;
    return a > b ? a : b;
}
template <int N> __host__ __device__ constexpr int tri_sym(int r, int c) {
    return r <= c ? r * N - (r * (r - 1)) / 2 + (c - r) : c * N - (c * (c - 1)) / 2 + (r - c);
}
constexpr int CS_LASER = 0, CS_GROUND = 1, CS_IMU = 2, CS_WHEEL = 3;
__host__ __device__ inline size_t cs_index(int n, int b, int role, int rec) { return ((size_t)b * 4 + role) * n + rec; }
constexpr int PWS = 92;
__host__ __device__ constexpr int PW_II(int r, int c) { return tri_sym<6>(r, c); }
__host__ __device__ constexpr int PW_IJ(int r, int c) { return 21 + r * 6 + c; }
__host__ __device__ constexpr int PW_JJ(int r, int c) { return 57 + tri_sym<6>(r, c); }
__host__ __device__ constexpr int PW_G(int e) { return 78 + e; }
constexpr int PW_C = 90;
constexpr int PGS = 28;
__host__ __device__ constexpr int PG_H(int r, int c) { return tri_sym<7>(r, c); }
__host__ __device__ constexpr int PG_G(int r) { return tri_sym<7>(r, 6); }
constexpr int PG_C = 27;
constexpr int FTF = 32;

struct LmState {
    double radius, decrease_factor, x_cost, x_norm, minimum_cost;
    double cand_step_norm, model_cost_change;
    int reuse_diagonal, iteration, done, termination, successful, cur, invalid_steps, have_candidate;
    int max_iters, pad_;
    double initial_cost;
    double scale[15 * 64];
    double diagonal[15 * 64];
    double x0[15 * 64];
};

__device__ __forceinline__ void lm_reset(LmState& s, int max_iters) {
    s.radius = kInitRadius; s.decrease_factor = 2.0; s.x_cost = 0.0; s.x_norm = 0.0; s.minimum_cost = 0.0;
    s.cand_step_norm = 0.0; s.model_cost_change = 0.0; s.reuse_diagonal = 0; s.iteration = 0; s.done = 0; s.termination = 0;
    s.successful = 0; s.cur = 0; s.invalid_steps = 0; s.have_candidate = 0; s.initial_cost = 0.0; s.max_iters = max_iters; s.pad_ = 0;
}

struct WsView {
    double* PL[2]; double* PI[2]; double* PW[2]; double* PG[2];
    double* x_cand;
    int* group_off;
    LmState* lm;
    double* solve_ws;
    liw_summary* info;
    double* history;
    int history_records;
    int* active;
    int pi_frame;
    int pl_compact;
    double* CS[2];
    double* imu_pk;
    int* imu_pk_bad;
};
constexpr int IMU_PK = 192, IPK_DT = 15, IPK_J = 16, IPK_S = 70;
constexpr int REC_LD = 22;
constexpr int REC_GS = 15 * REC_LD;
constexpr int SOLVE_WS = REC_GS + 16;

struct LinArgs {
    int B, n, mode, eval_small;
    const double* x;
    const int* group_off;
    const int* laser_off;
    const double* laser_pts; int Ltot;
    const double* match_pose;
    const unsigned char* has_match;
    const double* imu_X; const double* imu_J; const double* imu_sqrtP; const double* imu_Dt;
    const double* wheel_T; const double* wheel_sqrtP;
    double* PL[2]; double* PI[2]; double* PW[2]; double* PG[2];
    const LmState* lm;
    const LmState* gate;
    LmState* reset_lm;
    int reset_iters;
    int marg_older;
    int candidate;
    int small_per_wave;
    int imu_per_wave;
    int small_nd;
    int* active;
    int pi_frame;
    int pl_compact;
    double* CS[2];
    const double* imu_pk;
    const int* imu_pk_bad;
    const int* laser_hz;
    const double* laser_pk;
    const long long* laser_slab_off;
    const int* laser_perm;
    int role_mask;
    double* dbg_laser_res; double* dbg_laser_jac; double* dbg_imu_res; double* dbg_imu_jac;
    double* dbg_wheel_res; double* dbg_wheel_jac; double* dbg_ground_res; double* dbg_ground_jac;
};

template <bool BOTH> constexpr int laser_pairidx(int c1, int c2) {
    constexpr int NC = BOTH ? 9 : 6;
    return c1 > c2 ? laser_pairidx<BOTH>(c2, c1) : c1 * NC - c1 * (c1 - 1) / 2 + (c2 - c1);
}
constexpr int laser_col_a(int idx) { return idx < 2 ? idx : (idx == 2 ? -1 : idx - 1); }
template <bool BOTH> constexpr int laser_col_b(int idx) { return BOTH ? (idx < 2 ? idx : (idx == 2 ? -1 : idx + 2)) : (idx == 2 ? -1 : (idx < 2 ? idx : idx - 1)); }
template <bool BOTH> constexpr bool laser_neg_b(int idx) { return BOTH && idx < 2; }
template <bool BOTH>
__host__ __device__ constexpr int laser_slot_code(int s) {
    constexpr int RC = (BOTH ? 9 : 6) - 1;
    int src = -1;
    bool neg = false;
    if (s < 0) {
    } else if (s < 36) {
        const int ca = laser_col_a(s / 6), cb = laser_col_a(s % 6);
        if (BOTH && ca >= 0 && cb >= 0) src = laser_pairidx<BOTH>(ca, cb);
    } else if (s < 72) {
        const int ia = (s - 36) / 6, ib = (s - 36) % 6, ca = laser_col_b<BOTH>(ia), cb = laser_col_b<BOTH>(ib);
        if (ca >= 0 && cb >= 0) { src = laser_pairidx<BOTH>(ca, cb); neg = laser_neg_b<BOTH>(ia) != laser_neg_b<BOTH>(ib); }
    } else if (s < 108) {
        const int ia = (s - 72) / 6, ib = (s - 72) % 6, ca = laser_col_a(ia), cb = laser_col_b<BOTH>(ib);
        if (BOTH && ca >= 0 && cb >= 0) { src = laser_pairidx<BOTH>(ca, cb); neg = laser_neg_b<BOTH>(ib); }
    } else if (s < 114) {
        const int ca = laser_col_a(s - 108);
        if (BOTH && ca >= 0) src = laser_pairidx<BOTH>(ca, RC);
    } else if (s < 120) {
        const int cb = laser_col_b<BOTH>(s - 114);
        if (cb >= 0) { src = laser_pairidx<BOTH>(cb, RC); neg = laser_neg_b<BOTH>(s - 114); }
    } else if (s == 120) {
        src = laser_pairidx<BOTH>(RC, RC);
    }
    return src < 0 ? -1 : (src | (neg ? 64 : 0));
}
template <bool BOTH> __host__ __device__ constexpr bool laser_slot_zero(int s) { return laser_slot_code<BOTH>(s) < 0; }
constexpr int LPC = LIW_LASER_PARTIAL_COMPACT;
__host__ __device__ constexpr int laser_stride(int compact) { return compact ? LPC : LP; }
constexpr int LPC_COST_BOTH = laser_pairidx<true>(8, 8), LPC_COST_ONE = laser_pairidx<false>(5, 5);
static_assert(laser_slot_code<true>(120) == LPC_COST_BOTH && laser_slot_code<false>(120) == LPC_COST_ONE && LPC_COST_BOTH == 44 && LPC_COST_ONE == 20, "cost total");
template <bool BOTH> __host__ __device__ inline double laser_slot(const double* rec, int s, int compact) {
    if (!compact) return rec[s];
    const int code = laser_slot_code<BOTH>(s);
    if (code < 0) return 0.0;
    const double v = rec[code & 63];
    return (code & 64) ? -v : v;
}
__host__ __device__ inline double laser_slot(const double* rec, int s, int compact, bool both) {
    return both ? laser_slot<true>(rec, s, compact) : laser_slot<false>(rec, s, compact);
}
struct LaserPackTable { short slot[45]; unsigned char neg[45]; };

__device__ __forceinline__ void lds_sync() {
    __builtin_amdgcn_fence(__ATOMIC_RELEASE, "wavefront");
    __builtin_amdgcn_wave_barrier();
    __builtin_amdgcn_fence(__ATOMIC_ACQUIRE, "wavefront");
}
__device__ __forceinline__ void wave_mem_sync() {
    __builtin_amdgcn_fence(__ATOMIC_RELEASE, "workgroup");
    __builtin_amdgcn_wave_barrier();
    __builtin_amdgcn_fence(__ATOMIC_ACQUIRE, "workgroup");
}

template <typename T> __device__ __forceinline__ void nt_store(T* p, T v) { __builtin_nontemporal_store(v, p); }

__device__ __forceinline__ double fast_rsqrt(double x) {
    double y = __builtin_amdgcn_rsq(x);
    const double hx = 0.5 * x;
    y = y * __builtin_fma(-hx, y * y, 1.5);
    y = y * __builtin_fma(-hx, y * y, 1.5);
    return y;
}
__device__ __forceinline__ double fast_rcp(double x) {
    double y = __builtin_amdgcn_rcp(x);
    y = __builtin_fma(__builtin_fma(-x, y, 1.0), y, y);
    y = __builtin_fma(__builtin_fma(-x, y, 1.0), y, y);
    return y;
}

__device__ __forceinline__ const int* usable_active_list(const int* active, int B) {
    if (!active) return nullptr;
    const int st = __builtin_amdgcn_readfirstlane(active[B + 2]);
    const int cnt = __builtin_amdgcn_readfirstlane(active[0]);
    return (st == 1 && cnt >= 0 && cnt <= B) ? active : nullptr;
}
__device__ __forceinline__ double touch_lines(const void* p, size_t bytes) {
    const int lane = threadIdx.x & 63;
    const size_t a0 = (size_t)p & ~(size_t)127, last = ((size_t)p + bytes - 8) & ~(size_t)127;
    const size_t q = a0 + 128 * (size_t)lane;
    return *reinterpret_cast<const double*>(q < last ? q : last);
}

__device__ __forceinline__ bool window_live(const LinArgs& A, int b) {
    if (A.gate) return A.gate[b].done != 0;
    if (A.lm) return A.lm[b].done == 0;
    return true;
}

struct LinFork {
    hipStream_t side[2];
    hipEvent_t ev_fork, ev_join[2], ev_compact;
};


struct StepArgs {
    int B, n, mode, max_iters, fast_mode;
    double* x;
    double* match_pose;
    const unsigned char* has_match;
    const double* prior_X; const double* prior_J; const int* has_prior;
    WsView w;
    int only_slow;
    int use_active;
};
struct ExportArgs {
    int B, n, mode, fast_mode, buf;
    const double* x; const double* prior_X; const double* prior_J; const int* has_prior;
    WsView w;
    double* H; double* g; double* cost;
};
struct MargArgs {
    int B, n;
    const double* x; double* prior_X; double* prior_J; double* prior_R; int* has_prior;
    WsView w;
    double* sqrt_H; double* Delta_H; double* Delta_g; int* status;
    double* out_X; double* out_J; double* out_R; int* out_has;
    const LmState* gate;
    int use_cur;
};
constexpr int LIW_RESULT_HDR = 8;
struct PackArgs {
    int n, mode;
    const LmState* lm; liw_summary* info; const double* x; double* match_pose; const unsigned char* has_match;
    const double* marg; const int* marg_status;
    double* out;
    int seq;
};
void launch_linearize(const LinArgs& A, const DevParams& P, hipStream_t s, const LinFork* fk, bool defer_join = false);
void launch_linearize_join(hipStream_t s, const LinFork* fk);
void launch_exchange_pack(int B, int n, bool both, int compact, const double* PL0, const double* PL1, int candidate, const LmState* lm, double* buf, hipStream_t s);
void launch_exchange_unpack(int B, int n, bool both, int compact, int world, size_t stride, const double* buf, double* PL0, double* PL1, double* CS0, double* CS1, int candidate, const LmState* lm, hipStream_t s, bool sysload = false);
constexpr int P2P_MAX = 16;
struct P2pPeers { double* area[P2P_MAX]; unsigned long long* flags[P2P_MAX]; };
void launch_p2p_exchange(size_t nd, const double* buf, const P2pPeers& peers, int rank, int world, unsigned long long epoch, int* err, hipStream_t s);
void launch_group_offsets(int B, int n, const int* laser_off, const int* laser_frame, int* group_off, hipStream_t s);
void launch_laser_z_scan(long Ltot, const double* laser_pts, int* flag, hipStream_t s);
__host__ __device__ inline int laser_slab_count(int B) { return (B + 63) / 64; }
void launch_laser_slab_prepare(int B, int n, const int* group_off, int* perm, int* mx, long long* off, const int* hz, hipStream_t s);
constexpr int LASER_SLAB_ROWD = 8 * 64;
void launch_laser_slab_pack(int B, int n, long Ltot, const int* group_off, const int* perm, const double* pts, const long long* off, const int* mx, double* pk, hipStream_t s);
void launch_lin_laser_slab(const LinArgs& A, const DevParams& P, hipStream_t s);
void launch_imu_pack(int B, int n, const double* imu_X, const double* imu_J, const double* imu_sqrtP, const double* imu_Dt, double* pk, int* bad, hipStream_t s);
void launch_pack_result(const PackArgs& a, hipStream_t s);
void launch_lm_begin(int B, int n, LmState* lm, int max_iters, hipStream_t s);
void launch_lm_step(const StepArgs& a, hipStream_t s);
void launch_lm_step_quad(const StepArgs& a, hipStream_t s);
bool lm_step_quad_fits(const StepArgs& a);
size_t compact_list_bytes_host(int B);
bool lin_builds_active_list(int B, int eval_small);
void launch_lm_finish(const StepArgs& a, hipStream_t s);
void launch_export_dense(const ExportArgs& a, hipStream_t s);
void launch_laser_expand(int B, int n, bool both, int compact, const double* PL, double* out, hipStream_t s);
void launch_marg_schur(const MargArgs& a, hipStream_t s);

struct PreintNoise { double q_na[3], q_nw[3], q_nba[3], q_nbw[3], wheel_cov[3]; };
void launch_preint_imu(int M, const int* sample_off, const double* samples, const double* t_start, const double* t_end, const double* bias6,
                       const PreintNoise& N, double* X, double* J, double* Pscratch, double* sqrtP, double* Dt, hipStream_t s);
void launch_preint_wheel(int M, const int* sample_off, const double* samples, const double* t_start, const double* t_end,
                         const PreintNoise& N, double* T12, double* sq9, double* Dt, hipStream_t s);

}
```

### include/liw_window.h

```cpp
#ifndef LIW_WINDOW_H
#define LIW_WINDOW_H
#include <stddef.h>
#include <stdint.h>

#ifdef __cplusplus
extern "C" {
#endif

#define LIW_OK 0
#define LIW_EINVAL (-22)
#define LIW_ENOMEM (-12)
#define LIW_ENODEV (-19)
#define LIW_EHIP (-5)
#define LIW_ESTATE (-1)

enum { LIW_MODE_INIT = 0, LIW_MODE_TRACK = 1, LIW_MODE_MARG = 2 };

typedef struct liw_params {
    double T_imu_to_wheel[16];
    double T_imu_to_laser[16];
    double g;
    double line_to_line_sigma;
    double manifold_p_sigma, manifold_q_sigma;
    double imu_noise_acc_sigma[3], imu_bias_acc_sigma[3], imu_noise_gyro_sigma[3], imu_bias_gyro_sigma[3];
    double wheel_sigma[3];
    int fast_mode;
    int normalize_extrinsics;
    int device;
} liw_params;

typedef struct liw_window {
    int n;
    int L;
    double* states;
    const int* laser_frame;
    const double* laser_pts;
    double* match_pose;
    const unsigned char* has_match;
    const double* imu_X;
    const double* imu_J;
    const double* imu_sqrtP;
    const double* imu_Dt;
    const double* wheel_T;
    const double* wheel_sqrtP;
    const double* wheel_Dt;
} liw_window;

typedef struct liw_summary {
    int iterations;
    int successful_steps;
    int termination;
    double initial_cost, final_cost;
} liw_summary;

typedef struct liw_ctx liw_ctx;

liw_ctx* liw_create(const liw_params* prm);
void liw_destroy(liw_ctx* ctx);
const char* liw_last_error(const liw_ctx* ctx);
int liw_get_extrinsics(const liw_ctx* ctx, double* T_imu_to_wheel16, double* T_imu_to_laser16);

int liw_set_window(liw_ctx* ctx, const liw_window* w);
int liw_clear_window(liw_ctx* ctx);
int liw_solve(liw_ctx* ctx, int mode, int max_iters, liw_summary* summary);
int liw_get_history(liw_ctx* ctx, double* x, int max_records);
int liw_linearize(liw_ctx* ctx, int mode, double* H, double* g, double* cost);
int liw_eval_factors(liw_ctx* ctx, int mode, double* laser_res, double* laser_jac, double* imu_res, double* imu_jac,
                     double* wheel_res, double* wheel_jac, double* ground_res, double* ground_jac);
int liw_marginalize(liw_ctx* ctx, double* sqrt_H36, double* Delta_H225, double* Delta_g15);
int liw_get_prior(liw_ctx* ctx, double* X15, double* J225, double* R15);
int liw_set_prior(liw_ctx* ctx, int has_prior, const double* X15, const double* J225, const double* R15);

typedef struct liw_batch {
    int B;
    int n;
    int Ltot;
    double* x;
    const int* laser_off;
    const int* laser_frame;
    const double* laser_pts;
    double* match_pose;
    const unsigned char* has_match;
    const double* imu_X;
    const double* imu_J;
    const double* imu_sqrtP;
    const double* imu_Dt;
    const double* wheel_T;
    const double* wheel_sqrtP;
    double* prior_X;
    double* prior_J;
    double* prior_R;
    int* has_prior;
    int eval_small;
    int history_records;
} liw_batch;

typedef struct liw_ws_layout {
    size_t bytes;
    size_t laser_partial_off[2];
    size_t laser_partial_bytes;
    size_t info_off;
    size_t history_off;
    int laser_partial_stride;
} liw_ws_layout;
#define LIW_LASER_PARTIAL 128
#define LIW_LASER_PARTIAL_COMPACT 48
int liw_batch_ws_layout(int B, int n, int history_records, liw_ws_layout* out);

int liw_batch_set_max_iters(liw_ctx* ctx, int mode, int max_iters);
int liw_batch_linearize(liw_ctx* ctx, const liw_batch* b, int mode, void* ws, void* stream);
int liw_batch_time_kernels(liw_ctx* ctx, const liw_batch* b, int mode, void* ws, void* stream, int reps, double* out_ms);
int liw_batch_lm_begin(liw_ctx* ctx, const liw_batch* b, int mode, int max_iters, void* ws, void* stream);
int liw_batch_launch_paths(liw_ctx* ctx, const liw_batch* b, const void* ws, int* flags);
int liw_batch_packed_rows(liw_ctx* ctx, const liw_batch* b, const void* ws, long long* rows, long long* blocks);
int liw_batch_lm_linearize(liw_ctx* ctx, const liw_batch* b, int mode, int candidate, void* ws, void* stream);
int liw_batch_laser_records(liw_ctx* ctx, const liw_batch* b, int mode, int buffer, void* ws, double* out, void* stream);
int liw_batch_lm_step(liw_ctx* ctx, const liw_batch* b, int mode, void* ws, void* stream);
int liw_batch_lm_finish(liw_ctx* ctx, const liw_batch* b, int mode, void* ws, void* stream);
int liw_batch_lm_linearize_async(liw_ctx* ctx, const liw_batch* b, int mode, int candidate, void* ws, void* stream);
int liw_batch_lm_join(liw_ctx* ctx, void* stream);
typedef int (*liw_exchange_fn)(void* user, double* buf, double* all, size_t doubles, void* stream);
int liw_batch_solve_sharded(liw_ctx* ctx, const liw_batch* b, int mode, int max_iters, void* ws, void* stream,
                            double* xbuf, double* xall, int world, liw_exchange_fn exchange, void* user);
size_t liw_batch_p2p_area_doubles(int B, int n, int mode, int world);
int liw_batch_p2p_setup(liw_ctx* ctx, int rank, int world, double* const* areas, unsigned long long* const* flags);
int liw_batch_p2p_status(liw_ctx* ctx, int* timed_out_rank_plus_1);
int liw_batch_exchange_timing(liw_ctx* ctx, int enable, double* avg_ms, int* count);
int liw_batch_exchange_doubles(int B, int n, int mode);
int liw_batch_exchange_pack(liw_ctx* ctx, const liw_batch* b, int mode, int candidate, void* ws, double* buf, void* stream);
int liw_batch_exchange_unpack(liw_ctx* ctx, const liw_batch* b, int mode, int candidate, void* ws, const double* buf, int copies, void* stream);
int liw_batch_solve(liw_ctx* ctx, const liw_batch* b, int mode, int max_iters, void* ws, void* stream, int use_graph);
int liw_batch_marg_linearize(liw_ctx* ctx, const liw_batch* b, void* ws, void* stream);
int liw_batch_marg_schur(liw_ctx* ctx, const liw_batch* b, void* ws, double* sqrt_H, double* Delta_H, double* Delta_g, void* stream);
int liw_batch_export_dense(liw_ctx* ctx, const liw_batch* b, int mode, int buf, void* ws, double* H, double* g, double* cost, void* stream);
int liw_set_timing(liw_ctx* ctx, int enable);
int liw_get_timing(liw_ctx* ctx, double* linearize_ms_avg, int* linearize_launches, double* step_ms_avg, int* step_launches);

int liw_batch_imu_preint(liw_ctx* ctx, int M, const int* sample_off, const double* samples, const double* t_start, const double* t_end,
                         const double* bias6, double* X, double* J, double* P_scratch, double* sqrt_inverse_P, double* Dt, void* stream);
int liw_batch_wheel_preint(liw_ctx* ctx, int M, const int* sample_off, const double* samples, const double* t_start, const double* t_end,
                           double* delta_Tij, double* sqrt_inverse_P, double* Dt, void* stream);

typedef struct liw_imu_preint liw_imu_preint;
liw_imu_preint* liw_imu_preint_create(const liw_params* prm);
void liw_imu_preint_destroy(liw_imu_preint* p);
void liw_imu_preint_reset(liw_imu_preint* p, double time, const double* acc_bias3, const double* gyr_bias3);
int liw_imu_preint_add(liw_imu_preint* p, double time_stamp, const double* acc3, const double* gyro3);
void liw_imu_preint_update_only_t(liw_imu_preint* p, double time);
double liw_imu_preint_Dt(const liw_imu_preint* p);
void liw_imu_preint_result(const liw_imu_preint* p, double* X15, double* J225, double* sqrt_inverse_P225, double* Dt);

typedef struct liw_wheel_preint liw_wheel_preint;
liw_wheel_preint* liw_wheel_preint_create(const liw_params* prm);
void liw_wheel_preint_destroy(liw_wheel_preint* p);
void liw_wheel_preint_reset(liw_wheel_preint* p, double time);
int liw_wheel_preint_add(liw_wheel_preint* p, double time_stamp, const double* pose_R9, const double* pose_t3);
void liw_wheel_preint_update_only_t(liw_wheel_preint* p, double time);
void liw_wheel_preint_result(const liw_wheel_preint* p, double* T12, double* sqrt_inverse_P9, double* Dt);

#ifdef __cplusplus
}
#endif
#endif
```

Baseline: 141,100 solves/s.

## Repack laser slabs to only live windows during LM early-exit

When the LM loop's periodic active-window check shows that fewer windows remain unconverged, the laser slab layout is rebuilt over only the live windows. The linearize kernel then launches over fewer slabs, which avoids launching blocks for converged windows. A cost model decides whether a repack pays off, weighing the slab launches saved over the remaining iterations against the repack cost. The repack adds host syncs and extra prepare and pack kernels, plus a stats API, and clamps per-slab counts to the packed max.

```diff
diff --git a/2dliw-slam_amd/__init__.py b/2dliw-slam_amd/__init__.py
--- a/2dliw-slam_amd/__init__.py
+++ b/2dliw-slam_amd/__init__.py
@@ -59,7 +59,7 @@
 EXPORTS = [
     "liw_create", "liw_destroy", "liw_last_error", "liw_get_extrinsics", "liw_set_window", "liw_clear_window", "liw_solve", "liw_get_history",
     "liw_linearize", "liw_eval_factors", "liw_marginalize", "liw_get_prior", "liw_set_prior", "liw_batch_ws_layout",
-    "liw_batch_set_max_iters", "liw_batch_launch_paths", "liw_batch_packed_rows", "liw_batch_linearize", "liw_batch_time_kernels", "liw_batch_lm_begin", "liw_batch_lm_linearize", "liw_batch_laser_records", "liw_batch_lm_step",
+    "liw_batch_set_max_iters", "liw_batch_launch_paths", "liw_batch_packed_rows", "liw_batch_repack_stats", "liw_batch_linearize", "liw_batch_time_kernels", "liw_batch_lm_begin", "liw_batch_lm_linearize", "liw_batch_laser_records", "liw_batch_lm_step",
     "liw_batch_lm_finish", "liw_batch_lm_linearize_async", "liw_batch_lm_join", "liw_batch_exchange_doubles", "liw_batch_exchange_pack",
     "liw_batch_exchange_unpack", "liw_batch_solve_sharded", "liw_batch_exchange_timing", "liw_batch_p2p_area_doubles", "liw_batch_p2p_setup", "liw_batch_p2p_status", "liw_batch_solve", "liw_batch_marg_linearize", "liw_batch_marg_schur", "liw_batch_export_dense",
     "liw_set_timing", "liw_get_timing", "liw_batch_imu_preint", "liw_batch_wheel_preint", "liw_imu_preint_create", "liw_imu_preint_destroy", "liw_imu_preint_reset",
diff --git a/2dliw-slam_amd/batch.py b/2dliw-slam_amd/batch.py
--- a/2dliw-slam_amd/batch.py
+++ b/2dliw-slam_amd/batch.py
@@ -278,6 +278,11 @@
         return dict(flags=flags.value, large_batch_format=bool(flags.value & 1), lane_per_group_laser=bool(flags.value & 2), packed_rows=rows.value,
                     blocks=blocks.value, padding_ratio=(64.0 * rows.value / blocks.value) if (rows.value and blocks.value) else None)
 
+    def repack_stats(self):
+        g, r0, r1 = C.c_int(0), C.c_longlong(0), C.c_longlong(0)
+        self._chk(self.L.liw_batch_repack_stats(self.h, C.byref(g), C.byref(r0), C.byref(r1)))
+        return dict(generations=g.value, rows_first=r0.value, rows_last=r1.value)
+
     def solve(self, mode, max_iters=0, use_graph=False):
         self._pl_mode = int(mode)
         if not self.sharded:
diff --git a/2dliw-slam_amd/csrc/k_laser_slab.hip b/2dliw-slam_amd/csrc/k_laser_slab.hip
--- a/2dliw-slam_amd/csrc/k_laser_slab.hip
+++ b/2dliw-slam_amd/csrc/k_laser_slab.hip
@@ -140,6 +140,8 @@
     const int g0 = A.group_off[bb * (n + 1) + f], g1 = A.group_off[bb * (n + 1) + f + 1];
     const int hm = A.has_match[bb * n + f];
     const int curv = A.lm ? A.lm[bb].cur : 0;
+    const int mxp = A.laser_mx[(size_t)s * n + f];
+
     double pa6[6], pb6[6];
 #pragma unroll
     for (int k = 0; k < 6; ++k) {
@@ -149,7 +151,7 @@
     if (in) in = window_live(A, bb);
     if (!__any(in)) return;
     const bool fon = in && hm != 0 && (BOTH || A.mode != LIW_MODE_TRACK || f == n - 1 || A.marg_older);
-    const int cnt = fon ? g1 - g0 : 0;
+    const int cnt = fon ? min(g1 - g0, mxp) : 0;
     int maxc = cnt;
 #pragma unroll
     for (int o = 32; o > 0; o >>= 1) maxc = max(maxc, __shfl_xor(maxc, o, 64));
@@ -414,15 +416,18 @@
 __global__ __launch_bounds__(64, 2) void k_lin_laser_slab1(LinArgs A, DevParams P) { slab_item<false>(A, P, (int)blockIdx.x); }
 
 constexpr int SORT_BINS = 4096;
-__global__ __launch_bounds__(1024) void k_laser_slab_order(int B, int n, const int* group_off, int* perm) {
+__global__ __launch_bounds__(1024) void k_laser_slab_order(int B, int n, const int* group_off, const LmState* lm, const int* list, int cand, int* perm, int* taken) {
     __shared__ int bin[SORT_BINS];
     __shared__ int part[1024];
     const int f = (int)blockIdx.x, t = (int)threadIdx.x;
     const size_t Bp = (size_t)((B + SLAB - 1) / SLAB) * SLAB;
     for (int e = t; e < SORT_BINS; e += 1024) bin[e] = 0;
     __syncthreads();
-    auto key = [&](int b) { return SORT_BINS - 1 - min(group_off[b * (n + 1) + f + 1] - group_off[b * (n + 1) + f], SORT_BINS - 1); };
-    for (int b = t; b < B; b += 1024) atomicAdd(&bin[key(b)], 1);
+    auto key = [&](int b) { return SORT_BINS - 1 - min(max(group_off[b * (n + 1) + f + 1] - group_off[b * (n + 1) + f], 0), SORT_BINS - 1); };
+    auto take = [&](int b) { return !lm || lm[b].done == 0; };
+    auto window = [&](int i) { const int b = list ? list[i] : i; return (b >= 0 && b < B) ? b : -1; };
+    if (!list) cand = B;
+    for (int i = t; i < cand; i += 1024) { const int b = window(i); if (b >= 0 && take(b)) atomicAdd(&bin[key(b)], 1); }
     __syncthreads();
     int sum = 0;
 #pragma unroll
@@ -439,16 +444,17 @@
 #pragma unroll
     for (int k = 0; k < SORT_BINS / 1024; ++k) { const int h = bin[t * (SORT_BINS / 1024) + k]; bin[t * (SORT_BINS / 1024) + k] = base; base += h; }
     __syncthreads();
-    for (int b = t; b < B; b += 1024) perm[(size_t)f * Bp + atomicAdd(&bin[key(b)], 1)] = b;
-    for (size_t e = (size_t)B + t; e < Bp; e += 1024) perm[(size_t)f * Bp + e] = -1;
-}
-__global__ void k_laser_slab_max(int B, int n, const int* group_off, const int* perm, int* mx) {
+    for (int i = t; i < cand; i += 1024) { const int b = window(i); if (b >= 0 && take(b)) perm[(size_t)f * Bp + atomicAdd(&bin[key(b)], 1)] = b; }
+    for (size_t e = (size_t)part[1023] + t; e < Bp; e += 1024) perm[(size_t)f * Bp + e] = -1;
+    if (taken && f == 0 && t == 0) *taken = part[1023];
+}
+__global__ void k_laser_slab_max(int B, int n, int slabs, int f_lo, const int* group_off, const int* perm, int* mx) {
     const int t = blockIdx.x * blockDim.x + threadIdx.x;
     const int S = (B + SLAB - 1) / SLAB;
-    if (t >= S * n) return;
+    if (t >= slabs * n) return;
     const int s = t / n, f = t % n;
     int m = 0;
-    for (int l = 0; l < SLAB; ++l) {
+    for (int l = 0; l < SLAB && f >= f_lo; ++l) {
         const int b = perm[(size_t)f * ((size_t)S * SLAB) + (size_t)s * SLAB + l];
         if (b >= 0) m = max(m, group_off[b * (n + 1) + f + 1] - group_off[b * (n + 1) + f]);
     }
@@ -513,16 +519,23 @@
 void launch_laser_slab_prepare(int B, int n, const int* group_off, int* perm, int* mx, long long* off, const int* hz, hipStream_t s) {
     const int N = laser_slab_count(B) * n;
     if (std::getenv("LIW_SLAB_BATCH_ORDER")) hipLaunchKernelGGL(k_laser_slab_identity, dim3((unsigned)(((size_t)N * SLAB + 255) / 256)), dim3(256), 0, s, B, n, perm);
-    else hipLaunchKernelGGL(k_laser_slab_order, dim3((unsigned)n), dim3(1024), 0, s, B, n, group_off, perm);
-    hipLaunchKernelGGL(k_laser_slab_max, dim3((N + 255) / 256), dim3(256), 0, s, B, n, group_off, (const int*)perm, mx);
+    else hipLaunchKernelGGL(k_laser_slab_order, dim3((unsigned)n), dim3(1024), 0, s, B, n, group_off, (const LmState*)nullptr, (const int*)nullptr, B, perm, (int*)nullptr);
+    hipLaunchKernelGGL(k_laser_slab_max, dim3((N + 255) / 256), dim3(256), 0, s, B, n, laser_slab_count(B), 0, group_off, (const int*)perm, mx);
     hipLaunchKernelGGL(k_laser_slab_scan, dim3(1), dim3(1024), 0, s, N, (const int*)mx, off, hz);
 }
-void launch_laser_slab_pack(int B, int n, long Ltot, const int* group_off, const int* perm, const double* pts, const long long* off, const int* mx, double* pk, hipStream_t s) {
-    hipLaunchKernelGGL(k_laser_slab_pack, dim3((unsigned)(laser_slab_count(B) * n)), dim3(256), 0, s, B, n, Ltot, group_off, perm, pts, off, mx, pk);
+void launch_laser_slab_prepare_live(int B, int n, int slabs, int f_lo, const int* group_off, const LmState* lm, const int* list, int cand, int* perm, int* mx, long long* off, int* taken, hipStream_t s) {
+    const int N = slabs * n;
+    hipLaunchKernelGGL(k_laser_slab_order, dim3((unsigned)n), dim3(1024), 0, s, B, n, group_off, lm, list, cand < B ? cand : B, perm, taken);
+    hipLaunchKernelGGL(k_laser_slab_max, dim3((N + 255) / 256), dim3(256), 0, s, B, n, slabs, f_lo, group_off, (const int*)perm, mx);
+    hipLaunchKernelGGL(k_laser_slab_scan, dim3(1), dim3(1024), 0, s, N, (const int*)mx, off, (const int*)taken);
+}
+void launch_laser_slab_pack(int B, int n, int slabs, long Ltot, const int* group_off, const int* perm, const double* pts, const long long* off, const int* mx, double* pk, hipStream_t s) {
+    hipLaunchKernelGGL(k_laser_slab_pack, dim3((unsigned)(slabs * n)), dim3(256), 0, s, B, n, Ltot, group_off, perm, pts, off, mx, pk);
 }
 void launch_lin_laser_slab(const LinArgs& A, const DevParams& P, hipStream_t s) {
-    if (A.mode == LIW_MODE_INIT) hipLaunchKernelGGL(k_lin_laser_slab, dim3((unsigned)(laser_slab_count(A.B) * A.n)), dim3(64), 0, s, A, P);
-    else hipLaunchKernelGGL(k_lin_laser_slab1, dim3((unsigned)(laser_slab_count(A.B) * A.n)), dim3(64), 0, s, A, P);
-}
-
-}
+    const int slabs = A.laser_slabs > 0 ? min(A.laser_slabs, laser_slab_count(A.B)) : laser_slab_count(A.B);
+    if (A.mode == LIW_MODE_INIT) hipLaunchKernelGGL(k_lin_laser_slab, dim3((unsigned)(slabs * A.n)), dim3(64), 0, s, A, P);
+    else hipLaunchKernelGGL(k_lin_laser_slab1, dim3((unsigned)(slabs * A.n)), dim3(64), 0, s, A, P);
+}
+
+}
diff --git a/2dliw-slam_amd/csrc/liw_capi.hip b/2dliw-slam_amd/csrc/liw_capi.hip
--- a/2dliw-slam_amd/csrc/liw_capi.hip
+++ b/2dliw-slam_amd/csrc/liw_capi.hip
@@ -72,6 +72,10 @@
     struct { const void* ws; const void* pts; const void* frame; int B, n; long Ltot; } lpk_key{};
     bool lpk_on = false;
     long long lpk_rows = 0;
+    DevBuf lpk2, lpk2_off, lpk2_mx, lpk2_perm;
+    int lpk2_slabs = 0;
+    int lpk_gens = 0;
+    long long lpk_last_rows = 0;
     int* rb_pin = nullptr;
     hipGraphExec_t gexec = nullptr;
     std::vector<unsigned char> gkey;
@@ -179,7 +183,7 @@
     if (!c) return;
     if (c->have_device) {
         (void)hipSetDevice(c->prm.device);
-        DevBuf* bufs[] = {&c->lpk, &c->lpk_off, &c->lpk_mx, &c->lpk_perm, &c->p2p_err, &c->arena, &c->prior_X, &c->prior_J, &c->prior_R, &c->has_prior, &c->ws, &c->scratch,
+        DevBuf* bufs[] = {&c->lpk, &c->lpk_off, &c->lpk_mx, &c->lpk_perm, &c->lpk2, &c->lpk2_off, &c->lpk2_mx, &c->lpk2_perm, &c->p2p_err, &c->arena, &c->prior_X, &c->prior_J, &c->prior_R, &c->has_prior, &c->ws, &c->scratch,
                           &c->priorn_X, &c->priorn_J, &c->priorn_R, &c->has_priorn, &c->result, &c->marg_status};
         if (c->pinned) (void)hipHostFree(c->pinned);
         if (c->rb_pin) (void)hipHostFree(c->rb_pin);
@@ -287,6 +291,7 @@
 }
 static int laser_slab_begin(liw_ctx* c, const liw_batch* b, int mode, const WsView& v, void* ws, hipStream_t s, bool may_sync) {
     c->lpk_on = false;
+    c->lpk2_slabs = 0; c->lpk_gens = 0; c->lpk_last_rows = 0;
     if (!may_sync || std::getenv("LIW_NO_LASER_SLAB")) return LIW_OK;
     const int S = laser_slab_count(b->B), N = S * b->n;
     if ((mode == LIW_MODE_INIT ? N < 2048 : S < 256) || b->Ltot <= 0) return LIW_OK;
@@ -302,11 +307,40 @@
     if (tail[1] != 0 || rows <= 0) return LIW_OK;
     if (rows * 64 > 4 * (long long)b->Ltot + 64ll * N) return LIW_OK;
     if (c->lpk.ensure(sizeof(double) * LASER_SLAB_ROWD * (size_t)rows)) { c->lpk.release(); return LIW_OK; }
-    launch_laser_slab_pack(b->B, b->n, (long)b->Ltot, v.group_off, c->lpk_perm.as<int>(), b->laser_pts, c->lpk_off.as<long long>(), c->lpk_mx.as<int>(), c->lpk.as<double>(), s);
+    launch_laser_slab_pack(b->B, b->n, S, (long)b->Ltot, v.group_off, c->lpk_perm.as<int>(), b->laser_pts, c->lpk_off.as<long long>(), c->lpk_mx.as<int>(), c->lpk.as<double>(), s);
     c->lpk_key = {ws, b->laser_pts, b->laser_frame, b->B, b->n, (long)b->Ltot};
     c->lpk_on = true;
     c->lpk_rows = rows;
-    return LIW_OK;
+    c->lpk_gens = 1; c->lpk_last_rows = rows;
+    return LIW_OK;
+}
+static int laser_slab_repack(liw_ctx* c, const liw_batch* b, int mode, const WsView& v, int live, hipStream_t s, bool* packed) {
+    *packed = false;
+    c->lpk2_slabs = 0;
+    const int S = laser_slab_count(b->B), slabs = laser_slab_count(live), N = slabs * b->n;
+    if (live <= 0 || live > b->B) return LIW_OK;
+    if (c->lpk2_mx.ensure(sizeof(int) * ((size_t)S * b->n + 1)) || c->lpk2_off.ensure(sizeof(long long) * ((size_t)S * b->n + 2)) ||
+        c->lpk2_perm.ensure(sizeof(int) * (size_t)S * b->n * 64))
+        return LIW_OK;
+    int* const taken = c->lpk2_mx.as<int>() + (size_t)S * b->n;
+    const int f_lo = mode == LIW_MODE_TRACK ? b->n - 1 : 0;
+    launch_laser_slab_prepare_live(b->B, b->n, slabs, f_lo, v.group_off, v.lm, v.active + 1, live, c->lpk2_perm.as<int>(), c->lpk2_mx.as<int>(), c->lpk2_off.as<long long>(), taken, s);
+    long long* const tail = reinterpret_cast<long long*>(c->rb_pin) + 2;
+    tail[0] = -1; tail[1] = -1;
+    HIPCHK(c, hipMemcpyAsync(tail, c->lpk2_off.as<long long>() + N, 2 * sizeof(long long), hipMemcpyDeviceToHost, s));
+    HIPCHK(c, hipStreamSynchronize(s));
+    const long long rows = tail[0];
+    if (tail[1] != (long long)live || rows <= 0 || rows > c->lpk_rows) return LIW_OK;
+    if (c->lpk2.ensure(sizeof(double) * LASER_SLAB_ROWD * (size_t)rows)) { c->lpk2.release(); return LIW_OK; }
+    launch_laser_slab_pack(b->B, b->n, slabs, (long)b->Ltot, v.group_off, c->lpk2_perm.as<int>(), b->laser_pts, c->lpk2_off.as<long long>(), c->lpk2_mx.as<int>(), c->lpk2.as<double>(), s);
+    c->lpk2_slabs = slabs;
+    c->lpk_gens += 1; c->lpk_last_rows = rows;
+    *packed = true;
+    return LIW_OK;
+}
+static void take_laser_rows(LinArgs& A, const liw_ctx* c) {
+    A.laser_pk = c->lpk.as<double>(); A.laser_slab_off = c->lpk_off.as<long long>(); A.laser_perm = c->lpk_perm.as<int>();
+    A.laser_mx = c->lpk_mx.as<int>(); A.laser_slabs = 0;
 }
 static LinArgs lin_args(const liw_batch* b, int mode, const double* x, const WsView& v, int candidate, bool use_lm, bool packed = false, const liw_ctx* c = nullptr, const void* ws = nullptr) {
     LinArgs A{};
@@ -324,7 +358,7 @@
     for (int k = 0; k < 2; ++k) A.CS[k] = v.pi_frame ? v.CS[k] : nullptr;
     if (packed && b->n > 1 && b->eval_small) { A.imu_pk = v.imu_pk; A.imu_pk_bad = v.imu_pk_bad; }
     if (packed) A.laser_hz = v.imu_pk_bad + 1;
-    if (packed && lpk_matches(c, b, ws)) { A.laser_pk = c->lpk.as<double>(); A.laser_slab_off = c->lpk_off.as<long long>(); A.laser_perm = c->lpk_perm.as<int>(); }
+    if (packed && lpk_matches(c, b, ws)) take_laser_rows(A, c);
     return A;
 }
 static StepArgs step_args(liw_ctx* c, const liw_batch* b, int mode, int max_iters, const WsView& v) {
@@ -364,6 +398,7 @@
     } else {
         (void)hipMemsetAsync(v.imu_pk_bad + 1, 0xff, sizeof(int), s);
         c->lpk_on = false;
+        c->lpk2_slabs = 0; c->lpk_gens = 0; c->lpk_last_rows = 0;
     }
     HIPCHK(c, hipGetLastError());
     return LIW_OK;
@@ -380,6 +415,13 @@
     if (int r = check_batch(c, b)) return r;
     if (rows) *rows = lpk_matches(c, b, ws) ? c->lpk_rows : 0;
     if (blocks) *blocks = (long long)b->Ltot;
+    return LIW_OK;
+}
+int liw_batch_repack_stats(liw_ctx* c, int* generations, long long* rows_first, long long* rows_last) {
+    if (!c) return LIW_EINVAL;
+    if (generations) *generations = c->lpk_gens;
+    if (rows_first) *rows_first = c->lpk_gens > 0 ? c->lpk_rows : 0;
+    if (rows_last) *rows_last = c->lpk_last_rows;
     return LIW_OK;
 }
 int liw_batch_lm_linearize(liw_ctx* c, const liw_batch* b, int mode, int candidate, void* ws, void* stream) {
@@ -598,14 +640,20 @@
     if (pack) launch_imu_pack(b->B, b->n, b->imu_X, b->imu_J, b->imu_sqrtP, b->imu_Dt, v.imu_pk, v.imu_pk_bad, s);
     if (pack) launch_laser_z_scan(b->Ltot, b->laser_pts, v.imu_pk_bad + 1, s);
     c->lpk_on = false;
+    c->lpk2_slabs = 0; c->lpk_gens = 0; c->lpk_last_rows = 0;
     if (pack) {
         hipStreamCaptureStatus cap = hipStreamCaptureStatusNone;
         (void)hipStreamIsCapturing(s, &cap);
         if (int r = laser_slab_begin(c, b, mode, v, ws, s, cap == hipStreamCaptureStatusNone)) return r;
     }
+    struct DropSurvivors { liw_ctx* c; ~DropSurvivors() { c->lpk2_slabs = 0; } } drop_survivors{c};
     StepArgs st = step_args(c, b, mode, K, v);
     auto lin = [&](int cand) {
         LinArgs A = lin_args(b, mode, cand ? v.x_cand : b->x, v, cand, true, pack, c, ws);
+        if (A.laser_pk && c->lpk2_slabs > 0) {
+            A.laser_pk = c->lpk2.as<double>(); A.laser_slab_off = c->lpk2_off.as<long long>(); A.laser_perm = c->lpk2_perm.as<int>();
+            A.laser_mx = c->lpk2_mx.as<int>(); A.laser_slabs = c->lpk2_slabs;
+        }
         if (timed) (void)hipEventRecord(next_event(c->ev_lin, c->ev_lin_used), s);
         launch_linearize(A, c->dp, s, c->have_fork ? &c->fork : nullptr);
         if (timed) (void)hipEventRecord(next_event(c->ev_lin, c->ev_lin_used), s);
@@ -620,6 +668,11 @@
     (void)hipStreamIsCapturing(s, &capst);
     const bool no_exit = std::getenv("LIW_NO_EARLY_EXIT") != nullptr;
     const bool can_exit = capst == hipStreamCaptureStatusNone && !no_exit && lin_builds_active_list(b->B, b->eval_small);
+    constexpr double REPACK_LAUNCHES = 2.5, REPACK_RHO = 0.5, REPACK_FIXED = 2048.0, REPACK_CHIP = 2048.0;
+    const double repack_frames = mode == LIW_MODE_TRACK ? 1.0 : (double)b->n;
+    const bool repack_always = std::getenv("LIW_LASER_REPACK_ALWAYS") != nullptr;
+    const bool can_repack = can_exit && !std::getenv("LIW_NO_LASER_REPACK") && lpk_matches(c, b, ws);
+    int packed_windows = b->B;
     int next_check = can_exit ? 3 : K + 1;
     for (int k = 0; k < K; ++k) {
         step();
@@ -633,6 +686,14 @@
             HIPCHK(c, hipStreamSynchronize(s));
             if (act[1] != 1 || act[0] < 0 || act[0] > b->B) { next_check = K + 1; continue; }
             if (act[0] == 0) break;
+            const int live = act[0];
+            const double wl = laser_slab_count(live) * repack_frames;
+            const double saved = std::max(laser_slab_count(packed_windows) * repack_frames, REPACK_CHIP) - std::max(wl, REPACK_CHIP);
+            if (can_repack && live < packed_windows && (repack_always || saved * (K - (k + 1)) * REPACK_RHO >= REPACK_LAUNCHES * wl + REPACK_FIXED)) {
+                bool ok = false;
+                if (int r = laser_slab_repack(c, b, mode, v, live, s, &ok)) return r;
+                packed_windows = ok ? live : b->B;
+            }
             next_check += act[0] > b->B / 4 ? (mode == LIW_MODE_TRACK ? 3 : 8) : (act[0] > b->B / 64 ? 3 : 2);
         }
     }
@@ -665,6 +726,7 @@
             c->gkey = key;
         }
         c->lpk_on = false;
+        c->lpk2_slabs = 0; c->lpk_gens = 0; c->lpk_last_rows = 0;
         HIPCHK(c, hipGraphLaunch(c->gexec, s));
         return LIW_OK;
     }
@@ -680,7 +742,7 @@
     hipStream_t s = (hipStream_t)stream;
     launch_group_offsets(b->B, b->n, b->laser_off, b->laser_frame, v.group_off, s);
     LinArgs A = lin_args(b, LIW_MODE_MARG, b->x, v, 0, false);
-    if (lpk_matches(c, b, ws)) { A.laser_pk = c->lpk.as<double>(); A.laser_slab_off = c->lpk_off.as<long long>(); A.laser_perm = c->lpk_perm.as<int>(); }
+    if (lpk_matches(c, b, ws)) take_laser_rows(A, c);
     if (c->timing) (void)hipEventRecord(next_event(c->ev_lin, c->ev_lin_used), s);
     launch_linearize(A, c->dp, s, c->have_fork ? &c->fork : nullptr);
     if (c->timing) (void)hipEventRecord(next_event(c->ev_lin, c->ev_lin_used), s);
@@ -766,7 +828,7 @@
     {
         launch_group_offsets(b->B, b->n, b->laser_off, b->laser_frame, v.group_off, s);
         LinArgs A = lin_args(b, LIW_MODE_MARG, b->x, v, 0, false);
-        if (lpk_matches(c, b, ws)) { A.laser_pk = c->lpk.as<double>(); A.laser_slab_off = c->lpk_off.as<long long>(); A.laser_perm = c->lpk_perm.as<int>(); }
+        if (lpk_matches(c, b, ws)) take_laser_rows(A, c);
         A.role_mask = 6;
         launch_linearize(A, c->dp, s, nullptr);
         (void)hipEventRecord(m[0], s);
diff --git a/2dliw-slam_amd/csrc/liw_kernels.hpp b/2dliw-slam_amd/csrc/liw_kernels.hpp
--- a/2dliw-slam_amd/csrc/liw_kernels.hpp
+++ b/2dliw-slam_amd/csrc/liw_kernels.hpp
@@ -125,6 +125,8 @@
     const double* laser_pk;
     const long long* laser_slab_off;
     const int* laser_perm;
+    const int* laser_mx;
+    int laser_slabs;
     int role_mask;
     double* dbg_laser_res; double* dbg_laser_jac; double* dbg_imu_res; double* dbg_imu_jac;
     double* dbg_wheel_res; double* dbg_wheel_jac; double* dbg_ground_res; double* dbg_ground_jac;
@@ -276,8 +278,9 @@
 void launch_laser_z_scan(long Ltot, const double* laser_pts, int* flag, hipStream_t s);
 __host__ __device__ inline int laser_slab_count(int B) { return (B + 63) / 64; }
 void launch_laser_slab_prepare(int B, int n, const int* group_off, int* perm, int* mx, long long* off, const int* hz, hipStream_t s);
+void launch_laser_slab_prepare_live(int B, int n, int slabs, int f_lo, const int* group_off, const LmState* lm, const int* list, int cand, int* perm, int* mx, long long* off, int* taken, hipStream_t s);
 constexpr int LASER_SLAB_ROWD = 8 * 64;
-void launch_laser_slab_pack(int B, int n, long Ltot, const int* group_off, const int* perm, const double* pts, const long long* off, const int* mx, double* pk, hipStream_t s);
+void launch_laser_slab_pack(int B, int n, int slabs, long Ltot, const int* group_off, const int* perm, const double* pts, const long long* off, const int* mx, double* pk, hipStream_t s);
 void launch_lin_laser_slab(const LinArgs& A, const DevParams& P, hipStream_t s);
 void launch_imu_pack(int B, int n, const double* imu_X, const double* imu_J, const double* imu_sqrtP, const double* imu_Dt, double* pk, int* bad, hipStream_t s);
 void launch_pack_result(const PackArgs& a, hipStream_t s);
diff --git a/include/liw_window.h b/include/liw_window.h
--- a/include/liw_window.h
+++ b/include/liw_window.h
@@ -113,6 +113,7 @@
 int liw_batch_lm_begin(liw_ctx* ctx, const liw_batch* b, int mode, int max_iters, void* ws, void* stream);
 int liw_batch_launch_paths(liw_ctx* ctx, const liw_batch* b, const void* ws, int* flags);
 int liw_batch_packed_rows(liw_ctx* ctx, const liw_batch* b, const void* ws, long long* rows, long long* blocks);
+int liw_batch_repack_stats(liw_ctx* ctx, int* generations, long long* rows_first, long long* rows_last);
 int liw_batch_lm_linearize(liw_ctx* ctx, const liw_batch* b, int mode, int candidate, void* ws, void* stream);
 int liw_batch_laser_records(liw_ctx* ctx, const liw_batch* b, int mode, int buffer, void* ws, double* out, void* stream);
 int liw_batch_lm_step(liw_ctx* ctx, const liw_batch* b, int mode, void* ws, void* stream);
```

Result: no change. 142,100 solves/s, median of 3 (+0.7%).
